# SiyuanHuang95/SUG

Measured on AMD Instinct MI355X. Metric: point-clouds/sec (train step, N=1024), higher is better.
Workload: dtype f32

## Files before the change

include/sug_amd.h:

```cpp
#ifndef SUG_AMD_H
#define SUG_AMD_H

#include <stdint.h>

#ifdef __cplusplus
extern "C" {
#endif

#define SUG_OK 0
#define SUG_ERR_ARG (-1)
#define SUG_ERR_LAUNCH (-2)
#define SUG_STATS_BLOCKS 1024

const char* sug_last_error(void);
#define SUG_ABI_VERSION 7
int sug_abi_version(void);

int sug_knn(const float* x, int64_t ldx, int B, int N, int C, int k,
            int32_t* idx, void* stream);

int sug_knn_reverse(const int32_t* idx, int B, int N, int k,
                    int32_t* rev_off, int32_t* rev_ent, void* stream);

int sug_fps(const float* xyz, const int32_t* start, int B, int N, int npoint,
            int32_t* out, void* stream);

int sug_ball_query(const float* xyz, const float* query, int B, int N, int S,
                   float r2, int nsample, int32_t* out, void* stream);

int sug_knn_query(const float* xyz, const float* query, int B, int N, int S,
                  int k, int32_t* idx_out, float* dist_out, void* stream);
int sug_knn_query_direct(const float* xyz, const float* query, int B, int N, int S, int k,
                         int32_t* idx_out, float* dist_out, void* stream);

int sug_three_nn(const float* query, const float* cand, int B, int N, int S,
                 int32_t* idx3, float* dist3, void* stream);

int sug_three_nn_direct(const float* query, const float* cand, int B, int N, int S,
                        int32_t* idx3, float* dist3, void* stream);

int sug_ball_query_multi(const float* xyz, const float* query, int B, int N, int S, int R, const float* r2,
                         const int32_t* nsample, int32_t* const* out, void* stream);

int sug_fp_interp_fwd(const float* src, int64_t lds, const int32_t* idx3, const float* d3, int B, int N, int S, int D,
                      float* out, int64_t ldo, float* w3, void* stream);
int sug_fp_interp_bwd(const float* g, int64_t ldg, const int32_t* idx3, const float* w3, int B, int N, int S, int D,
                      int32_t* rev_off, int32_t* rev_ent, float* dsrc, int64_t ldd, void* stream);

int sug_copy_rows2d(const float* src, int64_t lds, float* dst, int64_t ldd, int64_t rows, int C, void* stream);

int sug_gather_rows(const float* feat, int64_t ldf, const int32_t* idx,
                    int B, int N, int S, int C, float* out, int64_t ldo, void* stream);
int sug_scatter_add_rows(const float* g, int64_t ldg, const int32_t* idx,
                         int B, int N, int S, int C, float* dfeat, int64_t ldf, void* stream);
int64_t sug_scatter_rows_workspace(int B, int N, int S);
int sug_scatter_rows_ordered_supported(int B, int N, int S);
int sug_scatter_rows_ordered(const float* g, int64_t ldg, const int32_t* idx, int B, int N, int S, int C,
                             float* dfeat, int64_t ldf, int32_t* ws, void* stream);

int sug_group_max(const float* feat, int64_t ldf, const int32_t* idx, int B, int N, int S,
                  int ns, int C, float* out, int32_t* arg, void* stream);
int sug_group_max_bwd(const float* g, const int32_t* arg, int B, int N, int S, int C,
                      float* dfeat, int64_t ldf, void* stream);

int sug_edgeconv_fwd(const float* pq, int64_t ldpq, const int32_t* idx, const float* gamma,
                     int B, int N, int k, int Co, float* z, uint8_t* arg, float* s1,
                     double* stats, float* ws, void* stream);

int sug_bn_finalize(const double* stats, const float* gamma, const float* beta, int C,
                    double count, float eps, float momentum, float* running_mean,
                    float* running_var, float* coef, void* stream);

int sug_edgeconv_fwd_bn(const float* pq, int64_t ldpq, const int32_t* idx, const float* gamma,
                        const float* beta, int B, int N, int k, int Co, float eps, float momentum,
                        float* running_mean, float* running_var, float* z, uint8_t* arg, float* s1,
                        float* coef, float* ws, void* stream);
int sug_col_stats_bn(const float* y, int64_t ldy, int64_t rows, int C, const float* gamma, const float* beta,
                     float eps, float momentum, float* running_mean, float* running_var, float* coef,
                     float* ws, void* stream);

int sug_col_stats_bn_grouped(const float* y, int64_t ldy, int64_t rows, int C, int groups, const float* gamma,
                             const float* beta, float eps, float momentum, float* running_mean, float* running_var,
                             float* coef, float* ws, void* stream);

int sug_bn_replay(const float* coef, int G, int C, float momentum, float* running_mean, float* running_var,
                  void* stream);
int sug_bn_replay_multi(int n, const void* const* coef, const int32_t* G, const int32_t* C, const float* momentum,
                        void* const* running_mean, void* const* running_var, void* stream);

int sug_affine_act(const float* z, int64_t ldz, const float* coef, int64_t rows, int C,
                   float slope, float* out, int64_t ldo, void* stream);

int sug_col_stats(const float* y, int64_t ldy, int64_t rows, int C, double* stats, float* ws,
                  void* stream);

int sug_edgeconv_bwd_reduce(const float* gout, int64_t ldg, const float* z, const float* coef,
                            int64_t rows, int Co, float slope, float* a, double* red, float* ws,
                            void* stream);
int sug_edgeconv_bwd_scatter(const float* a, const uint8_t* arg, const float* s1,
                             const float* pq, int64_t ldpq, const int32_t* rev_off,
                             const int32_t* rev_ent, const float* coef, const double* red,
                             int B, int N, int k, int Co, float* dpq, int64_t lddpq, void* stream);

int64_t sug_linear_dw_workspace(int64_t R, int M, int N);
int sug_linear_dw(const float* g, int64_t ldg, const float* x, int64_t ldx, int64_t R, int M, int N,
                  float* dw, float* ws, void* stream);
int sug_linear_dw_fold(const float* part, int nchunk, int64_t MN, float* dw, void* stream);
int sug_linear_dw_bias(const float* g, int64_t ldg, const float* x, int64_t ldx, int64_t R, int M, int N,
                       float* dw, float* db, float* ws, void* stream);

int64_t sug_colsum_workspace(int64_t rows, int C);
int sug_colsum(const void* x, int64_t ld, int64_t rows, int C, int dtype, float sign, float* out, float* ws, void* stream);

int sug_gate_fwd(const float* x, const float* z, int64_t n, float* out, void* stream);
int sug_gate_bwd(const float* g, const float* x, const float* z, int64_t n, float* dx, float* dz, void* stream);
int sug_gate_bn_fwd(const float* x, const float* z, int M, int C, const float* gamma, const float* beta,
                    float* running_mean, float* running_var, int training, float eps, float momentum, float* out,
                    float* stat, void* stream);
int sug_gate_bn_bwd(const float* g, const float* x, const float* z, int M, int C, const float* gamma, const float* stat,
                    int training, float* dx, float* dz, float* dgamma, float* dbeta, void* stream);

int sug_calayer_supported(int layers, int M, int C, int Hd);
int sug_calayer_fwd(int layers, const float* x, int64_t ldx, int M, int C, int Hd, const float* const* W0,
                    const float* const* b0, const float* const* W2, const float* const* b2, float* hp, float* h, float* z,
                    void* stream);
int sug_calayer_bwd(int layers, const float* x, int64_t ldx, int M, int C, int Hd, const float* const* W0,
                    const float* const* W2, const float* h, const float* dz, const float* dxg, float* const* dW0,
                    float* const* db0, float* const* dW2, float* const* db2, float* dhp, float* dh, float* dx, int64_t lddx,
                    void* stream);

int sug_head_linear_supported(int M, int K, int No, int pro, int epi);
int sug_head_linear_fwd(int heads, const float* const* in, int64_t ldin, const float* const* W, const float* const* bias,
                        float* const* z, const float* const* gamma, const float* const* beta, const float* const* u,
                        float* const* stats, float* const* act, int M, int K, int No, int pro, float slope, float eps,
                        float p_drop, void* stream);
int sug_head_ln_bwd(int heads, const float* const* gup, int64_t ldg, const float* const* z, const float* const* stats,
                    const float* const* gamma, const float* const* beta, const float* const* u,
                    const float* const* gextra, float* const* dz, float* const* dgamma, float* const* dbeta,
                    float* const* db, int M, int No, float slope, float p_drop, void* stream);
int sug_head_linear_bwd(int heads, int sum_da, const float* const* dz, int64_t ldg, const float* const* in, int64_t ldin,
                        const float* const* stats_in, const float* const* gamma_in, const float* const* beta_in,
                        const float* const* u_in, const float* const* W, float* const* dW, float* const* db,
                        float* const* da, int64_t ldda, int M, int K, int No, int pro, float slope, float p_drop_in,
                        void* stream);

int sug_ln_act_fwd(const float* x, const float* gamma, const float* beta, int rows, int C, float eps, float slope,
                   float* y, float* stat, void* stream);
int sug_ln_act_bwd(const float* g, const float* x, const float* gamma, const float* beta, const float* stat, int rows,
                   int C, float slope, float* dx, float* dgamma, float* dbeta, float* ws, void* stream);

int sug_adam_chunk(void);
int sug_adam_step(const int64_t* table, const int32_t* block_first, const int32_t* block_first_host, int T,
                  const void* const* grads_host, double lr, double beta1, double beta2, double eps,
                  double weight_decay, double bias_corr1, double bias_corr2, void* stream);
int sug_adam_step_capturable(const int64_t* table, const int32_t* block_first, const int32_t* block_first_host,
                             int T, const void* const* grads_host, double lr, double beta1, double beta2,
                             double eps, double weight_decay, int32_t* step_dev, float* scalars_dev,
                             const double* lr_dev, void* stream);

#define SUG_ADAM_CHAIN_SLOTS 2
#define SUG_ADAM_CHAIN_BUCKETS 8
int sug_adam_chain_chunk(void);
int sug_adam_chain_step(const int64_t* table, const int32_t* block_map, const int32_t* block_first_host, int T,
                        const void* const* grads_host, int nbuckets, const double* hyper_host, int32_t* steps_dev,
                        float* scalars_dev, const double* lr_dev, void* stream);

int sug_node_offset_fwd(const float* proj, const float* loc, const int32_t* fidx,
                        const int32_t* gidx, int B, int N, int S, int ns, float* off, float* nloc,
                        void* stream);
int sug_node_offset_bwd(const float* proj, const float* loc, const int32_t* fidx,
                        const int32_t* gidx, const float* goff, int B, int N, int S, int ns,
                        float* dproj, void* stream);
int sug_interp3_cat_fwd(const float* fea, int64_t ldf, int C1, const float* node,
                        const int32_t* idx3, const float* d3, int B, int N, int S, int C2,
                        float* out, int64_t ldo, void* stream);
int sug_interp3_cat_bwd(const float* g, int64_t ldg, int C1, const float* node, const int32_t* idx3,
                        const float* d3, const float* xyz, const float* nloc, int B, int N, int S,
                        int C2, float* dnode, float* dnloc, void* stream);
int sug_interp3_cat_bwd_lists(const float* g, int64_t ldg, int C1, const float* node, const int32_t* idx3,
                              const float* d3, const float* xyz, const float* nloc, int B, int N, int S, int C2,
                              int32_t* rev_off, int32_t* rev_ent, float* ddw, float* dnode, float* dnloc,
                              void* stream);
int sug_interp3_cat_bwd_lists_supported(int B, int N, int S);

int sug_bn_bwd_apply(const float* a, const float* y, int64_t ldy, const float* coef,
                     const double* red, int64_t rows, int C, float* dy, int64_t lddy, void* stream);

int sug_bn_act_pool_fwd(const float* y, int64_t ldy, const float* coef, int B, int N, int C,
                        float slope, float* out_max, float* out_mean, int64_t ld_pool, int32_t* arg, float* ws,
                        void* stream);
int sug_bn_act_pool_bwd(const float* y, int64_t ldy, const float* coef, const float* gmax,
                        const float* gmean, int64_t ld_pool, const int32_t* arg, int B, int N, int C, float slope,
                        int train, double* red, float* ws, float* dy, int64_t lddy, void* stream);

int sug_edgeconv_layer_fwd(const float* pq, int64_t ldpq, const int32_t* idx, const float* gamma,
                           const float* beta, int B, int N, int k, int Co, int groups, int training,
                           float eps, float momentum, float slope, float* running_mean,
                           float* running_var, float* z, uint8_t* arg, float* s1, float* coef,
                           float* out, int64_t ldo, double* stats, float* ws, void* stream);
int sug_edgeconv_fused_supported(int N, int k, int Cin, int Co);
int sug_edgeconv_fused_layer_fwd(const float* x, int64_t ldx, int Cin, const float* wcat, const float* qbias,
                                 const int32_t* idx, const float* gamma, const float* beta, int B, int N, int k,
                                 int Co, int groups, int training, float eps, float momentum, float slope,
                                 float* running_mean, float* running_var, float* z, uint8_t* arg, float* s1,
                                 float* pq_out, int64_t ldpq, float* coef, float* out, int64_t ldo, float* ws,
                                 void* stream);
int sug_edgeconv_layer_bwd(const float* gout, int64_t ldg, const float* z, const uint8_t* arg,
                           const float* s1, const float* pq, int64_t ldpq, const int32_t* idx,
                           const float* coef, int B, int N, int k, int Co, int groups, int training,
                           float slope, float* a, double* red, int32_t* rev_off, int32_t* rev_ent,
                           float* dpq, int64_t lddpq, float* ws, float* dgb, void* stream);
int sug_sa_first_fwd(const float* P, int64_t ldp, const float* Q, const int32_t* idx, int B, int N, int S,
                     int ns, int C, int groups, const float* gamma, const float* beta, int training,
                     float eps, float momentum, float* running_mean, float* running_var, float* coef,
                     float* Z, float* ws, void* stream);
int sug_sa_first_bwd(const float* gz, const float* P, int64_t ldp, const float* Q, const int32_t* idx, int B,
                     int N, int S, int ns, int C, int groups, int training, const float* coef, double* red,
                     int32_t* rev_off, int32_t* rev_ent, float* segsum, float* dP, float* dQ, float* ws, float* dgb,
                     void* stream);
int sug_sa_first_geo_fwd(const float* Pf, int64_t ldp, const float* xyz, const float* cent, const float* Wx, int ldw,
                         const float* bias, const int32_t* idx, int B, int N, int S, int ns, int C, int groups,
                         const float* gamma, const float* beta, int training, float eps, float momentum,
                         float* running_mean, float* running_var, float* coef, float* Z, float* ws, void* stream);
int sug_sa_first_geo_bwd(const float* gz, const float* Pf, int64_t ldp, const float* xyz, const float* cent, const float* Wx,
                         int ldw, const float* bias, const int32_t* idx, int B, int N, int S, int ns, int C, int groups,
                         int training, const float* coef, double* red, int32_t* rev_off, int32_t* rev_ent, float* segsum,
                         float* dP, float* dQ, float* ws, float* dgb, void* stream);

int sug_bn_act_rows_fwd(const float* y, int64_t ldy, int64_t rows, int C, int groups, const float* gamma,
                        const float* beta, int training, float eps, float momentum, float slope,
                        float* running_mean, float* running_var, float* coef, float* out, int64_t ldo,
                        double* stats, float* ws, void* stream);
int sug_bn_act_rows_bwd(const float* gout, int64_t ldg, const float* y, int64_t ldy, const float* coef,
                        int64_t rows, int C, int groups, int training, float slope, float* a, double* red,
                        float* dy, float* ws, float* dgb, void* stream);
int sug_bn_act_pool_layer_fwd(const float* y, int64_t ldy, int B, int N, int C, int groups,
                              const float* gamma, const float* beta, int training, float eps, float momentum,
                              float slope, float* running_mean, float* running_var, float* coef,
                              float* out_max, float* out_mean, int64_t ld_pool, int32_t* arg, double* stats, float* ws_stats,
                              float* ws_pool, void* stream);
int sug_bn_act_pool_layer_bwd(const float* y, int64_t ldy, const float* coef, const float* gmax,
                              const float* gmean, int64_t ld_pool, const int32_t* arg, int B, int N, int C, int groups,
                              float slope, int training, double* red, float* ws, float* dy, int64_t lddy,
                              float* dgb, void* stream);

int sug_pointmlp_max_fwd(const float* x, int64_t ldx, int64_t rows, int K, const float* w, const float* bias,
                         const float* gamma, int Co, int seg, float* zext, int32_t* arg, float* ws, int* nblk,
                         void* stream);
int sug_rows_gemm(const float* x, int64_t ldx, int64_t rows, int K, const float* w, const float* bias, int Co,
                  float* y, int64_t ldy, void* stream);
int sug_pointmlp_max_layer_fwd(const float* x, int64_t ldx, int64_t rows, int K, const float* w, const float* bias,
                               const float* gamma, const float* beta, int Co, int seg, int groups, int training,
                               float eps, float momentum, float slope, float* running_mean, float* running_var,
                               float* zext, int32_t* arg, float* coef, float* out, int64_t ldo, float* ws,
                               void* stream);
int sug_pointmlp_max_layer_fwd_xf(const float* y, int64_t ldy, int64_t rows, int K, const float* xcoef, float xslope,
                                  float* zout, int64_t ldz, const float* w, const float* bias, const float* gamma,
                                  const float* beta, int Co, int seg, int groups, int training, float eps, float momentum,
                                  float slope, float* running_mean, float* running_var, float* zext, int32_t* arg,
                                  float* coef, float* out, int64_t ldo, float* ws, void* stream);
int sug_pointmlp_max_bwd_coef(const float* coef, const double* red, const float* bias, const float* w, int64_t rows,
                              int K, int Co, float* kb, float* k2, float* nkb, float* nwk, void* stream);
int sug_pointmlp_max_bwd_dwfix(float* dw, const float* dws, const float* kb, const float* k2, const float* w,
                               const float* xtx, const float* sx, int K, int Co, int with_stats, void* stream);
int64_t sug_pointmlp_max_bwd_workspace(int64_t rows, int K, int Co, int seg);
int sug_pointmlp_max_bwd_sparse(const float* a, const int32_t* arg, const float* x, int64_t ldx, const float* w,
                                int64_t rows, int K, int Co, int seg, float* dx, int64_t lddx, float* dw,
                                float* ws, void* stream);

int sug_ptran_pos1_fwd(const float* xyz, const int32_t* nbr, const float* w1, const float* b1, int B, int n, int k,
                       int d, int dtype, void* out, void* stream);
int sug_ptran_pos1_bwd(const void* g, const float* xyz, const int32_t* nbr, const float* w1, const float* b1, int B,
                       int n, int k, int d, int dtype, float* dw1, float* db1, float* ws, void* stream);
int sug_ptran_qk_fwd(const float* q, const float* kf, const void* delta, const int32_t* nbr, int B, int n, int k, int d,
                     int dtype, void* out, void* stream);
int sug_ptran_qk_bwd(const void* du, void* da, const int32_t* rev_off, const int32_t* rev_ent, int B, int n, int k, int d,
                     int dtype, float* dq, float* dk, float* db, float* ws, void* stream);
int sug_ptran_attn_fwd(const void* logits, const void* delta, const float* vf, const int32_t* nbr, int B, int n, int k,
                       int d, int dtype, float scale, float* mixed, float* mx, float* sm, void* stream);
int sug_ptran_attn_bwd(const float* g, const float* mixed, const void* logits, const void* delta, const float* vf,
                       const int32_t* nbr, const float* mx, const float* sm, const int32_t* rev_off, const int32_t* rev_ent,
                       int B, int n, int k, int d, int dtype, float scale, void* dlogits, void* da, float* dv, float* db,
                       float* ws, void* stream);
int sug_ptran_fused_supported(int B, int n, int k, int d);
int sug_ptran_fused_fwd(const float* xyz, const int32_t* nbr, const float* q, const float* kf, const float* vf,
                        const float* w1, const float* b1, const void* w2, const void* b2, const void* wg1, const void* bg1,
                        const void* wg2, const void* bg2, int B, int n, int k, int d, float scale, int save, void* T0,
                        void* delta, void* U, void* T1, void* Lg, float* mixed, float* mx, float* sm, void* stream);
int64_t sug_ptran_colsum_workspace(int64_t rows);
int sug_ptran_relu_bwd_db(void* G, const void* T1, int64_t rows, int d, int dtype, float* db, float* ws, void* stream);
int sug_grad_scale16(const float* g0, int64_t n0, const float* g1, int64_t n1, const float* g2, int64_t n2, int log2_target,
                     float* out, float* ws, void* stream);

int sug_fold_groups(const double* red, int groups, int n, float* out, void* stream);

int sug_mmd_rbf(const float* z, int64_t ldz, int m, int D, const float* w,
                const float* neg_gamma, int nsigma, double* sums, float* wt, void* stream);

int sug_mmd_rbf_value(const float* z, int64_t ldz, int m, int D, const float* w, const float* neg_gamma,
                      int nsigma, double* sums, float* wt, float* value, void* stream);

int sug_mmd_rbf_bwd(const float* z, int64_t ldz, const float* wt, int m, int D, const float* gscale,
                    float* dz, int64_t lddz, void* stream);

int sug_mmd_rbf_rows(const float* z, int64_t ldz, int m, int D, const float* w, const float* neg_gamma,
                     int nsigma, int row0, int mloc, double* sums, float* wt, void* stream);
int sug_mmd_rbf_rows_bwd(const float* z, int64_t ldz, const float* wt, int m, int D, int row0, int mloc,
                         const float* gscale, float gmul, float* dz, int64_t lddz, void* stream);

int sug_sda_prob_weights(const float* pred_s, int64_t lds, const float* pred_t, int64_t ldt,
                         const int64_t* label_s, const int64_t* label_t, int m, int num_class,
                         float label_weight, int method, float* weights, void* stream);
int sug_sda_prob_weights_multi(int n, const void* const* pred_s, const int64_t* lds, const void* const* pred_t,
                               const int64_t* ldt, const int64_t* label_s, const int64_t* label_t, int m, int num_class,
                               float label_weight, int method, void* const* weights, void* stream);

int sug_mmd_assemble(const float* feat_s, int64_t lds, const float* feat_t, int64_t ldt, const int64_t* label_s,
                     const int64_t* label_t, int m, int D, int num_class, float label_scale, float* z, void* stream);

int sug_soft_mmd_multi_fwd(int n, const void* const* feat_s, const int64_t* lds, const void* const* feat_t,
                           const int64_t* ldt, const int32_t* D, const float* label_scale, const int64_t* label_s,
                           const int64_t* label_t, int m, int num_class, const void* const* w, const float* neg_gamma,
                           int nsigma, void* const* z, void* const* wt, double* sums, float* values, void* stream);
int sug_soft_mmd_multi_bwd(int n, const void* const* z, const int32_t* D, const void* const* wt,
                           const void* const* gscale, int m, int num_class, void* const* dz, void* stream);

#define SUG_CLASS_MMD_MAX_ROWS 1024
#define SUG_CLASS_MMD_MAX_CLASSES 64
#define SUG_CLASS_MMD_MAX_D 1048576
int sug_mmd_select(const int64_t* label_s, const int64_t* label_t, int m, int num_class, int mode, int32_t* idx_s,
                   int32_t* idx_t, int32_t* pos_s, int32_t* pos_t, int32_t* count, void* stream);
int sug_class_mmd_fwd(const float* feat_s, int64_t lds, const float* feat_t, int64_t ldt, int m, int D,
                      const int32_t* idx_s, const int32_t* idx_t, const int32_t* count, const float* neg_gamma,
                      int nsigma, float* z, float* wt, double* sums, float* value, void* stream);
int sug_class_mmd_bwd(const float* z, const float* wt, int m, int D, const int32_t* count, const int32_t* pos_s,
                      const int32_t* pos_t, const float* gscale, float* dz, float* dfeat_s, int64_t ldds,
                      float* dfeat_t, int64_t lddt, void* stream);

#define SUG_MMD_EST_MAX_ROWS 1024
#define SUG_MMD_EST_MAX_D 1048576
#define SUG_MMD_EST_MAX_SIGMAS 8
#define SUG_MMD_POLY_MAX_DEGREE 8
#define SUG_MMD_RATIO_ROW_FIELDS 9
#define SUG_MMD_RATIO_STATS 16
int sug_mmd_ratio_fwd(const float* z, int64_t ldz, int m, int D, const float* neg_gamma, int nsigma, int biased, float* K,
                      float* G, double* rows, double* stats, float* out3, float* wt_m, float* wt_v, void* stream);
int sug_mmd_ratio_bwd(const float* z, int64_t ldz, int m, int D, const float* wt_m, const float* wt_v, const float* out3,
                      const float* g3, float* dz, int64_t lddz, void* stream);
int sug_mmd_adjacent_fwd(const float* x, int64_t ldx, const float* y, int64_t ldy, int m, int D, int mode, int degree,
                         double alpha, double c, double* part, float* coef, float* value, void* stream);
int sug_mmd_adjacent_bwd(const float* x, int64_t ldx, const float* y, int64_t ldy, int m, int D, int mode, const float* coef,
                         const float* gscale, float* dx, int64_t lddx, float* dy, int64_t lddy, void* stream);

#define SUG_CL_LOSS_MAX_ROWS 1024
#define SUG_CL_LOSS_MAX_D 1048576
#define SUG_CL_LOSS_MAX_TERMS 4
#define SUG_CL_LOSS_SUM_FIELDS 3
#define SUG_CL_LOSS_ROW_FIELDS 4
int sug_cl_loss_fwd(int n, const void* const* x, const int64_t* ldx, const void* const* y, const int64_t* ldy, const int32_t* D,
                    const double* margin, const int64_t* label_s, const int64_t* label_t, int m, const void* const* w,
                    double* sums, void* const* coef, float* values, void* stream);
int sug_cl_loss_bwd(int n, const void* const* x, const int64_t* ldx, const void* const* y, const int64_t* ldy, const int32_t* D,
                    int m, const void* const* coef, const void* const* gscale, void* const* dx, const int64_t* lddx,
                    void* const* dy, const int64_t* lddy, void* stream);

int sug_edge_weight_split(const float* in, int Co, int C, int backward, float* out, void* stream);
int sug_edge_weight_split_multi(const void* const* in_host, const int32_t* Co_host, const int32_t* C_host, int n,
                                int backward, void* const* out_host, void* stream);

int64_t sug_chamfer_workspace(int B, int N, int M);
int sug_chamfer(const float* a, const float* b, int B, int N, int M, float* out, float* ws, void* stream);
int sug_chamfer_weights(const float* a, const float* b, int B, int N, int M, int method, float* out, float* ws, void* stream);

#define SUG_CE_PAIR_MAX_ROWS 512
#define SUG_CE_PAIR_MAX_CLASSES 32
int sug_ce_pair_fwd(const float* logits1, const float* logits2, int64_t ld, const int64_t* label, int M, int C, float w,
                    int64_t ignore_index, float* loss, float* lse, void* stream);
int sug_ce_pair_bwd(const float* logits1, const float* logits2, int64_t ld, const int64_t* label, int M, int Mtot, int C,
                    float w, int64_t ignore_index, const float* g, const float* lse, float* d1, float* d2, void* stream);
#define SUG_CE_MAX_ROWS 1024
#define SUG_CE_MAX_CLASSES 64
int sug_ce_fwd(const float* logits, int64_t ld, const int64_t* label, int M, int C, int64_t ignore_index, float label_smoothing,
               float* loss, float* lse, double* totals, void* stream);
int sug_ce_bwd(const float* logits, int64_t ld, const int64_t* label, int M, int C, int64_t ignore_index, float label_smoothing,
               const float* g, const float* lse, float* dlogits, void* stream);
#define SUG_MCD_MAX_ROWS 1024
int sug_mcd_loss_fwd(const float* ys1, const float* ys2, const float* yt1, const float* yt2, int64_t ld, const int64_t* label,
                     const int64_t* label_t, int Ms, int Mt, int C, float a_s, float a_t, float r_s, float* out4, float* lse,
                     double* totals, void* stream);
int sug_mcd_loss_bwd(const float* ys1, const float* ys2, const float* yt1, const float* yt2, int64_t ld, const int64_t* label,
                     const int64_t* label_t, int Ms, int Mt, int C, float a_s, float a_t, const float* g, const float* lse,
                     float* ds1, float* ds2, float* dt1, float* dt2, void* stream);
int sug_cls_loss_fwd(const float* ys1, const float* ys2, const float* yt1, const float* yt2, int64_t ld, const int64_t* label,
                     const int64_t* label_t, int Ms, int Mt, int C, const float* alpha, float gamma, int reduce_sum,
                     int64_t ignore_index, float a_s, float a_t, float a_d, float r_s, float* out4, float* save, double* totals,
                     void* stream);
int sug_cls_loss_bwd(const float* ys1, const float* ys2, const float* yt1, const float* yt2, int64_t ld, const int64_t* label,
                     const int64_t* label_t, int Ms, int Mt, int C, const float* alpha, float gamma, int reduce_sum,
                     int64_t ignore_index, float a_s, float a_t, float a_d, float r_s, const float* g, const float* save,
                     float* ds1, float* ds2, float* dt1, float* dt2, void* stream);
int sug_loss_combine_fwd(const float* loss_cls, const float* v_geo, const float* v_sem1, const float* v_sem2, float wg, float ws,
                         float* out3, void* stream);
int sug_loss_combine_bwd(const float* g, float wg, float ws, float* out4, void* stream);

#define SUG_EVAL_MAX_ROWS 4096
#define SUG_EVAL_MAX_CLASSES 64
#define SUG_EVAL_BATCH_COUNT 0
#define SUG_EVAL_DATA_TOTAL 1
#define SUG_EVAL_CORRECT_TOTAL 2
#define SUG_EVAL_ERROR 3
#define SUG_EVAL_LOSS_TOTAL 4
#define SUG_EVAL_CLASS_ACC 8
#define SUG_EVAL_CLASS_ROWS 136
#define SUG_EVAL_CLASS_CORRECT 200
#define SUG_EVAL_BATCH_ACC 264
#define SUG_EVAL_STATE_WORDS(cap) (SUG_EVAL_BATCH_ACC + (cap))
int sug_eval_accumulate(const float* logits1, const float* logits2, int64_t ld, const int64_t* label, int B, int C,
                        const float* loss_in, int ce_mode, int64_t ignore_index, float label_smoothing, float* out,
                        int64_t* pred, int cls_eval, void* state, int cap, void* stream);


#define SUG_KPCONV_MAX_CLOUD 4096
int sug_grid_subsample(const float* pts, const int32_t* off, int B, int cap, float dl, float* out_pad, int32_t* cnt,
                       float* out, int32_t* out_off, void* stream);
int sug_radius_neighbors(const float* q, const int32_t* qoff, int Nq, const float* s, const int32_t* soff, int Ns, int B,
                         float radius, int limit, int32_t* out, void* stream);
int sug_radius_reverse(const int32_t* nbr, const int32_t* qoff, const int32_t* soff, int B, int H, int Ns, int cap,
                       int32_t* rev_be, int32_t* rev_ent, void* stream);
int sug_kpconv_fwd(const float* q, const float* s, const int32_t* nbr, int Nq, int H, int Ns, const float* kp, int K,
                   float extent, const float* x, int Cin, float* wf, float* w, float* cnt, void* stream);
int sug_kpconv_bwd(const int32_t* rev_be, const int32_t* rev_ent, int H, int K, const float* w, const float* cnt,
                   const float* dwf, int Ns, int Cin, float* dx, void* stream);
int sug_seg_instnorm_fwd(const float* x, const int32_t* off, int B, int C, float eps, int mode, const float* sc, float* y,
                         float* mean, float* rstd, void* stream);
int sug_seg_instnorm_bwd(const float* g, const float* y, const float* x, const float* mean, const float* rstd,
                         const int32_t* off, int B, int C, int mode, float* dx, float* dsc, void* stream);
int sug_seg_max_pool_fwd(const float* x, const int32_t* nbr, int Nq, int H, int Ns, int C, float* y, int32_t* arg,
                         void* stream);
int sug_seg_max_pool_bwd(const float* g, const int32_t* arg, const int32_t* rev_be, const int32_t* rev_ent, int H, int Ns,
                         int C, float* dx, void* stream);
int sug_seg_mean_fwd(const float* x, const int32_t* off, int B, int C, float* y, void* stream);
int sug_seg_mean_bwd(const float* g, const int32_t* off, int B, int N, int C, float* dx, void* stream);
#define SUG_KPCONV_RECORD_INTS 8
int sug_grid_subsample_cap(const float* pts, const int32_t* off, int B, int cap, float dl, int C, int level, float* out_pad,
                           int32_t* cnt, float* out, int32_t* out_off, int32_t* record, void* stream);
int sug_radius_neighbors_cap(const float* q, const int32_t* qoff, int Cq, const float* s, const int32_t* soff, int Cs, int B,
                             float radius, int limit, int32_t* out, void* stream);
int sug_radius_reverse_cap(const int32_t* nbr, const int32_t* qoff, const int32_t* soff, int B, int H, int Cs, int cap,
                           int32_t* rev_be, int32_t* rev_ent, void* stream);
int sug_kpconv_fwd_cap(const float* q, const float* s, const int32_t* nbr, const int32_t* nq_valid, int Cq, int H, int Cs,
                       const float* kp, int K, float extent, const float* x, int Cin, float* wf, float* w, float* cnt,
                       void* stream);
int sug_seg_instnorm_fwd_cap(const float* x, const int32_t* off, int B, int N, int C, float eps, int mode, const float* sc,
                             float* y, float* mean, float* rstd, void* stream);
int sug_seg_instnorm_bwd_cap(const float* g, const float* y, const float* x, const float* mean, const float* rstd,
                             const int32_t* off, int B, int N, int C, int mode, float* dx, float* dsc, void* stream);
int sug_seg_mean_fwd_cap(const float* x, const int32_t* off, int B, int C, float* y, void* stream);
int sug_seg_mean_bwd_cap(const float* g, const int32_t* off, int B, int N, int C, float* dx, void* stream);
int sug_kp_sample_rows(const float* x, const int32_t* off, int B, int S, int D, float* out, void* stream);

int sug_ptcls_head_supported(int B, int P, int K, int N1, int N2, int NC);
int sug_ptcls_head_fwd(const float* points, int B, int P, int K, const float* W1, const float* b1, int N1, const float* W2,
                       const float* b2, int N2, const float* W3, const float* b3, int NC, float* mean, float* h1, float* h2,
                       float* logits, void* stream);
int sug_ptcls_head_bwd(const float* dlogits, const float* mean, const float* h1, const float* h2, int B, int P, int K,
                       const float* W1, int N1, const float* W2, int N2, const float* W3, int NC, float* dz1, float* dz2,
                       float* dpoints, float* dW1, float* db1, float* dW2, float* db2, float* dW3, float* db3,
                       void* stream);

#define SUG_PREP_MAX_POINTS 4096
#define SUG_PREP_NORMALIZE 1
#define SUG_PREP_ROTATE_Z 2
#define SUG_PREP_JITTER 4
#define SUG_PREP_SHUFFLE 8
#define SUG_PREP_DRAW_ANGLE 0x00000000u
#define SUG_PREP_DRAW_SUBSET 0x10000000u
#define SUG_PREP_DRAW_NOISE 0x20000000u
int sug_prepare_batch(const float* pts, int M, int P, const int32_t* idx, int B, int N, int stages,
// ... 33 lines not shown
```

sug_amd/csrc/adapt.hip:

```cpp
#include "common.h"

namespace {

__global__ __launch_bounds__(256) void node_offset_fwd_kernel(const float* __restrict__ proj,
                                                              const float* __restrict__ loc,
                                                              const int32_t* __restrict__ fidx,
                                                              const int32_t* __restrict__ gidx, int N,
                                                              int S, int ns, int total,
                                                              float* __restrict__ off,
                                                              float* __restrict__ nloc) {
  const int e = blockIdx.x * 4 + (threadIdx.x >> 6);
  if (e >= total) return;
  const int lane = threadIdx.x & 63;
  const int b = e / S;
  const float* pb = proj + (int64_t)b * N * 3;
  const float* lb = loc + (int64_t)b * N * 3;
  int f = fidx[e];
  f = f < 0 ? 0 : (f >= N ? N - 1 : f);
  const float pcx = pb[f * 3 + 0], pcy = pb[f * 3 + 1], pcz = pb[f * 3 + 2];
  const float lcx = lb[f * 3 + 0], lcy = lb[f * 3 + 1], lcz = lb[f * 3 + 2];
  float ax = 0.f, ay = 0.f, az = 0.f;
  const int32_t* g = gidx + (int64_t)e * ns;
  for (int j = lane; j < ns; j += 64) {
    const int n = g[j];
    if (n < 0 || n >= N) continue;
    ax += tanhf(pb[n * 3 + 0] - pcx) * (lb[n * 3 + 0] - lcx);
    ay += tanhf(pb[n * 3 + 1] - pcy) * (lb[n * 3 + 1] - lcy);
    az += tanhf(pb[n * 3 + 2] - pcz) * (lb[n * 3 + 2] - lcz);
  }
  ax = wave_sum_f(ax); ay = wave_sum_f(ay); az = wave_sum_f(az);
  if (lane == 0) {
    const float inv = 1.0f / (float)ns;
    ax *= inv; ay *= inv; az *= inv;
    off[e * 3 + 0] = ax; off[e * 3 + 1] = ay; off[e * 3 + 2] = az;
    nloc[e * 3 + 0] = lcx + ax; nloc[e * 3 + 1] = lcy + ay; nloc[e * 3 + 2] = lcz + az;
  }
}

__global__ __launch_bounds__(256) void node_offset_bwd_kernel(const float* __restrict__ proj,
                                                              const float* __restrict__ loc,
                                                              const int32_t* __restrict__ fidx,
                                                              const int32_t* __restrict__ gidx,
                                                              const float* __restrict__ goff, int N,
                                                              int S, int ns, int total,
                                                              float* __restrict__ dproj) {
  const int e = blockIdx.x * 4 + (threadIdx.x >> 6);
  if (e >= total) return;
  const int lane = threadIdx.x & 63;
  const int b = e / S;
  const float* pb = proj + (int64_t)b * N * 3;
  const float* lb = loc + (int64_t)b * N * 3;
  float* db = dproj + (int64_t)b * N * 3;
  int f = fidx[e];
  f = f < 0 ? 0 : (f >= N ? N - 1 : f);
  const float pcx = pb[f * 3 + 0], pcy = pb[f * 3 + 1], pcz = pb[f * 3 + 2];
  const float lcx = lb[f * 3 + 0], lcy = lb[f * 3 + 1], lcz = lb[f * 3 + 2];
  const float inv = 1.0f / (float)ns;
  const float gx = goff[e * 3 + 0] * inv, gy = goff[e * 3 + 1] * inv, gz = goff[e * 3 + 2] * inv;
  float cx = 0.f, cy = 0.f, cz = 0.f;
  const int32_t* g = gidx + (int64_t)e * ns;
  for (int j = lane; j < ns; j += 64) {
    const int n = g[j];
    if (n < 0 || n >= N) continue;
    const float tx = tanhf(pb[n * 3 + 0] - pcx), ty = tanhf(pb[n * 3 + 1] - pcy), tz = tanhf(pb[n * 3 + 2] - pcz);
    const float vx = gx * (lb[n * 3 + 0] - lcx) * (1.f - tx * tx);
    const float vy = gy * (lb[n * 3 + 1] - lcy) * (1.f - ty * ty);
    const float vz = gz * (lb[n * 3 + 2] - lcz) * (1.f - tz * tz);
    atomicAdd(&db[n * 3 + 0], vx); atomicAdd(&db[n * 3 + 1], vy); atomicAdd(&db[n * 3 + 2], vz);
    cx += vx; cy += vy; cz += vz;
  }
  cx = wave_sum_f(cx); cy = wave_sum_f(cy); cz = wave_sum_f(cz);
  if (lane == 0) {
    atomicAdd(&db[f * 3 + 0], -cx); atomicAdd(&db[f * 3 + 1], -cy); atomicAdd(&db[f * 3 + 2], -cz);
  }
}

__global__ __launch_bounds__(1024) void node_offset_bwd_lds_kernel(const float* __restrict__ proj,
                                                                   const float* __restrict__ loc,
                                                                   const int32_t* __restrict__ fidx,
                                                                   const int32_t* __restrict__ gidx,
                                                                   const float* __restrict__ goff, int N, int S,
                                                                   int ns, float* __restrict__ dproj) {
  extern __shared__ float s_d[];
  const int b = blockIdx.x;
  const int lane = threadIdx.x & 63, wave = threadIdx.x >> 6;
  for (int i = threadIdx.x; i < N * 3; i += 1024) s_d[i] = 0.f;
  __syncthreads();
  const float* pb = proj + (int64_t)b * N * 3;
  const float* lb = loc + (int64_t)b * N * 3;
  const float inv = 1.0f / (float)ns;
  for (int sn = wave; sn < S; sn += 16) {
    const int e = b * S + sn;
    int f = fidx[e];
    f = f < 0 ? 0 : (f >= N ? N - 1 : f);
    const float pcx = pb[f * 3 + 0], pcy = pb[f * 3 + 1], pcz = pb[f * 3 + 2];
    const float lcx = lb[f * 3 + 0], lcy = lb[f * 3 + 1], lcz = lb[f * 3 + 2];
    const float gx = goff[e * 3 + 0] * inv, gy = goff[e * 3 + 1] * inv, gz = goff[e * 3 + 2] * inv;
    float cx = 0.f, cy = 0.f, cz = 0.f;
    const int32_t* g = gidx + (int64_t)e * ns;
    for (int j = lane; j < ns; j += 64) {
      const int n = g[j];
      if (n < 0 || n >= N) continue;
      const float tx = tanhf(pb[n * 3 + 0] - pcx), ty = tanhf(pb[n * 3 + 1] - pcy), tz = tanhf(pb[n * 3 + 2] - pcz);
      const float vx = gx * (lb[n * 3 + 0] - lcx) * (1.f - tx * tx);
      const float vy = gy * (lb[n * 3 + 1] - lcy) * (1.f - ty * ty);
      const float vz = gz * (lb[n * 3 + 2] - lcz) * (1.f - tz * tz);
      atomicAdd(&s_d[n * 3 + 0], vx); atomicAdd(&s_d[n * 3 + 1], vy); atomicAdd(&s_d[n * 3 + 2], vz);
      cx += vx; cy += vy; cz += vz;
    }
    cx = wave_sum_f(cx); cy = wave_sum_f(cy); cz = wave_sum_f(cz);
    if (lane == 0) {
      atomicAdd(&s_d[f * 3 + 0], -cx); atomicAdd(&s_d[f * 3 + 1], -cy); atomicAdd(&s_d[f * 3 + 2], -cz);
    }
  }
  __syncthreads();
  float* db = dproj + (int64_t)b * N * 3;
  for (int i = threadIdx.x; i < N * 3; i += 1024) db[i] = s_d[i];
}

template <int P>
__global__ __launch_bounds__(64 * P) void node_offset_bwd_ordered_kernel(const float* __restrict__ proj,
                                                                         const float* __restrict__ loc,
                                                                         const int32_t* __restrict__ fidx,
                                                                         const int32_t* __restrict__ gidx,
                                                                         const float* __restrict__ goff, int N, int S,
                                                                         int ns, float* __restrict__ dproj) {
  extern __shared__ __attribute__((aligned(16))) float s_o[];
  const int lane = threadIdx.x & 63, wave = threadIdx.x >> 6;
  float* plane = s_o + (size_t)wave * 3 * N;
  int* tag = reinterpret_cast<int*>(s_o + (size_t)P * 3 * N) + (size_t)wave * N;
  const int b = blockIdx.x;
  for (int i = lane; i < 3 * N; i += 64) plane[i] = 0.f;
  __builtin_amdgcn_wave_barrier();
  const float* pb = proj + (int64_t)b * N * 3;
  const float* lb = loc + (int64_t)b * N * 3;
  const float inv = 1.0f / (float)ns;
  auto add_node = [&](int n, float vx, float vy, float vz) {
    if (n >= 0) tag[n] = 0x7fffffff;
    __builtin_amdgcn_wave_barrier();
    if (n >= 0) atomicMin(&tag[n], lane);
    __builtin_amdgcn_wave_barrier();
    const int leader = n >= 0 ? tag[n] : lane;
    unsigned long long dup = __ballot(leader != lane);
    float ax = vx, ay = vy, az = vz;
    while (dup) {
      const int i = __builtin_ctzll(dup);
      dup &= dup - 1;
      const int li = __builtin_amdgcn_readlane(leader, i);
      const float dx = __int_as_float(__builtin_amdgcn_readlane(__float_as_int(vx), i));
      const float dy = __int_as_float(__builtin_amdgcn_readlane(__float_as_int(vy), i));
      const float dz = __int_as_float(__builtin_amdgcn_readlane(__float_as_int(vz), i));
      const bool mine = lane == li;
      ax = mine ? ax + dx : ax; ay = mine ? ay + dy : ay; az = mine ? az + dz : az;
    }
    if (n >= 0 && leader == lane) {
      plane[n * 3 + 0] += ax; plane[n * 3 + 1] += ay; plane[n * 3 + 2] += az;
    }
    __builtin_amdgcn_wave_barrier();
  };
  auto centre = [&](int f, float cx, float cy, float cz) {
    cx = wave_sum_f(cx); cy = wave_sum_f(cy); cz = wave_sum_f(cz);
    if (lane == 0) {
      plane[f * 3 + 0] -= cx; plane[f * 3 + 1] -= cy; plane[f * 3 + 2] -= cz;
    }
    __builtin_amdgcn_wave_barrier();
  };
  if (ns <= 64) {
    struct Idx { int f, n; float gx, gy, gz; };
    struct Val { float pc[3], lc[3], pn[3], ln[3]; };
    auto load_idx = [&](int sn) {
      Idx r;
      const int e = b * S + sn;
      int f = fidx[e];
      r.f = f < 0 ? 0 : (f >= N ? N - 1 : f);
      int n = lane < ns ? gidx[(int64_t)e * ns + lane] : -1;
      r.n = n >= N ? -1 : n;
      r.gx = goff[e * 3 + 0] * inv; r.gy = goff[e * 3 + 1] * inv; r.gz = goff[e * 3 + 2] * inv;
      return r;
    };
    auto load_val = [&](const Idx& ix) {
      Val v;
      const int n = ix.n >= 0 ? ix.n : ix.f;
#pragma unroll
      for (int d = 0; d < 3; ++d) {
        v.pc[d] = pb[ix.f * 3 + d]; v.lc[d] = lb[ix.f * 3 + d];
        v.pn[d] = pb[n * 3 + d];    v.ln[d] = lb[n * 3 + d];
      }
      return v;
    };
    Idx i0 = {}, i1 = {};
    Val v0 = {};
    if (wave < S) { i0 = load_idx(wave); v0 = load_val(i0); }
    if (wave + P < S) i1 = load_idx(wave + P);
    for (int sn = wave; sn < S; sn += P) {
      const Idx ci = i0;
      const Val cv = v0;
      i0 = i1;
      if (sn + P < S) v0 = load_val(i0);
      if (sn + 2 * P < S) i1 = load_idx(sn + 2 * P);
      float vx = 0.f, vy = 0.f, vz = 0.f;
      if (ci.n >= 0) {
        const float tx = tanhf(cv.pn[0] - cv.pc[0]), ty = tanhf(cv.pn[1] - cv.pc[1]), tz = tanhf(cv.pn[2] - cv.pc[2]);
        vx = ci.gx * (cv.ln[0] - cv.lc[0]) * (1.f - tx * tx);
        vy = ci.gy * (cv.ln[1] - cv.lc[1]) * (1.f - ty * ty);
        vz = ci.gz * (cv.ln[2] - cv.lc[2]) * (1.f - tz * tz);
      }
      add_node(ci.n, vx, vy, vz);
      centre(ci.f, vx, vy, vz);
    }
  } else {
    for (int sn = wave; sn < S; sn += P) {
      const int e = b * S + sn;
      int f = fidx[e];
      f = f < 0 ? 0 : (f >= N ? N - 1 : f);
      const float pcx = pb[f * 3 + 0], pcy = pb[f * 3 + 1], pcz = pb[f * 3 + 2];
      const float lcx = lb[f * 3 + 0], lcy = lb[f * 3 + 1], lcz = lb[f * 3 + 2];
      const float gx = goff[e * 3 + 0] * inv, gy = goff[e * 3 + 1] * inv, gz = goff[e * 3 + 2] * inv;
      float cx = 0.f, cy = 0.f, cz = 0.f;
      const int32_t* g = gidx + (int64_t)e * ns;
      for (int j0 = 0; j0 < ns; j0 += 64) {
        const int j = j0 + lane;
        int n = j < ns ? g[j] : -1;
        if (n >= N) n = -1;
        float vx = 0.f, vy = 0.f, vz = 0.f;
        if (n >= 0) {
          const float tx = tanhf(pb[n * 3 + 0] - pcx), ty = tanhf(pb[n * 3 + 1] - pcy), tz = tanhf(pb[n * 3 + 2] - pcz);
          vx = gx * (lb[n * 3 + 0] - lcx) * (1.f - tx * tx);
          vy = gy * (lb[n * 3 + 1] - lcy) * (1.f - ty * ty);
          vz = gz * (lb[n * 3 + 2] - lcz) * (1.f - tz * tz);
        }
        cx += vx; cy += vy; cz += vz;
        add_node(n, vx, vy, vz);
      }
      centre(f, cx, cy, cz);
    }
  }
  __syncthreads();
  float* db = dproj + (int64_t)b * N * 3;
  for (int i = threadIdx.x; i < N * 3; i += 64 * P) {
    float a = s_o[i];
#pragma unroll
    for (int p = 1; p < P; ++p) a += s_o[(size_t)p * 3 * N + i];
    db[i] = a;
  }
}

__global__ __launch_bounds__(256) void interp3_cat_fwd_kernel(const float* __restrict__ fea, int64_t ldf,
                                                              int C1, const float* __restrict__ node,
                                                              const int32_t* __restrict__ idx3,
                                                              const float* __restrict__ d3, int N, int S,
                                                              int C2, int64_t BN, float* __restrict__ out,
                                                              int64_t ldo) {
  const int64_t p = (int64_t)blockIdx.x * 16 + threadIdx.x / 16;
  if (p >= BN) return;
  const int lane = threadIdx.x & 15;
  const int64_t b = p / N;
  const float r0 = 1.0f / fmaxf(d3[p * 3 + 0], 1e-10f), r1 = 1.0f / fmaxf(d3[p * 3 + 1], 1e-10f),
              r2 = 1.0f / fmaxf(d3[p * 3 + 2], 1e-10f);
  const float R = (r0 + r1) + r2;
  const float w0 = r0 / R, w1 = r1 / R, w2 = r2 / R;
  const float* n0 = node + (b * S + idx3[p * 3 + 0]) * C2;
  const float* n1 = node + (b * S + idx3[p * 3 + 1]) * C2;
  const float* n2 = node + (b * S + idx3[p * 3 + 2]) * C2;
  for (int c = lane * 4; c < C1; c += 64)
    *reinterpret_cast<float4*>(out + p * ldo + c) = *reinterpret_cast<const float4*>(fea + p * ldf + c);
  for (int c = lane * 4; c < C2; c += 64) {
    const float4 a = *reinterpret_cast<const float4*>(n0 + c), bq = *reinterpret_cast<const float4*>(n1 + c),
                 cq = *reinterpret_cast<const float4*>(n2 + c);
    float4 o;
    o.x = (a.x * w0 + bq.x * w1) + cq.x * w2; o.y = (a.y * w0 + bq.y * w1) + cq.y * w2;
    o.z = (a.z * w0 + bq.z * w1) + cq.z * w2; o.w = (a.w * w0 + bq.w * w1) + cq.w * w2;
    *reinterpret_cast<float4*>(out + p * ldo + C1 + c) = o;
  }
}

__global__ __launch_bounds__(256) void interp3_cat_bwd_kernel(const float* __restrict__ g, int64_t ldg,
                                                              int C1, const float* __restrict__ node,
                                                              const int32_t* __restrict__ idx3,
                                                              const float* __restrict__ d3,
                                                              const float* __restrict__ xyz,
                                                              const float* __restrict__ nloc, int N,
                                                              int S, int C2, int chunks,
                                                              float* __restrict__ dnode,
                                                              float* __restrict__ dnloc) {
  extern __shared__ float s_acc[];
  float* s_dn = s_acc;
  float* s_dl = s_acc + S * C2;
  const int b = blockIdx.y, ck = blockIdx.x;
  for (int i = threadIdx.x; i < S * C2 + S * 3; i += 256) s_acc[i] = 0.f;
  __syncthreads();
  const int lane = threadIdx.x & 15, grp = threadIdx.x >> 4;
  const int n0 = (int)((int64_t)N * ck / chunks), n1 = (int)((int64_t)N * (ck + 1) / chunks);
  const float* nodeb = node + (int64_t)b * S * C2;
  for (int n = n0 + grp; n < n1 + 15; n += 16) {
    const bool live = n < n1;
    const int64_t p = (int64_t)b * N + (live ? n : n0);
    const float d0 = d3[p * 3 + 0], d1 = d3[p * 3 + 1], d2 = d3[p * 3 + 2];
    const float r0 = 1.0f / fmaxf(d0, 1e-10f), r1 = 1.0f / fmaxf(d1, 1e-10f), r2 = 1.0f / fmaxf(d2, 1e-10f);
    const float R = (r0 + r1) + r2;
    const float w0 = r0 / R, w1 = r1 / R, w2 = r2 / R;
    const int i0 = idx3[p * 3 + 0], i1 = idx3[p * 3 + 1], i2 = idx3[p * 3 + 2];
    float s0 = 0.f, s1 = 0.f, s2 = 0.f;
    if (live) {
      for (int c = lane * 4; c < C2; c += 64) {
        const float4 gv = *reinterpret_cast<const float4*>(g + p * ldg + C1 + c);
        const float4 a = *reinterpret_cast<const float4*>(nodeb + i0 * C2 + c);
        const float4 bq = *reinterpret_cast<const float4*>(nodeb + i1 * C2 + c);
        const float4 cq = *reinterpret_cast<const float4*>(nodeb + i2 * C2 + c);
        const float gg[4] = {gv.x, gv.y, gv.z, gv.w};
        const float aa[4] = {a.x, a.y, a.z, a.w}, bb[4] = {bq.x, bq.y, bq.z, bq.w}, cc[4] = {cq.x, cq.y, cq.z, cq.w};
#pragma unroll
        for (int v = 0; v < 4; ++v) {
          const float o = (aa[v] * w0 + bb[v] * w1) + cc[v] * w2;
          s0 += gg[v] * (aa[v] - o); s1 += gg[v] * (bb[v] - o); s2 += gg[v] * (cc[v] - o);
          atomicAdd(&s_dn[i0 * C2 + c + v], w0 * gg[v]);
          atomicAdd(&s_dn[i1 * C2 + c + v], w1 * gg[v]);
          atomicAdd(&s_dn[i2 * C2 + c + v], w2 * gg[v]);
        }
      }
    }
#pragma unroll
    for (int o = 8; o > 0; o >>= 1) {
      s0 += __shfl_xor(s0, o); s1 += __shfl_xor(s1, o); s2 += __shfl_xor(s2, o);
    }
    if (live && lane < 3) {
      const float sv = lane == 0 ? s0 : (lane == 1 ? s1 : s2);
      const float d = lane == 0 ? d0 : (lane == 1 ? d1 : d2);
      const float r = lane == 0 ? r0 : (lane == 1 ? r1 : r2);
      const int i = lane == 0 ? i0 : (lane == 1 ? i1 : i2);
      const float dd = (d < 1e-10f) ? 0.f : -(r * r / R) * sv;
      const float* q = xyz + p * 3;
      const float* cpos = nloc + ((int64_t)b * S + i) * 3;
      atomicAdd(&s_dl[i * 3 + 0], dd * 2.f * (cpos[0] - q[0]));
      atomicAdd(&s_dl[i * 3 + 1], dd * 2.f * (cpos[1] - q[1]));
      atomicAdd(&s_dl[i * 3 + 2], dd * 2.f * (cpos[2] - q[2]));
    }
  }
  __syncthreads();
  float* dnb = dnode + (int64_t)b * S * C2;
  float* dlb = dnloc + (int64_t)b * S * 3;
  for (int i = threadIdx.x; i < S * C2; i += 256) atomicAdd(&dnb[i], s_dn[i]);
  for (int i = threadIdx.x; i < S * 3; i += 256) atomicAdd(&dlb[i], s_dl[i]);
}

__global__ __launch_bounds__(256) void interp3_bwd_point_kernel(const float* __restrict__ g, int64_t ldg, int C1,
                                                                const float* __restrict__ node,
                                                                const int32_t* __restrict__ idx3,
                                                                const float* __restrict__ d3, int N, int S, int C2,
                                                                int64_t BN, float* __restrict__ ddw) {
  const int64_t p = (int64_t)blockIdx.x * 16 + threadIdx.x / 16;
  if (p >= BN) return;
  const int lane = threadIdx.x & 15;
  const int64_t b = p / N;
  const float d0 = d3[p * 3 + 0], d1 = d3[p * 3 + 1], d2 = d3[p * 3 + 2];
  const float r0 = 1.0f / fmaxf(d0, 1e-10f), r1 = 1.0f / fmaxf(d1, 1e-10f), r2 = 1.0f / fmaxf(d2, 1e-10f);
  const float R = (r0 + r1) + r2;
  const float w0 = r0 / R, w1 = r1 / R, w2 = r2 / R;
  const float* n0 = node + (b * S + idx3[p * 3 + 0]) * C2;
  const float* n1 = node + (b * S + idx3[p * 3 + 1]) * C2;
  const float* n2 = node + (b * S + idx3[p * 3 + 2]) * C2;
  float s0 = 0.f, s1 = 0.f, s2 = 0.f;
  for (int c = lane * 4; c < C2; c += 64) {
    const float4 gv = *reinterpret_cast<const float4*>(g + p * ldg + C1 + c);
    const float4 a = *reinterpret_cast<const float4*>(n0 + c), bq = *reinterpret_cast<const float4*>(n1 + c),
                 cq = *reinterpret_cast<const float4*>(n2 + c);
    const float gg[4] = {gv.x, gv.y, gv.z, gv.w};
    const float aa[4] = {a.x, a.y, a.z, a.w}, bb[4] = {bq.x, bq.y, bq.z, bq.w}, cc[4] = {cq.x, cq.y, cq.z, cq.w};
#pragma unroll
    for (int v = 0; v < 4; ++v) {
      const float o = (aa[v] * w0 + bb[v] * w1) + cc[v] * w2;
      s0 += gg[v] * (aa[v] - o); s1 += gg[v] * (bb[v] - o); s2 += gg[v] * (cc[v] - o);
    }
  }
#pragma unroll
  for (int o = 8; o > 0; o >>= 1) {
    s0 += __shfl_xor(s0, o); s1 += __shfl_xor(s1, o); s2 += __shfl_xor(s2, o);
  }
  if (lane < 3) {
    const float sv = lane == 0 ? s0 : (lane == 1 ? s1 : s2);
    const float d = lane == 0 ? d0 : (lane == 1 ? d1 : d2);
    const float r = lane == 0 ? r0 : (lane == 1 ? r1 : r2);
    const float w = lane == 0 ? w0 : (lane == 1 ? w1 : w2);
    ddw[p * 6 + lane] = (d < 1e-10f) ? 0.f : -(r * r / R) * sv;
    ddw[p * 6 + 3 + lane] = w;
  }
}

__global__ __launch_bounds__(256) void interp3_bwd_node_kernel(const float* __restrict__ g, int64_t ldg, int C1,
                                                               const float* __restrict__ ddw,
                                                               const int32_t* __restrict__ rev_off,
                                                               const int32_t* __restrict__ rev_ent,
                                                               const float* __restrict__ xyz,
                                                               const float* __restrict__ nloc, int N, int S, int C2,
                                                               int64_t BS, float* __restrict__ dnode,
                                                               float* __restrict__ dnloc) {
  const int64_t q = (int64_t)blockIdx.x * 16 + threadIdx.x / 16;
  if (q >= BS) return;
  const int lane = threadIdx.x & 15;
  const int64_t b = q / S;
  const int sn = (int)(q - b * S);
  const int32_t* offb = rev_off + b * (S + 1);
  const int off = offb[sn], cnt = offb[sn + 1] - off;
  const int32_t* ent = rev_ent + b * 3 * N + off;
  const int ax = lane < 3 ? lane : 0;
  const float cpos = nloc[q * 3 + ax];
  float dl = 0.f;
  const int npass = (C2 + 63) / 64;
  for (int pass = 0; pass < npass; ++pass) {
    const int c0 = pass * 64 + lane * 4;
    const bool chan = c0 < C2;
    float4 acc = make_float4(0, 0, 0, 0);
    constexpr int JB = 8;
    for (int t0 = 0; t0 < cnt; t0 += JB) {
      int en[JB];
      float4 gv[JB];
      float wv[JB], dv[JB], xv[JB];
#pragma unroll
      for (int t = 0; t < JB; ++t) en[t] = ent[t0 + t < cnt ? t0 + t : cnt - 1];
#pragma unroll
      for (int t = 0; t < JB; ++t) {
        const int n = en[t] / 3, tt = en[t] - 3 * n;
        const int64_t p = b * N + n;
        gv[t] = chan ? *reinterpret_cast<const float4*>(g + p * ldg + C1 + c0) : make_float4(0, 0, 0, 0);
        wv[t] = ddw[p * 6 + 3 + tt];
        dv[t] = ddw[p * 6 + tt];
        xv[t] = xyz[p * 3 + ax];
      }
#pragma unroll
      for (int t = 0; t < JB; ++t) {
        if (t0 + t >= cnt) continue;
        acc.x = fmaf(wv[t], gv[t].x, acc.x); acc.y = fmaf(wv[t], gv[t].y, acc.y);
        acc.z = fmaf(wv[t], gv[t].z, acc.z); acc.w = fmaf(wv[t], gv[t].w, acc.w);
        if (pass == 0) dl += dv[t] * 2.f * (cpos - xv[t]);
      }
    }
    if (chan) *reinterpret_cast<float4*>(dnode + q * C2 + c0) = acc;
  }
  if (lane < 3) dnloc[q * 3 + lane] = dl;
}

}

extern "C" int sug_node_offset_fwd(const float* proj, const float* loc, const int32_t* fidx,
                                   const int32_t* gidx, int B, int N, int S, int ns, float* off,
                                   float* nloc, void* stream) {
  SUG_REQUIRE(proj && loc && fidx && gidx && off && nloc, "sug_node_offset_fwd: null pointer");
  SUG_REQUIRE(B > 0 && N > 0 && S > 0 && ns > 0, "sug_node_offset_fwd: bad shape");
  const int total = B * S;
  hipLaunchKernelGGL(node_offset_fwd_kernel, dim3(sug_divup(total, 4)), dim3(256), 0, (hipStream_t)stream,
                     proj, loc, fidx, gidx, N, S, ns, total, off, nloc);
  SUG_LAUNCH_CHECK("sug_node_offset_fwd");
  return SUG_OK;
}

extern "C" int sug_node_offset_bwd(const float* proj, const float* loc, const int32_t* fidx,
                                   const int32_t* gidx, const float* goff, int B, int N, int S, int ns,
                                   float* dproj, void* stream) {
  SUG_REQUIRE(proj && loc && fidx && gidx && goff && dproj, "sug_node_offset_bwd: null pointer");
  SUG_REQUIRE(B > 0 && N > 0 && S > 0 && ns > 0, "sug_node_offset_bwd: bad shape");
  const int total = B * S;
  hipStream_t st = (hipStream_t)stream;
  {
    static const int unordered = getenv("SUG_NODE_OFFSET_UNORDERED") ? atoi(getenv("SUG_NODE_OFFSET_UNORDERED")) : 0;
    const size_t per_plane = (size_t)N * 4 * sizeof(float);
    if (!unordered && per_plane <= 150 * 1024) {
      if (8 * per_plane <= 150 * 1024) {
        static SugLdsOptIn note;
        if (int rc = sug_allow_dynamic_lds(note, &node_offset_bwd_ordered_kernel<8>, 150 * 1024, "sug_node_offset_bwd")) return rc;
        hipLaunchKernelGGL(node_offset_bwd_ordered_kernel<8>, dim3(B), dim3(512), 8 * per_plane, st, proj, loc, fidx, gidx, goff, N,
                           S, ns, dproj);
      } else if (4 * per_plane <= 150 * 1024) {
        static SugLdsOptIn note;
        if (int rc = sug_allow_dynamic_lds(note, &node_offset_bwd_ordered_kernel<4>, 150 * 1024, "sug_node_offset_bwd")) return rc;
        hipLaunchKernelGGL(node_offset_bwd_ordered_kernel<4>, dim3(B), dim3(256), 4 * per_plane, st, proj, loc, fidx, gidx, goff, N,
                           S, ns, dproj);
      } else if (2 * per_plane <= 150 * 1024) {
        static SugLdsOptIn note;
        if (int rc = sug_allow_dynamic_lds(note, &node_offset_bwd_ordered_kernel<2>, 150 * 1024, "sug_node_offset_bwd")) return rc;
        hipLaunchKernelGGL(node_offset_bwd_ordered_kernel<2>, dim3(B), dim3(128), 2 * per_plane, st, proj, loc, fidx, gidx, goff, N,
                           S, ns, dproj);
      } else {
        static SugLdsOptIn note;
        if (int rc = sug_allow_dynamic_lds(note, &node_offset_bwd_ordered_kernel<1>, 150 * 1024, "sug_node_offset_bwd")) return rc;
        hipLaunchKernelGGL(node_offset_bwd_ordered_kernel<1>, dim3(B), dim3(64), per_plane, st, proj, loc, fidx, gidx, goff, N, S,
                           ns, dproj);
      }
      SUG_LAUNCH_CHECK("sug_node_offset_bwd");
      return SUG_OK;
    }
  }
  if ((size_t)N * 3 * sizeof(float) <= 60 * 1024) {
    hipLaunchKernelGGL(node_offset_bwd_lds_kernel, dim3(B), dim3(1024), (size_t)N * 3 * sizeof(float), st, proj, loc, fidx,
                       gidx, goff, N, S, ns, dproj);
    SUG_LAUNCH_CHECK("sug_node_offset_bwd");
    return SUG_OK;
  }
  if (hipMemsetAsync(dproj, 0, (size_t)B * N * 3 * sizeof(float), st) != hipSuccess) {
    sug_set_error("sug_node_offset_bwd: memset failed");
    return SUG_ERR_LAUNCH;
  }
  hipLaunchKernelGGL(node_offset_bwd_kernel, dim3(sug_divup(total, 4)), dim3(256), 0, st,
                     proj, loc, fidx, gidx, goff, N, S, ns, total, dproj);
  SUG_LAUNCH_CHECK("sug_node_offset_bwd");
  return SUG_OK;
}

extern "C" int sug_interp3_cat_fwd(const float* fea, int64_t ldf, int C1, const float* node,
                                   const int32_t* idx3, const float* d3, int B, int N, int S, int C2,
                                   float* out, int64_t ldo, void* stream) {
  SUG_REQUIRE((fea || C1 == 0) && node && idx3 && d3 && out, "sug_interp3_cat_fwd: null pointer");
  SUG_REQUIRE(B > 0 && N > 0 && S >= 3 && C1 >= 0 && C2 > 0 && C1 % 4 == 0 && C2 % 4 == 0 && ldf % 4 == 0 &&
                  ldo % 4 == 0 && ldo >= C1 + C2 && ldf >= C1,
              "sug_interp3_cat_fwd: bad shape (channel counts and strides must be multiples of 4)");
  SUG_REQUIRE(((uintptr_t)fea % 16 == 0) && ((uintptr_t)node % 16 == 0) && ((uintptr_t)out % 16 == 0),
              "sug_interp3_cat_fwd: pointers must be 16-byte aligned");
  const int64_t BN = (int64_t)B * N;
  hipLaunchKernelGGL(interp3_cat_fwd_kernel, dim3(sug_divup(BN, 16)), dim3(256), 0, (hipStream_t)stream, fea,
                     ldf, C1, node, idx3, d3, N, S, C2, BN, out, ldo);
  SUG_LAUNCH_CHECK("sug_interp3_cat_fwd");
  return SUG_OK;
}

extern "C" int sug_interp3_cat_bwd(const float* g, int64_t ldg, int C1, const float* node,
                                   const int32_t* idx3, const float* d3, const float* xyz,
                                   const float* nloc, int B, int N, int S, int C2, float* dnode,
                                   float* dnloc, void* stream) {
  SUG_REQUIRE(g && node && idx3 && d3 && xyz && nloc && dnode && dnloc, "sug_interp3_cat_bwd: null pointer");
  SUG_REQUIRE(B > 0 && N > 0 && S >= 3 && C2 > 0 && C1 % 4 == 0 && C2 % 4 == 0 && ldg % 4 == 0 &&
                  ldg >= C1 + C2 && ((uintptr_t)g % 16 == 0) && ((uintptr_t)node % 16 == 0),
              "sug_interp3_cat_bwd: bad shape / alignment");
  const size_t sh = (size_t)(S * C2 + S * 3) * sizeof(float);
  SUG_REQUIRE(sh <= 64 * 1024 && B <= 65535, "sug_interp3_cat_bwd: S*C2=%d too large for the LDS accumulator", S * C2);
  int chunks = 512 / B;
  if (chunks < 1) chunks = 1;
  if (chunks > sug_divup(N, 64)) chunks = sug_divup(N, 64);
  hipLaunchKernelGGL(interp3_cat_bwd_kernel, dim3(chunks, B), dim3(256), sh, (hipStream_t)stream, g, ldg, C1, node,
                     idx3, d3, xyz, nloc, N, S, C2, chunks, dnode, dnloc);
  SUG_LAUNCH_CHECK("sug_interp3_cat_bwd");
  return SUG_OK;
}

size_t sug_reverse_lists_lds_bytes(int B, int E, int N, int* ranges);

extern "C" int sug_interp3_cat_bwd_lists_supported(int B, int N, int S) {
  return (B > 0 && N > 0 && S >= 3 && (int64_t)3 * N <= INT32_MAX &&
          sug_reverse_lists_lds_bytes(B, 3 * N, S, nullptr) <= 160 * 1024) ? 1 : 0;
}

extern "C" int sug_interp3_cat_bwd_lists(const float* g, int64_t ldg, int C1, const float* node, const int32_t* idx3,
                                         const float* d3, const float* xyz, const float* nloc, int B, int N, int S, int C2,
                                         int32_t* rev_off, int32_t* rev_ent, float* ddw, float* dnode, float* dnloc,
                                         void* stream) {
  SUG_REQUIRE(g && node && idx3 && d3 && xyz && nloc && rev_off && rev_ent && ddw && dnode && dnloc,
              "sug_interp3_cat_bwd_lists: null pointer");
  SUG_REQUIRE(B > 0 && N > 0 && S >= 3 && C2 > 0 && C1 % 4 == 0 && C2 % 4 == 0 && ldg % 4 == 0 &&
                  ldg >= C1 + C2 && ((uintptr_t)g % 16 == 0) && ((uintptr_t)node % 16 == 0) && ((uintptr_t)dnode % 16 == 0),
              "sug_interp3_cat_bwd_lists: bad shape / alignment");
  hipStream_t st = (hipStream_t)stream;
  if (int rc = sug_reverse_lists(idx3, B, 3 * N, S, 1, rev_off, rev_ent, st)) return rc;
  const int64_t BN = (int64_t)B * N, BS = (int64_t)B * S;
  hipLaunchKernelGGL(interp3_bwd_point_kernel, dim3(sug_divup(BN, 16)), dim3(256), 0, st, g, ldg, C1, node, idx3, d3, N, S, C2,
                     BN, ddw);
  SUG_LAUNCH_CHECK("sug_interp3_cat_bwd_lists(point)");
  hipLaunchKernelGGL(interp3_bwd_node_kernel, dim3(sug_divup(BS, 16)), dim3(256), 0, st, g, ldg, C1, ddw, rev_off, rev_ent, xyz,
                     nloc, N, S, C2, BS, dnode, dnloc);
  SUG_LAUNCH_CHECK("sug_interp3_cat_bwd_lists(node)");
  return SUG_OK;
}
```

sug_amd/csrc/group.hip:

```cpp
#include "common.h"

namespace {

__global__ __launch_bounds__(256) void gather_rows_kernel(const float* __restrict__ feat, int64_t ldf,
                                                          const int32_t* __restrict__ idx, int N,
                                                          int S, int C, int64_t total,
                                                          float* __restrict__ out, int64_t ldo) {
  for (int64_t e = (int64_t)blockIdx.x * 256 + threadIdx.x; e < total; e += (int64_t)gridDim.x * 256) {
    const int c = (int)(e % C);
    const int64_t row = e / C;
    const int b = (int)(row / S);
    const int j = idx[row];
    float v = 0.f;
    if (j >= 0 && j < N) v = feat[((int64_t)b * N + j) * ldf + c];
    out[row * ldo + c] = v;
  }
}

__global__ __launch_bounds__(256) void scatter_add_rows_kernel(const float* __restrict__ g, int64_t ldg,
                                                               const int32_t* __restrict__ idx, int N,
                                                               int S, int C, int64_t total,
                                                               float* __restrict__ dfeat, int64_t ldf) {
  for (int64_t e = (int64_t)blockIdx.x * 256 + threadIdx.x; e < total; e += (int64_t)gridDim.x * 256) {
    const int c = (int)(e % C);
    const int64_t row = e / C;
    const int b = (int)(row / S);
    const int j = idx[row];
    if (j >= 0 && j < N) atomicAdd(&dfeat[((int64_t)b * N + j) * ldf + c], g[row * ldg + c]);
  }
}

__global__ __launch_bounds__(256) void group_max_kernel(const float* __restrict__ feat, int64_t ldf,
                                                        const int32_t* __restrict__ idx, int N, int S,
                                                        int ns, int C, int64_t total,
                                                        float* __restrict__ out,
                                                        int32_t* __restrict__ arg) {
  for (int64_t e = (int64_t)blockIdx.x * 256 + threadIdx.x; e < total; e += (int64_t)gridDim.x * 256) {
    const int c = (int)(e % C);
    const int64_t row = e / C;
    const int b = (int)(row / S);
    const int32_t* ir = idx + row * ns;
    float best = -INFINITY;
    int bj = -1;
    for (int t0 = 0; t0 < ns; t0 += 8) {
      int j[8];
      float v[8];
#pragma unroll
      for (int u = 0; u < 8; ++u) j[u] = ir[t0 + u < ns ? t0 + u : ns - 1];
#pragma unroll
      for (int u = 0; u < 8; ++u) {
        const int jc = j[u] < 0 ? 0 : (j[u] >= N ? N - 1 : j[u]);
        v[u] = feat[((int64_t)b * N + jc) * ldf + c];
      }
#pragma unroll
      for (int u = 0; u < 8; ++u) {
        if (t0 + u >= ns || j[u] < 0 || j[u] >= N) continue;
        if (v[u] > best || bj < 0) {
          best = v[u];
          bj = j[u];
        }
      }
    }
    out[e] = bj < 0 ? 0.f : best;
    arg[e] = bj;
  }
}

__global__ __launch_bounds__(256) void group_max_bwd_kernel(const float* __restrict__ g,
                                                            const int32_t* __restrict__ arg, int N,
                                                            int S, int C, int64_t total,
                                                            float* __restrict__ dfeat, int64_t ldf) {
  for (int64_t e = (int64_t)blockIdx.x * 256 + threadIdx.x; e < total; e += (int64_t)gridDim.x * 256) {
    const int c = (int)(e % C);
    const int64_t row = e / C;
    const int b = (int)(row / S);
    const int j = arg[e];
    if (j >= 0 && j < N) atomicAdd(&dfeat[((int64_t)b * N + j) * ldf + c], g[e]);
  }
}

inline int ew_grid(int64_t total) {
  int64_t g = (total + 255) / 256;
  return (int)(g > 4096 ? 4096 : (g < 1 ? 1 : g));
}

__global__ __launch_bounds__(256) void copy_rows2d_kernel(const float* __restrict__ src, int64_t lds, float* __restrict__ dst,
                                                          int64_t ldd, int64_t R, int C4) {
  const int64_t total = R * C4;
  for (int64_t e = (int64_t)blockIdx.x * 256 + threadIdx.x; e < total; e += (int64_t)gridDim.x * 256) {
    const int64_t r = e / C4;
    const int c = (int)(e - r * C4) * 4;
    *reinterpret_cast<float4*>(dst + r * ldd + c) = *reinterpret_cast<const float4*>(src + r * lds + c);
  }
}

template <int V>
__global__ __launch_bounds__(256) void gather_sum_rows_kernel(const float* __restrict__ g, int64_t ldg,
                                                              const int32_t* __restrict__ rev_off,
                                                              const int32_t* __restrict__ rev_ent, int N, int S, int C,
                                                              int64_t total, float* __restrict__ dfeat, int64_t ldf) {
  const int CV = C / V;
  for (int64_t t = (int64_t)blockIdx.x * 256 + threadIdx.x; t < total; t += (int64_t)gridDim.x * 256) {
    const int c = (int)(t % CV) * V;
    const int64_t row = t / CV;
    const int64_t b = row / N;
    const int n = (int)(row - b * N);
    const int32_t* off = rev_off + b * (N + 1) + n;
    const int e0 = off[0], e1 = off[1];
    const int32_t* ent = rev_ent + b * S;
    float acc[V];
#pragma unroll
    for (int v = 0; v < V; ++v) acc[v] = 0.f;
    for (int i = e0; i < e1; ++i) {
      const float* gr = g + (b * S + ent[i]) * ldg + c;
      if (V == 4) {
        const float4 q = *reinterpret_cast<const float4*>(gr);
        acc[0] += q.x; acc[1] += q.y; acc[2] += q.z; acc[3] += q.w;
      } else {
#pragma unroll
        for (int v = 0; v < V; ++v) acc[v] += gr[v];
      }
    }
#pragma unroll
    for (int v = 0; v < V; ++v) dfeat[row * ldf + c + v] = acc[v];
  }
}

constexpr int GMB_CH = 16;
__global__ __launch_bounds__(256) void group_max_bwd_ordered_kernel(const float* __restrict__ g,
                                                                    const int32_t* __restrict__ arg, int N, int S, int C,
                                                                    float* __restrict__ dfeat, int64_t ldf) {
  extern __shared__ __attribute__((aligned(16))) int s_gm[];
  int (*s_arg)[GMB_CH + 1] = reinterpret_cast<int (*)[GMB_CH + 1]>(s_gm);
  float (*s_g)[GMB_CH + 1] = reinterpret_cast<float (*)[GMB_CH + 1]>(s_gm + 64 * (GMB_CH + 1));
  const int lane = threadIdx.x & 63, wv = threadIdx.x >> 6;
  int* tag = s_gm + 2 * 64 * (GMB_CH + 1) + wv * N;
  const int b = blockIdx.y, c0 = blockIdx.x * GMB_CH;
  const int cc = (C - c0 < GMB_CH) ? C - c0 : GMB_CH;
  for (int e = threadIdx.x; e < S * GMB_CH; e += 256) {
    const int sI = e / GMB_CH, c = e % GMB_CH;
    const bool in = c < cc;
    const int64_t o = ((int64_t)b * S + sI) * C + c0 + c;
    s_arg[sI][c] = in ? arg[o] : -1;
    s_g[sI][c] = in ? g[o] : 0.f;
  }
  __syncthreads();
  for (int c = wv; c < cc; c += 4) {
    int j = lane < S ? s_arg[lane][c] : -1;
    if (j >= N) j = -1;
    const float gv = lane < S ? s_g[lane][c] : 0.f;
    if (j >= 0) tag[j] = 0x7fffffff;
    __builtin_amdgcn_wave_barrier();
    if (j >= 0) atomicMin(&tag[j], lane);
    __builtin_amdgcn_wave_barrier();
    const int leader = j >= 0 ? tag[j] : lane;
    unsigned long long dup = __ballot(leader != lane);
    float acc = gv;
    while (dup) {
      const int i = __builtin_ctzll(dup);
      dup &= dup - 1;
      const int li = __builtin_amdgcn_readlane(leader, i);
      const float gi = __int_as_float(__builtin_amdgcn_readlane(__float_as_int(gv), i));
      acc = (lane == li) ? acc + gi : acc;
    }
    if (j >= 0 && leader == lane) dfeat[((int64_t)b * N + j) * ldf + c0 + c] = acc;
    __builtin_amdgcn_wave_barrier();
  }
}

}

extern "C" int sug_gather_rows(const float* feat, int64_t ldf, const int32_t* idx, int B, int N, int S,
                               int C, float* out, int64_t ldo, void* stream) {
  SUG_REQUIRE(feat && idx && out, "sug_gather_rows: null pointer");
  SUG_REQUIRE(B > 0 && N > 0 && S > 0 && C > 0 && ldf >= C && ldo >= C, "sug_gather_rows: bad shape");
  const int64_t total = (int64_t)B * S * C;
  hipLaunchKernelGGL(gather_rows_kernel, dim3(ew_grid(total)), dim3(256), 0, (hipStream_t)stream, feat,
                     ldf, idx, N, S, C, total, out, ldo);
  SUG_LAUNCH_CHECK("sug_gather_rows");
  return SUG_OK;
}

extern "C" int sug_scatter_add_rows(const float* g, int64_t ldg, const int32_t* idx, int B, int N,
                                    int S, int C, float* dfeat, int64_t ldf, void* stream) {
  SUG_REQUIRE(g && idx && dfeat, "sug_scatter_add_rows: null pointer");
  SUG_REQUIRE(B > 0 && N > 0 && S > 0 && C > 0 && ldf >= C && ldg >= C, "sug_scatter_add_rows: bad shape");
  const int64_t total = (int64_t)B * S * C;
  hipLaunchKernelGGL(scatter_add_rows_kernel, dim3(ew_grid(total)), dim3(256), 0, (hipStream_t)stream,
                     g, ldg, idx, N, S, C, total, dfeat, ldf);
  SUG_LAUNCH_CHECK("sug_scatter_add_rows");
  return SUG_OK;
}

extern "C" int64_t sug_scatter_rows_workspace(int B, int N, int S) { return (int64_t)B * (N + 1) + (int64_t)B * S; }

size_t sug_reverse_lists_lds_bytes(int B, int E, int N, int* ranges);

extern "C" int sug_scatter_rows_ordered_supported(int B, int N, int S) {
  return (B > 0 && N > 0 && S > 0 && sug_reverse_lists_lds_bytes(B, S, N, nullptr) <= 160 * 1024) ? 1 : 0;
}

extern "C" int sug_scatter_rows_ordered(const float* g, int64_t ldg, const int32_t* idx, int B, int N, int S, int C,
                                        float* dfeat, int64_t ldf, int32_t* ws, void* stream) {
  SUG_REQUIRE(g && idx && dfeat && ws, "sug_scatter_rows_ordered: null pointer");
  SUG_REQUIRE(B > 0 && N > 0 && S > 0 && C > 0 && ldf >= C && ldg >= C, "sug_scatter_rows_ordered: bad shape");
  SUG_REQUIRE(sug_scatter_rows_ordered_supported(B, N, S), "sug_scatter_rows_ordered: %d entries per cloud do not fit the LDS-resident "
              "reverse-list build (use sug_scatter_add_rows)", S);
  int32_t* rev_off = ws;
  int32_t* rev_ent = ws + (int64_t)B * (N + 1);
  hipStream_t st = (hipStream_t)stream;
  if (int rc = sug_reverse_lists(idx, B, S, N, 1, rev_off, rev_ent, st)) return rc;
  const bool v4 = C % 4 == 0 && ldg % 4 == 0 && ((uintptr_t)g % 16) == 0;
  const int64_t total = (int64_t)B * N * (v4 ? C / 4 : C);
  if (v4)
    hipLaunchKernelGGL((gather_sum_rows_kernel<4>), dim3(ew_grid(total)), dim3(256), 0, st, g, ldg, rev_off, rev_ent, N, S, C, total,
                       dfeat, ldf);
  else
    hipLaunchKernelGGL((gather_sum_rows_kernel<1>), dim3(ew_grid(total)), dim3(256), 0, st, g, ldg, rev_off, rev_ent, N, S, C, total,
                       dfeat, ldf);
  SUG_LAUNCH_CHECK("sug_scatter_rows_ordered");
  return SUG_OK;
}

extern "C" int sug_group_max(const float* feat, int64_t ldf, const int32_t* idx, int B, int N, int S,
                             int ns, int C, float* out, int32_t* arg, void* stream) {
  SUG_REQUIRE(feat && idx && out && arg, "sug_group_max: null pointer");
  SUG_REQUIRE(B > 0 && N > 0 && S > 0 && ns > 0 && C > 0 && ldf >= C, "sug_group_max: bad shape");
  const int64_t total = (int64_t)B * S * C;
  hipLaunchKernelGGL(group_max_kernel, dim3(ew_grid(total)), dim3(256), 0, (hipStream_t)stream, feat,
                     ldf, idx, N, S, ns, C, total, out, arg);
  SUG_LAUNCH_CHECK("sug_group_max");
  return SUG_OK;
}

extern "C" int sug_group_max_bwd(const float* g, const int32_t* arg, int B, int N, int S, int C,
                                 float* dfeat, int64_t ldf, void* stream) {
  SUG_REQUIRE(g && arg && dfeat, "sug_group_max_bwd: null pointer");
  SUG_REQUIRE(B > 0 && N > 0 && S > 0 && C > 0 && ldf >= C, "sug_group_max_bwd: bad shape");
  const int64_t total = (int64_t)B * S * C;
  static const int unordered = getenv("SUG_GROUP_MAX_UNORDERED") ? atoi(getenv("SUG_GROUP_MAX_UNORDERED")) : 0;
  const size_t sh = ((size_t)2 * 64 * (GMB_CH + 1) + (size_t)4 * N) * sizeof(int);
  bool ordered = S <= 64 && B <= 65535 && sh <= 150 * 1024 && !unordered;
  if (ordered && sh > 64 * 1024) {
    static SugLdsOptIn note;
    if (int rc = sug_allow_dynamic_lds(note, &group_max_bwd_ordered_kernel, 150 * 1024, "sug_group_max_bwd")) return rc;
  }
  if (ordered) {
    hipLaunchKernelGGL(group_max_bwd_ordered_kernel, dim3(sug_divup(C, GMB_CH), B), dim3(256), sh, (hipStream_t)stream, g, arg, N, S, C,
                       dfeat, ldf);
    SUG_LAUNCH_CHECK("sug_group_max_bwd");
    return SUG_OK;
  }
  hipLaunchKernelGGL(group_max_bwd_kernel, dim3(ew_grid(total)), dim3(256), 0, (hipStream_t)stream, g,
                     arg, N, S, C, total, dfeat, ldf);
  SUG_LAUNCH_CHECK("sug_group_max_bwd");
  return SUG_OK;
}

extern "C" int sug_copy_rows2d(const float* src, int64_t lds, float* dst, int64_t ldd, int64_t rows, int C, void* stream) {
  SUG_REQUIRE(src && dst && rows > 0 && C > 0 && C % 4 == 0 && lds >= C && ldd >= C && lds % 4 == 0 && ldd % 4 == 0,
              "sug_copy_rows2d: bad shape rows=%lld C=%d lds=%lld ldd=%lld", (long long)rows, C, (long long)lds, (long long)ldd);
  SUG_REQUIRE(((uintptr_t)src % 16) == 0 && ((uintptr_t)dst % 16) == 0, "sug_copy_rows2d: operands must be 16-byte aligned");
  const int64_t total = rows * (C / 4);
  const int grid = (int)(total / 256 + 1 < 8192 ? total / 256 + 1 : 8192);
  hipLaunchKernelGGL(copy_rows2d_kernel, dim3(grid), dim3(256), 0, (hipStream_t)stream, src, lds, dst, ldd, rows, C / 4);
  SUG_LAUNCH_CHECK("sug_copy_rows2d");
  return SUG_OK;
}
```

sug_amd/model/Model.py:

```python
import weakref

import torch
import torch.nn as nn
import torch.nn.functional as F

from .. import ops
from .model_utils import conv_2d, fc_layer, transform_net, adapt_layer_off, _bn_rows, bn_module, edge_wcats
from . import model_utils as _mu
from .pointnet2_utils import PointNetSetAbstraction
from . import PTran_utils
from .Ptran_transformer import TransformerBlock

K = 20


class _PrefixEntry:

    def __init__(self, tensors, extra=None, source=None, live=None, provider=None):
        self.tensors, self.extra = tensors, extra
        self._live, self.provider = live, provider
        self._source = weakref.ref(source) if source is not None else None
        self._flag = flag = [True]
        last = tensors[-1]
        if last.requires_grad:
            last.register_hook(lambda grad, f=flag: f.__setitem__(0, False))

    @property
    def alive(self):
        return self._flag[0]

    def __deepcopy__(self, memo):
        return _dead_prefix_entry()

    def __reduce__(self):
        return (_dead_prefix_entry, ())

    def servable(self):
        return self._flag[0] and self._source is not None and self._source() is not None and (self._live is None or self._live())

    def serves(self, x):
        return self._flag[0] and self._source is not None and self._source() is x and (self._live is None or self._live())


class _PrefixSharing:

    def _prefix_params(self):
        raise NotImplementedError

    def _prefix_key(self, x):
        ver = sum(p._version for p in self._prefix_params())
        return (x.data_ptr(), x._version, tuple(x.shape), torch.is_grad_enabled(), ver, ops.CTX.bn_groups)

    def find_prefix(self, x):
        hit = self._prefix_cache.get(self._prefix_key(x))
        return hit if (hit is not None and hit.serves(x)) else None

    def last_prefix(self, x):
        return self._prefix_cache.get(self._prefix_key(x))

    def _prune_prefix_cache(self):
        if len(self._prefix_cache) >= 4:
            self._prefix_cache = {k: e for k, e in self._prefix_cache.items() if e.servable()}
            if len(self._prefix_cache) >= 8:
                self._prefix_cache.clear()

    def install_prefix(self, x, tensors, extra, live=None, provider=None):
        self._prune_prefix_cache()
        e = self._prefix_cache[self._prefix_key(x)] = _PrefixEntry(tuple(tensors), extra, source=x, live=live, provider=provider)
        return e

    def clear_prefix_cache(self):
        self._prefix_cache = {}


def _dead_prefix_entry():
    e = _PrefixEntry.__new__(_PrefixEntry)
    e.tensors, e.extra, e._source, e._flag, e._live, e.provider = (), None, None, [False], None, None
    return e


def _sharing_on(flag, training):
    return bool(flag) and training


class CALayer(nn.Module):

    def __init__(self, channel, reduction=8):
        super(CALayer, self).__init__()
        self.conv_du = nn.Sequential(
            nn.Conv2d(channel, channel // reduction, 1, padding=0, bias=True),
            nn.ReLU(inplace=False),
            nn.Conv2d(channel // reduction, channel, 1, padding=0, bias=True),
            nn.Sigmoid())
        self.bn = nn.BatchNorm1d(4096)

    def forward(self, x):
        v = x.reshape(x.shape[0], -1)
        if ops.calayer_supported((self,), v):
            return ops.calayers((self,), v)
        c0, c2 = self.conv_du[0], self.conv_du[2]
        y = F.relu(F.linear(v, c0.weight.view(c0.weight.shape[0], -1), c0.bias))
        z = F.linear(y, c2.weight.view(c2.weight.shape[0], -1), c2.bias)
        if ops.gate_bn_supported(v, self.bn):
            return ops.gate_bn(v, z, self.bn)
        return self.bn(ops.gate(v, z))


class GradReverse(torch.autograd.Function):

    @staticmethod
    def forward(ctx, x):
        return x.view_as(x)

    @staticmethod
    def backward(ctx, g):
        return g


def grad_reverse(x, lambd=1.0):
    return x.view_as(x)


class DGCNN(nn.Module, _PrefixSharing):

    def __init__(self):
        super(DGCNN, self).__init__()
        self.k = K
        self.input_transform_net = transform_net(6, 3)
        self.conv1 = conv_2d(6, 64, kernel=1, bias=False, activation='leakyrelu')
        self.conv2 = conv_2d(64 * 2, 64, kernel=1, bias=False, activation='leakyrelu')
        self.conv3 = conv_2d(64 * 2, 128, kernel=1, bias=False, activation='leakyrelu')
        self.conv4 = conv_2d(128 * 2, 256, kernel=1, bias=False, activation='leakyrelu')
        self.bn5 = nn.BatchNorm1d(512)
        self.conv5 = nn.Conv1d(64 + 64 + 128 + 256, 512, kernel_size=1, bias=False)
        self.node_fea_adapt = adapt_layer_off()
        self.conv1d = nn.Conv1d(128, 64, 1)
        self.dim_redu = nn.MaxPool1d(3, stride=16)
        self.share_prefix = 'auto'
        self._prefix_cache = {}

    def _prefix_params(self):
        return [p for m in (self.conv1, self.conv2) for p in m.parameters()]

    def _prefix(self, x, loc, nb, out1=None, wc=(None, None)):
        if not _sharing_on(self.share_prefix, self.training):
            x1 = self.conv1.edge_rows(loc, nb(loc, 0), out=out1, wcat=wc[0])
            return x1, self.conv2.edge_rows(x1, nb(x1, 1), wcat=wc[1])
        key = self._prefix_key(x)
        hit = self._prefix_cache.get(key)
        if hit is not None and hit.serves(x):
            x1, x2 = hit.tensors
            st1, st2 = hit.extra
            ops.replay_bn_stats([(self.conv1.conv[1], st1), (self.conv2.conv[1], st2)])
            return x1, x2
        x1, st1 = self.conv1.edge_rows(loc, nb(loc, 0), return_stats=True, out=out1, wcat=wc[0])
        x2, st2 = self.conv2.edge_rows(x1, nb(x1, 1), return_stats=True, wcat=wc[1])
        self._prune_prefix_cache()
        self._prefix_cache[key] = _PrefixEntry((x1, x2), (st1, st2), source=x)
        return x1, x2

    def plan_geometry(self, x, passes, groups=1):
        return self.node_fea_adapt.plan_geometry(ops.cloud_rows(x), passes, groups)

    def forward(self, x, node=False, knn_idx=None, feat_grad=True):
        B, N = x.size(0), x.size(2)
        loc = ops.cloud_rows(x)
        gi = knn_idx or [None] * 4
        if knn_idx is not None:
            self._prefix_cache = {}
        nb = lambda f, i: gi[i] if gi[i] is not None else ops.knn(f, self.k)
        cat_in = torch.empty(B, N, 512, dtype=torch.float32, device=x.device)
        wc = edge_wcats((self.conv1, self.conv2, self.conv3, self.conv4))
        x1, x2 = self._prefix(x, loc, nb, out1=cat_in[:, :, 0:64], wc=wc[:2])
        x_, node_fea, _ = self.node_fea_adapt.rows(x2, loc)
        with torch.set_grad_enabled(torch.is_grad_enabled() and feat_grad):
            x2 = ops.linear_rows(x_, self.conv1d.weight.squeeze(-1), self.conv1d.bias)
            x3 = self.conv3.edge_rows(x2, nb(x2, 2), out=cat_in[:, :, 128:256], wcat=wc[2])
            x4 = self.conv4.edge_rows(x3, nb(x3, 3), out=cat_in[:, :, 256:512], wcat=wc[3])
            x5 = ops.linear_rows(ops.assemble_rows(cat_in, (x1, x2, x3, x4)), self.conv5.weight.squeeze(-1))
            if feat_grad:
                feat = ops.bn_act_pool_cat(x5, self.bn5, 0.2)
            else:
                ops.bn_update_stats(x5, self.bn5)
                feat = None
        node_fea = node_fea.transpose(1, 2).unsqueeze(-1)
        if node:
            return feat, node_fea, None
        return feat, node_fea


class Pointnet2_g(nn.Module):

    def __init__(self, normal_channel=False):
        super(Pointnet2_g, self).__init__()
        in_channel = 6 if normal_channel else 3
        self.normal_channel = normal_channel
        self.num_class = 10
        self.sa1 = PointNetSetAbstraction(512, 0.2, 32, in_channel, [64, 64, 128], False)
        self.sa2 = PointNetSetAbstraction(128, 0.4, 64, 128 + 3, [128, 128, 256], False)
        self.sa3 = PointNetSetAbstraction(None, None, None, 256 + 3, [256, 512, 1024], True)
        self.channel_redu = nn.Conv2d(512, 64, 1)
        self.dim_redu = nn.MaxPool1d(3, stride=8)

    def fps_plan(self, N):
        return [N, self.sa1.npoint]

    def can_plan_geometry(self):
        return not (self.normal_channel or self.sa1.group_all or self.sa2.group_all) and \
            all(sa.takes_index_path() for sa in (self.sa1, self.sa2))

    def plan_geometry(self, xyz, passes, groups=1):
        if self.normal_channel or self.sa1.group_all or self.sa2.group_all:
            return None
        if not all(sa.takes_index_path() for sa in (self.sa1, self.sa2)):
            return None
        loc = ops.cloud_rows(xyz)[:, :, :3].contiguous()
        B, N = loc.shape[0], loc.shape[1]
        S1, S2 = self.sa1.npoint, self.sa2.npoint
        st1, st2 = [], []
        dev = loc.device
        for _ in range(passes):
            if groups == 1:
                st1.append(ops.draw_start(B, N))
                st2.append(ops.draw_start(B, S1))
            else:
                d = [[ops.draw_group_start(B // groups, n) for n in (N, S1)] for _ in range(groups)]
                st1.append(torch.cat([d[g][0].to(device=dev, dtype=torch.int32, non_blocking=True) for g in range(groups)]))
                st2.append(torch.cat([d[g][1].to(device=dev, dtype=torch.int32, non_blocking=True) for g in range(groups)]))
        cat_starts = lambda sts: torch.cat([t.to(device=dev, dtype=torch.int32, non_blocking=True) for t in sts])
        locp = loc.repeat(passes, 1, 1) if passes > 1 else loc
        f1 = ops.fps(locp, S1, cat_starts(st1))
        nx1 = ops.gather_rows(locp, f1)
        i1 = ops.ball_query(locp, nx1, self.sa1.radius, self.sa1.nsample)
        f2 = ops.fps(nx1, S2, cat_starts(st2))
        nx2 = ops.gather_rows(nx1, f2)
        i2 = ops.ball_query(nx1, nx2, self.sa2.radius, self.sa2.nsample)
        return [[(nx1[p * B:(p + 1) * B], i1[p * B:(p + 1) * B]), (nx2[p * B:(p + 1) * B], i2[p * B:(p + 1) * B])]
                for p in range(passes)]

    def forward(self, xyz, node=False, feat_grad=True, need_node=True):
        rows = ops.cloud_rows(xyz)
        B = rows.shape[0]
        norm = rows[:, :, 3:].contiguous() if self.normal_channel else None
        loc = rows[:, :, :3].contiguous()
        if not need_node:
            l1_xyz, l1_pts = self.sa1.rows(loc, norm)
            with torch.set_grad_enabled(torch.is_grad_enabled() and feat_grad):
                l2_xyz, l2_pts = self.sa2.rows(l1_xyz, l1_pts)
                _, l3_pts = self.sa3.rows(l2_xyz, l2_pts)
            feat = l3_pts.reshape(B, 1024)
            return (feat, None, None) if node else (feat, None)
        l1_xyz, l1_pts, node_fea = self.sa1.rows(loc, norm, adapt=True, tail_grad=feat_grad)
        with torch.set_grad_enabled(torch.is_grad_enabled() and feat_grad):
            l2_xyz, l2_pts = self.sa2.rows(l1_xyz, l1_pts)
            _, l3_pts = self.sa3.rows(l2_xyz, l2_pts)
        feat = l3_pts.reshape(B, 1024)
        node_fea = self.dim_redu(node_fea.transpose(1, 2)).reshape(B, 64, 64, 1)
        if node:
            return feat, node_fea, None
        return feat, node_fea


class Pointnet_g(nn.Module, _PrefixSharing):

    def __init__(self):
        super(Pointnet_g, self).__init__()
        self.trans_net1 = transform_net(3, 3)
        self.trans_net2 = transform_net(64, 64)
        self.conv1 = conv_2d(3, 64, 1)
        self.conv2 = conv_2d(64, 64, 1)
        self.conv3 = adapt_layer_off()
        self.conv4 = conv_2d(128, 128, 1)
        self.conv5 = conv_2d(128, 1024, 1)
        self.bn1 = nn.BatchNorm1d(1024)
        self.share_prefix = 'auto'
        self._prefix_cache = {}

    def _prefix_modules(self):
        return (self.trans_net1, self.conv1, self.conv2, self.trans_net2)

    def _prefix_params(self):
        return [p for mod in self._prefix_modules() for p in mod.parameters()]

    def _prefix(self, x, loc):
        def run():
            y = torch.bmm(loc, self.trans_net1.rows(loc))
            y = self.conv2.rows(self.conv1.rows(y))
            return torch.bmm(y, self.trans_net2.rows(y))
        if not (_sharing_on(self.share_prefix, self.training) and x.is_cuda):
            return run()
        key = self._prefix_key(x)
        hit = self._prefix_cache.get(key)
        if hit is not None and hit.serves(x):
            ops.replay_bn_stats(hit.extra)
            return hit.tensors[0]
        with ops.record_bn_stats() as rec:
            y = run()
        self._prune_prefix_cache()
        self._prefix_cache[key] = _PrefixEntry((y,), rec, source=x)
        return y

    def plan_geometry(self, x, passes, groups=1):
        return self.conv3.plan_geometry(ops.cloud_rows(x), passes, groups)

    def forward(self, x, node=False, feat_grad=True):
        loc = ops.cloud_rows(x)
        y = self._prefix(x, loc)
        y, node_fea, node_off = self.conv3.rows(y, loc)
        with torch.set_grad_enabled(torch.is_grad_enabled() and feat_grad):
            y = self.conv5.rows_max_after(self.conv4, y)
            bn = self.bn1
            if y.is_cuda and y.dtype == torch.float32 and _mu.OWN_BN(bn) and bn.track_running_stats and bn.momentum is not None \
                    and bn.affine:
                y = ops.bn_act_rows(y, bn, 1.0)
            else:
                y = bn_module(bn, y)
        node_fea = node_fea.transpose(1, 2).unsqueeze(-1)
        node_off = node_off.transpose(1, 2)
        if node:
            return y, node_fea, node_off
        return y, node_fea


class TransitionDown(nn.Module):

    def __init__(self, k, nneighbor, channels):
        super().__init__()
        self.sa = PTran_utils.PointNetSetAbstraction(k, 0, nneighbor, channels[0], channels[1:], group_all=False,
                                                     knn=True)

    def forward(self, xyz, points):
        return self.sa(xyz, points)


class PTran_g(nn.Module, _PrefixSharing):

    def __init__(self):
        super(PTran_g, self).__init__()
        npoints, nblocks, nneighbor, d_points = 1024, 4, 16, 3
        transformer_dim = 512
        self.fc1 = nn.Sequential(nn.Linear(d_points, 32), nn.ReLU(), nn.Linear(32, 32))
        self.transformer1 = TransformerBlock(32, transformer_dim, nneighbor)
        self.transition_downs = nn.ModuleList()
        self.transformers = nn.ModuleList()
        for i in range(nblocks):
            channel = 32 * 2 ** (i + 1)
            self.transition_downs.append(TransitionDown(npoints // 4 ** (i + 1), nneighbor,
                                                        [channel // 2 + 3, channel, channel]))
            self.transformers.append(TransformerBlock(channel, transformer_dim, nneighbor))
        self.nblocks = nblocks
        self.npoints = npoints
        self.conv1d = nn.Conv1d(64, 64, 1, stride=2)
        self.share_prefix = 'auto'
        self._prefix_cache = {}

    def _prefix_params(self):
        return [p for m in (self.fc1, self.transformer1) for p in m.parameters()]

    def _prefix_key(self, x):
        ver = sum(p._version for p in self._prefix_params())
        return (x.data_ptr(), x._version, tuple(x.shape), torch.is_grad_enabled(), ver)

    def _lift(self, x_):
        h = F.relu(ops.linear_rows(x_, self.fc1[0].weight, self.fc1[0].bias))
        return ops.linear_rows(h, self.fc1[2].weight, self.fc1[2].bias)

    def _prefix(self, x, x_, xyz):
        if not _sharing_on(self.share_prefix, self.training):
            return self.transformer1(xyz, self._lift(x_))[0]
        key = self._prefix_key(x)
        hit = self._prefix_cache.get(key)
        if hit is None or not hit.serves(x):
            self._prune_prefix_cache()
            hit = self._prefix_cache[key] = _PrefixEntry((self.transformer1(xyz, self._lift(x_))[0],), source=x)
        return hit.tensors[0]

    def fps_plan(self, N):
        return [N] + [self.npoints // 4 ** (i + 1) for i in range(self.nblocks - 1)]

    def forward(self, x, node=False, feat_grad=True):
        x_ = ops.cloud_rows(x)
        xyz = x_[..., :3]
        points = self._prefix(x, x_, xyz)
        xyz_and_feats = [(xyz, points)]
        for i in range(self.nblocks):
            with torch.set_grad_enabled(torch.is_grad_enabled() and (feat_grad or i < 2)):
                xyz, points = self.transition_downs[i](xyz, points)
                points = self.transformers[i](xyz, points)[0]
            xyz_and_feats.append((xyz, points))
        nf = xyz_and_feats[2][1]
        node_features = torch.matmul(self.conv1d.weight.squeeze(-1), nf[:, :, ::2]) + self.conv1d.bias.view(1, -1, 1)
        points = points.mean(1)
        if node:
            return points, node_features, None
        return points, node_features


class Pointnet_c(nn.Module):

    def __init__(self, num_class=10, dgcnn_flag=False, PTran_flag=False):
        super(Pointnet_c, self).__init__()
        activate, bias = ('leakyrelu', True) if dgcnn_flag else ('relu', False)
        self.mlp1 = fc_layer(1024, 512, bn=True, activation=activate, bias=bias)
        self.dropout1 = nn.Dropout2d(p=0.4)
        self.mlp2 = fc_layer(512, 256, bn=True, activation=activate, bias=True)
        self.dropout2 = nn.Dropout2d(p=0.4)
        self.mlp3 = nn.Linear(256, num_class)
        self.PTran = PTran_flag

    @staticmethod
    def _drop(layer, x):
        if x.dim() == 2:
            return F.dropout(x, layer.p, layer.training)
        return layer(x)

    def forward(self, x, adapt=False):
        if not self.PTran:
            x = self._drop(self.dropout1, self.mlp1(x))
        x = self.mlp2(x)
        mid_feature = x
        x = self.mlp3(self._drop(self.dropout2, x))
        if adapt:
            return x, mid_feature
        return x


class KPConv_g(nn.Module):
    graph_capturable = False
    level_caps = None
    samples_fps = False

    def __init__(self, config=None):
        super(KPConv_g, self).__init__()
        from .KPConv_model import KPFEncoder, PreprocessorGPU, GlobalAverageBlock, KPConvConfig
        from .KPConv_blocks import sample_tensor_slices
        self.config = KPConvConfig if config is None else config
        self.sample_tensor_slices = sample_tensor_slices
        self.preprocessor = PreprocessorGPU(self.config)
        self.encoder = KPFEncoder(self.config)
        self.global_avg_pooling = GlobalAverageBlock()
        self.deform_fitting_power = self.config.deform_fitting_power

    def set_level_caps(self, caps):
        from .KPConv_model import LevelCaps
        LevelCaps.set_level_caps(self, caps)

    def capacity_report(self, reset=False):
        return self.preprocessor.capacity_report(reset)

    def forward(self, x, node=False, feat_grad=True):
        from .KPConv_model import _split_clouds
        pts, lengths = _split_clouds(x)
        kpconv_meta = self.preprocessor.forward_packed(pts, lengths)
        feats0 = kpconv_meta["points"][0][:, 0:1]
        feats = self.encoder(feats0, kpconv_meta)
        if kpconv_meta.get('capacity', False):
            nodes = ops.kp_sample_rows(feats[2], kpconv_meta["offsets"][1])
        else:
            nodes = self.sample_tensor_slices(feats[2], kpconv_meta["lengths"][1])
        feats = self.global_avg_pooling(feats[0], kpconv_meta["offsets"][-1], kpconv_meta.get('capacity', False))
        if node:
            return feats, nodes, None
        return feats, nodes


class KPConv_c(nn.Module):

    def __init__(self, num_class=10, dgcnn_flag=False, PTran_flag=False):
        super(KPConv_c, self).__init__()
        self.mlp1 = nn.Linear(1024, 256)
        self.mlp2 = nn.Linear(256, 64)
        self.mlp3 = nn.Linear(64, num_class)
        self.act = nn.ReLU()

    def forward(self, x, adapt=False):
        x = self.mlp1(x)
        mid_feature = x
# ... 218 lines not shown
```

sug_amd/model/model_utils.py:

```python
import torch
import torch.nn as nn
import torch.nn.functional as F

from .. import ops
from . import point_utils

_ACT_SLOPE = {'relu': 0.0, 'leakyrelu': 0.01}


def OWN_BN(bn):
    return True


def bn_module(bn, y):
    if ops.CTX.bn_groups == 1:
        return bn(y)
    return torch.cat([bn(c) for c in y.chunk(ops.CTX.bn_groups, dim=0)], dim=0)


def _bn_rows(bn, y):
    if ops.CTX.bn_groups > 1:
        G = ops.CTX.bn_groups
        with ops.bn_groups(1):
            return torch.cat([_bn_rows(bn, c) for c in y.chunk(G, dim=0)], dim=0)
    shp = y.shape
    y2 = y.reshape(-1, shp[-1])
    if bn.training and bn.track_running_stats and bn.num_batches_tracked is not None:
        bn.num_batches_tracked.add_(1)
    y2 = F.batch_norm(y2, bn.running_mean, bn.running_var, bn.weight, bn.bias,
                      bn.training or not bn.track_running_stats, bn.momentum, bn.eps)
    return y2.view(shp)


def edge_wcats(layers):
    grad = torch.is_grad_enabled()
    out, miss = [None] * len(layers), []
    for i, l in enumerate(layers):
        W = l.weight2d()
        hit = l._wcat if l.cache_weight_split else None
        if hit is not None and hit[0] == W._version and (hit[1] or not grad):
            out[i] = hit[2]
        else:
            miss.append((i, l, W))
    if miss:
        for (i, l, W), wc in zip(miss, ops.edge_weight_split_multi([W for _, _, W in miss])):
            out[i] = wc
            l._wcat = (W._version, grad, wc) if l.cache_weight_split else None
    return out


class conv_2d(nn.Module):

    def __init__(self, in_ch, out_ch, kernel, activation='relu', bias=True):
        super(conv_2d, self).__init__()
        assert kernel == 1 or kernel == (1, 1), 'the hot path only has 1x1 convolutions'
        act = {'relu': nn.ReLU(inplace=False), 'tanh': nn.Tanh(), 'leakyrelu': nn.LeakyReLU()}[activation]
        self.conv = nn.Sequential(nn.Conv2d(in_ch, out_ch, kernel_size=kernel, bias=bias),
                                  nn.BatchNorm2d(out_ch), act)
        self.activation = activation
        self.cache_weight_split = False
        self._wcat = None

    def weight2d(self):
        w = self.conv[0].weight
        return w.view(w.shape[0], w.shape[1])

    def rows(self, x):
        y = ops.linear_rows(x, self.weight2d(), self.conv[0].bias)
        if self.activation in _ACT_SLOPE and OWN_BN(self.conv[1]):
            return ops.bn_act_rows(y, self.conv[1], _ACT_SLOPE[self.activation])
        return self.conv[2](_bn_rows(self.conv[1], y))

    def forward(self, x):
        return self.rows(x.permute(0, 2, 3, 1)).permute(0, 3, 1, 2)

    def rows_max_after(self, prev, x):
        B, N, _ = x.shape
        Wp, W = prev.weight2d(), self.weight2d()
        if ops.SA_MID_FUSED and x.is_cuda and self.activation in _ACT_SLOPE and prev.activation in _ACT_SLOPE and \
                OWN_BN(self.conv[1]) and OWN_BN(prev.conv[1]) and prev.conv[1].training == self.conv[1].training and \
                ops.pointmlp_max_supported(Wp.shape[0], W.shape[0], N):
            y = ops.linear_rows(x, Wp, prev.conv[0].bias)
            return ops.bn_act_pointmlp_max(y, prev.conv[1], _ACT_SLOPE[prev.activation], W, self.conv[0].bias, self.conv[1],
                                           _ACT_SLOPE[self.activation], N)[0]
        return self.rows_max(prev.rows(x))

    def rows_max(self, x):
        B, N, C = x.shape
        W = self.weight2d()
        if self.activation in _ACT_SLOPE and OWN_BN(self.conv[1]) and ops.pointmlp_max_supported(C, W.shape[0], N):
            return ops.pointmlp_max(x, W, self.conv[0].bias, self.conv[1], _ACT_SLOPE[self.activation], N)
        return torch.max(self.rows(x), dim=1)[0]

    def edge_rows(self, x, idx, return_stats=False, out=None, wcat=None):
        assert self.activation in _ACT_SLOPE
        B, N, C = x.shape
        W = self.weight2d()
        assert W.shape[1] == 2 * C
        Wcat = wcat if wcat is not None else edge_wcats((self,))[0]
        bias = self.conv[0].bias
        bn = self.conv[1]
        ops._count_bn_call(bn)
        if ops.edgeconv_fused_supported(N, idx.shape[2], C, W.shape[0]):
            out, coef = ops.edgeconv_fused(x, Wcat, bias, idx, bn.weight, bn.bias, bn.running_mean, bn.running_var,
                                           bn.training, _ACT_SLOPE[self.activation], bn.eps, bn.momentum, out=out)
            return (out, coef) if return_stats else out
        pq = ops.linear_rows(x.reshape(B * N, C), Wcat)
        if bias is not None:
            pq = pq + torch.cat((torch.zeros_like(bias), bias))
        out, coef = ops.edgeconv_bn_act_max(pq.view(B, N, -1), idx, bn.weight, bn.bias, bn.running_mean,
                                            bn.running_var, bn.training, _ACT_SLOPE[self.activation],
                                            bn.eps, bn.momentum, out=out)
        return (out, coef) if return_stats else out

    def replay_bn_update(self, coef):
        ops.bn_replay(self.conv[1], coef)


class fc_layer(nn.Module):

    def __init__(self, in_ch, out_ch, bn=True, activation='leakyrelu', bias=False):
        super(fc_layer, self).__init__()
        self.ac = nn.ReLU(inplace=False) if activation == 'relu' else nn.LeakyReLU(negative_slope=0.2, inplace=False)
        layers = [nn.Linear(in_ch, out_ch, bias=bias)]
        if bn:
            layers.append(nn.LayerNorm(out_ch))
        layers.append(self.ac)
        self.fc = nn.Sequential(*layers)

    def forward(self, x):
        if ops.CTX.fused_heads and len(self.fc) == 3 and x.is_cuda and ops.ln_act_supported(x, self.fc[1]):
            slope = 0.0 if isinstance(self.ac, nn.ReLU) else self.ac.negative_slope
            return ops.ln_act(self.fc[0](x), self.fc[1], slope)
        return self.fc(x)


class transform_net(nn.Module):

    def __init__(self, in_ch, K=3):
        super(transform_net, self).__init__()
        self.K = K
        self.conv2d1 = conv_2d(in_ch, 64, 1)
        self.conv2d2 = conv_2d(64, 128, 1)
        self.conv2d3 = conv_2d(128, 1024, 1)
        self.maxpool1 = nn.MaxPool2d(kernel_size=(512, 1))
        self.fc1 = fc_layer(1024, 512)
        self.fc2 = fc_layer(512, 256)
        self.fc3 = nn.Linear(256, K * K)

    def rows(self, x):
        y = self.conv2d3.rows_max_after(self.conv2d2, self.conv2d1.rows(x))
        y = self.fc3(self.fc2(self.fc1(y)))
        y = y + torch.eye(self.K, device=y.device, dtype=y.dtype).view(1, self.K * self.K)
        return y.view(-1, self.K, self.K)

    def forward(self, x, DGCNN_Flag=False):
        if DGCNN_Flag:
            y = self.conv2d2(self.conv2d1(x)).max(dim=-1, keepdim=True)[0]
            return self.rows_tail(y.squeeze(-1).transpose(1, 2))
        return self.rows(x.squeeze(-1).transpose(1, 2))

    def rows_tail(self, y):
        y = self.conv2d3.rows_max(y)
        y = self.fc3(self.fc2(self.fc1(y)))
        y = y + torch.eye(self.K, device=y.device, dtype=y.dtype).view(1, self.K * self.K)
        return y.view(-1, self.K, self.K)


class adapt_layer_off(nn.Module):

    def __init__(self, num_node=64, offset_dim=3, trans_dim_in=64, trans_dim_out=64, fc_dim=64):
        super(adapt_layer_off, self).__init__()
        self.num_node = num_node
        self.offset_dim = offset_dim
        self.trans = conv_2d(trans_dim_in, trans_dim_out, 1)
        self.pred_offset = nn.Sequential(
            nn.Conv2d(trans_dim_out, offset_dim, kernel_size=1, bias=False),
            nn.Tanh())
        self.residual = conv_2d(trans_dim_in, fc_dim, 1)

    def rows(self, fea, loc):
        B, N, _ = loc.shape
        S = self.num_node
        plan = ops.CTX.geometry_plan
        if plan:
            fidx, f_loc, gidx = plan.pop(0)
            if fidx.shape != (B, S) or gidx.shape[:2] != (B, S):
                raise RuntimeError('geometry plan does not match the SA-node module')
        else:
            start = ops.draw_start(B, N)
            fidx = ops.fps(loc, S, start)
            f_loc = ops.gather_rows(loc, fidx)
            gidx = ops.ball_query(loc, f_loc, 0.3, 64)
        w_off = self.pred_offset[0].weight.view(self.offset_dim, -1)
        proj = ops.linear_rows(fea, w_off)
        if self.offset_dim == 3 and gidx.shape[2] == S:
            node_off, n_loc = ops.node_offset(proj, loc, fidx, gidx)
        else:
            sem = torch.tanh(ops.gather_rows(proj, gidx) - ops.gather_rows(proj, fidx).unsqueeze(2))
            g_loc = ops.gather_rows(loc, gidx) - f_loc.unsqueeze(2)
            node_off = (sem * g_loc).mean(dim=2)
            n_loc = f_loc + node_off
        gidx2 = ops.knn_query(loc, n_loc, 64)
        res = self.residual.rows(fea)
        node_fea = ops.group_max(res, gidx2)
        if fea.shape[2] % 4 == 0 and node_fea.shape[2] % 4 == 0:
            out = ops.interp3_cat(fea, node_fea, loc, n_loc)
        else:
            out = torch.cat((fea, point_utils.interpolate_rows(loc, n_loc, node_fea, 3)), dim=2)
        return out, node_fea, node_off

    def plan_geometry(self, loc, passes, groups=1):
        B, N, _ = loc.shape
        S = self.num_node
        starts = []
        for _ in range(passes):
            if ops.CTX.start_provider is not None or groups == 1:
                starts.append(ops.draw_start(B, N))
            else:
                starts.append(torch.cat([torch.randint(0, N, (B // groups,), dtype=torch.long) for _ in range(groups)]))
        dev = loc.device
        st = torch.cat([t.to(device=dev, dtype=torch.int32, non_blocking=True) for t in starts])
        locp = loc.repeat(passes, 1, 1) if passes > 1 else loc
        fidx = ops.fps(locp, S, st)
        f_loc = ops.gather_rows(locp, fidx)
        gidx = ops.ball_query(locp, f_loc, 0.3, 64)
        return [[(fidx[p * B:(p + 1) * B], f_loc[p * B:(p + 1) * B], gidx[p * B:(p + 1) * B])] for p in range(passes)]

    def forward(self, input_fea, input_loc):
        out, node_fea, node_off = self.rows(input_fea.squeeze(-1).transpose(1, 2).contiguous(),
                                            input_loc.transpose(1, 2).contiguous())
        return (out.transpose(1, 2).unsqueeze(3), node_fea.transpose(1, 2).unsqueeze(3),
                node_off.transpose(1, 2))


class focal_loss(nn.Module):

    def __init__(self, alpha=None, gamma=2, num_classes=3, size_average=True):
        super(focal_loss, self).__init__()
        self.size_average = size_average
        if isinstance(alpha, list):
            assert len(alpha) == num_classes
            self.alpha = torch.Tensor(alpha)
        else:
            self.alpha = torch.Tensor([1 / num_classes] * num_classes)
        self.gamma = gamma

    def forward(self, preds, labels):
        preds = preds.view(-1, preds.size(-1))
        logp = F.log_softmax(preds, dim=1).gather(1, labels.view(-1, 1)).view(-1)
        alpha = self.alpha.to(preds.device).gather(0, labels.view(-1))
        loss = alpha * (-(1 - torch.exp(logp)) ** self.gamma * logp)
        return loss.mean() if self.size_average else loss.sum()


def knn(x, k):
    return ops.knn(x.transpose(1, 2), k).long()


def get_graph_feature(x, k=20, idx=None):
    B, N = x.size(0), x.size(2)
    rows = x.reshape(B, -1, N).transpose(1, 2).contiguous()
    if idx is None:
        idx = ops.knn(rows, k)
    nbr = ops.gather_rows(rows, idx)
    ctr = rows.unsqueeze(2).expand_as(nbr)
    return torch.cat((nbr - ctr, ctr), dim=3).permute(0, 3, 1, 2)
```

sug_amd/ops.py:

```python
import contextlib
import ctypes
import math
import os as _os

import torch

from ._lib import lib, check, STATS_BLOCKS, CONSTANTS as _H

class StepContext:
    __slots__ = ('bn_groups', 'start_queue', 'start_provider', 'geometry_plan', 'profile', 'profile_only', 'parallel_branches',
                 'fused_heads', 'w16_cache', 'bn_record', 'pending_counts')

    def __init__(self):
        self.bn_groups = 1
        self.start_queue = self.start_provider = self.geometry_plan = None
        self.profile = self.profile_only = None
        self.parallel_branches = False
        self.fused_heads = False
        self.w16_cache = self.bn_record = self.pending_counts = None

    @contextlib.contextmanager
    def scoped(self, **fields):
        old = {k: getattr(self, k) for k in fields}
        for k, v in fields.items():
# ... 22 lines not shown
        return [f() for f in fns]
    main = torch.cuda.current_stream()
    dev = main.device_index
    sides = []
    for i in range(1, len(fns)):
        st = _SIDE_STREAMS.get((dev, i))
        if st is None:
            st = _SIDE_STREAMS[(dev, i)] = torch.cuda.Stream(device=dev)
        st.wait_stream(main)
        sides.append(st)
    outs = [fns[0]()]
    for f, st in zip(fns[1:], sides):
        with torch.cuda.stream(st):
            outs.append(f())
    for st in sides:
        main.wait_stream(st)
    return outs


@contextlib.contextmanager
def capture_guard():
    import gc
    clear_rows_cache()
    was = gc.isenabled()
    gc.disable()
    try:
        yield
    finally:
        if was:
            gc.enable()


def bn_groups(g):
    return CTX.scoped(bn_groups=int(g))


def start_queue(q):
    return CTX.scoped(start_queue=list(q) if q is not None else None)


def draw_start(B, N):
    if CTX.start_queue:
        t = CTX.start_queue.pop(0)
        if t.numel() != B:
            raise RuntimeError('FPS start plan does not match the encoder (%d starts for %d clouds)' % (t.numel(), B))
        return t
    if CTX.start_provider is not None:
        return CTX.start_provider(B, N)
    G = CTX.bn_groups
    if G > 1 and B % G == 0:
        return torch.cat([torch.randint(0, N, (B // G,), dtype=torch.long) for _ in range(G)])
    return torch.randint(0, N, (B,), dtype=torch.long)


def draw_group_start(B, N):
    if CTX.start_provider is not None:
        return CTX.start_provider(B, N)
    return torch.randint(0, N, (B,), dtype=torch.long)


def _timed(name, shape, call):
    if CTX.profile is None or (CTX.profile_only is not None and not name.startswith(tuple(CTX.profile_only))):
        return call()
    if torch.cuda.is_current_stream_capturing():
        return call()
    a = torch.cuda.Event(enable_timing=True)
    b = torch.cuda.Event(enable_timing=True)
    a.record()
    r = call()
    b.record()
    CTX.profile.setdefault(name, []).append((a, b, shape))
    return r


def _p(t):
    return ctypes.c_void_p(t.data_ptr()) if t is not None else None


def _st():
    return ctypes.c_void_p(torch._C._cuda_getCurrentRawStream(torch.cuda.current_device()))


def _need_gpu(*ts):
    for t in ts:
        if t is not None and not t.is_cuda:
            raise RuntimeError('sug_amd ops run on a HIP device only (got a %s tensor); '
                               'there is no CPU fallback' % t.device)


def _rows3(t):
    assert t.dim() == 3 and t.dtype == torch.float32
    B, N, C = t.shape
    if t.stride(2) != 1 or t.stride(0) != N * t.stride(1) or t.stride(1) < C:
        t = t.contiguous()
    return t, B, N, C, t.stride(1)


def _i32(t):
    return t if t.dtype == torch.int32 else t.to(torch.int32)


def knn(x, k):
    _need_gpu(x)
    x, B, N, C, ld = _rows3(x.detach())
    idx = torch.empty(B, N, k, dtype=torch.int32, device=x.device)
    check(_timed('knn_C%d' % C, {'B': B, 'N': N, 'C': C, 'k': k},
                 lambda: lib().sug_knn(_p(x), ld, B, N, C, k, _p(idx), _st())), 'sug_knn')
    return idx


def knn_reverse(idx):
    _need_gpu(idx)
    idx = _i32(idx).contiguous()
    B, N, k = idx.shape
    off = torch.empty(B, N + 1, dtype=torch.int32, device=idx.device)
    ent = torch.empty(B, N * k, dtype=torch.int32, device=idx.device)
    check(lib().sug_knn_reverse(_p(idx), B, N, k, _p(off), _p(ent), _st()), 'sug_knn_reverse')
    return off, ent


def fps(xyz, npoint, start):
    _need_gpu(xyz)
    xyz = xyz.detach().contiguous()
    B, N, _ = xyz.shape
    start = start.to(device=xyz.device, dtype=torch.int32, non_blocking=True)
    out = torch.empty(B, npoint, dtype=torch.int32, device=xyz.device)
    check(lib().sug_fps(_p(xyz), _p(start), B, N, npoint, _p(out), _st()), 'sug_fps')
    return out


def ball_query(xyz, query, radius, nsample):
    _need_gpu(xyz, query)
    xyz, query = xyz.detach().contiguous(), query.detach().contiguous()
    B, N, _ = xyz.shape
    S = query.shape[1]
    r2 = float(torch.tensor(radius ** 2, dtype=torch.float32))
    out = torch.empty(B, S, nsample, dtype=torch.int32, device=xyz.device)
    check(lib().sug_ball_query(_p(xyz), _p(query), B, N, S, r2, nsample, _p(out), _st()), 'sug_ball_query')
    return out


def knn_query(xyz, query, k, want_dist=False, direct=False):
    _need_gpu(xyz, query)
    xyz, query = xyz.detach().contiguous(), query.detach().contiguous()
    B, N, _ = xyz.shape
    S = query.shape[1]
    idx = torch.empty(B, S, k, dtype=torch.int32, device=xyz.device)
    dist = torch.empty(B, S, k, dtype=torch.float32, device=xyz.device) if want_dist else None
    fn = lib().sug_knn_query_direct if direct else lib().sug_knn_query
    check(fn(_p(xyz), _p(query), B, N, S, k, _p(idx), _p(dist), _st()), 'sug_knn_query')
    return (idx, dist) if want_dist else idx


def ball_query_multi(xyz, query, radii, nsamples):
    _need_gpu(xyz, query)
    xyz, query = xyz.detach().contiguous(), query.detach().contiguous()
    B, N, _ = xyz.shape
    S = query.shape[1]
    R = len(radii)
    if R != len(nsamples) or not 1 <= R <= 4:
        raise RuntimeError('ball_query_multi: need 1..4 radii and as many list lengths (got %d / %d)' % (R, len(nsamples)))
    outs = [torch.empty(B, S, int(ns), dtype=torch.int32, device=xyz.device) for ns in nsamples]
    r2 = (ctypes.c_float * R)(*[float(torch.tensor(r ** 2, dtype=torch.float32)) for r in radii])
    ns = (ctypes.c_int32 * R)(*[int(n) for n in nsamples])
    check(lib().sug_ball_query_multi(_p(xyz), _p(query), B, N, S, R, r2, ns, _ptrs(outs), _st()), 'sug_ball_query_multi')
    return outs


def three_nn_raw(query, cand, direct=False):
    _need_gpu(query, cand)
    query, cand = query.detach().contiguous(), cand.detach().contiguous()
    B, N, _ = query.shape
    S = cand.shape[1]
    idx = torch.empty(B, N, 3, dtype=torch.int32, device=query.device)
    dist = torch.empty(B, N, 3, dtype=torch.float32, device=query.device)
    if direct:
        check(lib().sug_three_nn_direct(_p(query), _p(cand), B, N, S, _p(idx), _p(dist), _st()), 'sug_three_nn_direct')
    else:
        check(lib().sug_three_nn(_p(query), _p(cand), B, N, S, _p(idx), _p(dist), _st()), 'sug_three_nn')
    return idx, dist


class _FPInterp(torch.autograd.Function):

    @staticmethod
    def forward(ctx, points1, src, idx3, d3):
        _need_gpu(points1, src, idx3, d3)
        src, B, S, D2, lds = _rows3(src)
        N = idx3.shape[1]
        D1 = 0 if points1 is None else points1.shape[2]
        out = torch.empty(B, N, D1 + D2, dtype=torch.float32, device=src.device)
        if D1:
            out[:, :, :D1].copy_(points1)
        w3 = torch.empty(B, N, 3, dtype=torch.float32, device=src.device)
        dst = ctypes.c_void_p(out.data_ptr() + 4 * D1)
        check(lib().sug_fp_interp_fwd(_p(src), lds, _p(idx3), _p(d3), B, N, S, D2, dst, D1 + D2, _p(w3), _st()),
              'sug_fp_interp_fwd')
        ctx.save_for_backward(idx3, w3)
        ctx.meta = (B, N, S, D1, D2)
        return out

    @staticmethod
    def backward(ctx, g):
        idx3, w3 = ctx.saved_tensors
        B, N, S, D1, D2 = ctx.meta
        g = g.contiguous()
        dsrc = None
        if ctx.needs_input_grad[1]:
            dsrc = torch.empty(B, S, D2, dtype=torch.float32, device=g.device)
            off = torch.empty(B, S + 1, dtype=torch.int32, device=g.device)
            ent = torch.empty(B, 3 * N, dtype=torch.int32, device=g.device)
            gs = ctypes.c_void_p(g.data_ptr() + 4 * D1)
            check(lib().sug_fp_interp_bwd(gs, D1 + D2, _p(idx3), _p(w3), B, N, S, D2, _p(off), _p(ent), _p(dsrc), D2, _st()),
                  'sug_fp_interp_bwd')
        return (g[:, :, :D1] if D1 and ctx.needs_input_grad[0] else None), dsrc, None, None


def fp_interp(xyz1, xyz2, points1, points2, direct=False):
    _need_gpu(xyz1, xyz2, points1, points2)
    if xyz1.requires_grad or xyz2.requires_grad:
        raise RuntimeError('fp_interp: no gradient flows to the coordinates (xyz1 / xyz2 require grad); the interpolation '
                           'weights are treated as constants -- pass detached coordinates')
    B, N, _ = xyz1.shape
    S = xyz2.shape[1]
    if S == 1:
        interp = points2.expand(B, N, points2.shape[2])
        return interp.contiguous() if points1 is None else torch.cat([points1, interp], dim=-1)
    if S == 2:
        raise RuntimeError('feature propagation needs S == 1 or S >= 3 coarse points: with S = 2 the reference itself fails '
                           '(three neighbours are taken of two candidates)')
    idx3, d3 = three_nn_raw(xyz1, xyz2, direct=direct)
    return _FPInterp.apply(points1, points2, idx3, d3)


class _ThreeNN(torch.autograd.Function):

    @staticmethod
    def forward(ctx, query, cand):
        idx, dist = three_nn_raw(query, cand)
        ctx.save_for_backward(query, cand, idx)
        ctx.mark_non_differentiable(idx)
        return idx, dist

    @staticmethod
    def backward(ctx, _gidx, gdist):
        query, cand, idx = ctx.saved_tensors
        B, N, _ = query.shape
        S = cand.shape[1]
        li = idx.long().view(B, N * 3)
        sel = torch.gather(cand, 1, li.unsqueeze(-1).expand(B, N * 3, 3)).view(B, N, 3, 3)
        g = (2.0 * gdist).unsqueeze(-1) * (sel - query.unsqueeze(2))
        gc = torch.zeros(B, S, 3, device=cand.device, dtype=cand.dtype)
        gc.scatter_add_(1, li.unsqueeze(-1).expand(B, N * 3, 3), g.view(B, N * 3, 3))
        return None, gc


def three_nn(query, cand):
    return _ThreeNN.apply(query, cand)


SCATTER_ORDERED = _os.environ.get('SUG_SCATTER_ORDERED', '1') != '0'


class _GatherRows(torch.autograd.Function):
    @staticmethod
    def forward(ctx, feat, idx):
        _need_gpu(feat, idx)
        feat_c, B, N, C, ld = _rows3(feat)
        idx2 = _i32(idx).reshape(B, -1).contiguous()
        S = idx2.shape[1]
        out = torch.empty(B, S, C, dtype=torch.float32, device=feat.device)
        check(lib().sug_gather_rows(_p(feat_c), ld, _p(idx2), B, N, S, C, _p(out), C, _st()), 'sug_gather_rows')
        ctx.save_for_backward(idx2)
        ctx.shape = (B, N, C)
        return out.view(*idx.shape, C)

    @staticmethod
    def backward(ctx, g):
        (idx2,) = ctx.saved_tensors
        B, N, C = ctx.shape
        S = idx2.shape[1]
        g = g.reshape(B, S, C).contiguous()
        L = lib()
        if SCATTER_ORDERED and L.sug_scatter_rows_ordered_supported(B, N, S):
            d = torch.empty(B, N, C, dtype=torch.float32, device=g.device)
            ws = torch.empty(L.sug_scatter_rows_workspace(B, N, S), dtype=torch.int32, device=g.device)
            check(L.sug_scatter_rows_ordered(_p(g), C, _p(idx2), B, N, S, C, _p(d), C, _p(ws), _st()), 'sug_scatter_rows_ordered')
            return d, None
        d = torch.zeros(B, N, C, dtype=torch.float32, device=g.device)
        check(L.sug_scatter_add_rows(_p(g), C, _p(idx2), B, N, S, C, _p(d), C, _st()), 'sug_scatter_add_rows')
        return d, None


def reverse_lists_fit(B, N, E):
    return bool(lib().sug_scatter_rows_ordered_supported(B, N, E))


def gather_rows(feat, idx):
    return _GatherRows.apply(feat, idx)


class _GroupMax(torch.autograd.Function):
    @staticmethod
    def forward(ctx, feat, idx):
        _need_gpu(feat, idx)
        feat_c, B, N, C, ld = _rows3(feat)
        idx = _i32(idx).contiguous()
        S, ns = idx.shape[1], idx.shape[2]
        out = torch.empty(B, S, C, dtype=torch.float32, device=feat.device)
        arg = torch.empty(B, S, C, dtype=torch.int32, device=feat.device)
        check(lib().sug_group_max(_p(feat_c), ld, _p(idx), B, N, S, ns, C, _p(out), _p(arg), _st()), 'sug_group_max')
        ctx.save_for_backward(arg)
        ctx.shape = (B, N, C)
        return out

    @staticmethod
    def backward(ctx, g):
        (arg,) = ctx.saved_tensors
        B, N, C = ctx.shape
        S = arg.shape[1]
        g = g.contiguous()
        d = torch.zeros(B, N, C, dtype=torch.float32, device=g.device)
        check(lib().sug_group_max_bwd(_p(g), _p(arg), B, N, S, C, _p(d), C, _st()), 'sug_group_max_bwd')
        return d, None


def group_max(feat, idx):
    return _GroupMax.apply(feat, idx)


DW_LIBRARY_SHAPES = set()
DW_FORCE_LIBRARY = False
DW_SHAPE_LOG = None
OWN_ROWS_GEMM = _os.environ.get('SUG_OWN_ROWS_GEMM', '0') == '1'


class _LinearRows(torch.autograd.Function):

    @staticmethod
    def forward(ctx, x, weight, bias):
        M, N = weight.shape
        x2 = x.reshape(-1, N)
        if OWN_ROWS_GEMM and N in (64, 128) and M % 128 == 0 and x2.shape[0] >= 4096 and x2.stride(1) == 1 \
                and x2.stride(0) % 4 == 0 and x2.data_ptr() % 16 == 0 and weight.is_contiguous():
            y = torch.empty(x2.shape[0], M, dtype=torch.float32, device=x.device)
            check(_timed('rows_gemm_K%d_Co%d' % (N, M), {'B': x2.shape[0], 'N': 1, 'k': N, 'Co': M},
                         lambda: lib().sug_rows_gemm(_p(x2), x2.stride(0), x2.shape[0], N, _p(weight.detach()),
                                                     _p(None if bias is None else bias.detach()), M, _p(y), M, _st())),
                  'sug_rows_gemm')
            y = y.view(*x.shape[:-1], M)
        else:
            y = torch.nn.functional.linear(x, weight, bias)
        ctx.save_for_backward(x, weight)
        ctx.has_bias = bias is not None
        return y

    @staticmethod
    def backward(ctx, g):
        x, weight = ctx.saved_tensors
        M, N = weight.shape
        dx, dw, db = linear_rows_backward(x.reshape(-1, N), weight, g.reshape(-1, M), ctx.needs_input_grad[0],
                                          ctx.needs_input_grad[1], ctx.has_bias and ctx.needs_input_grad[2])
        return (None if dx is None else dx.view(x.shape)), dw, db


DW_BMM = _os.environ.get('SUG_DW_BMM', '1') == '1'


def _dw_bmm_chunks(R, M, N, g2, x2):
    if not DW_BMM or M * N < 128 * 128 or min(M, N) < 64 or g2.stride(0) != M or x2.stride(0) != N or \
            g2.stride(1) != 1 or x2.stride(1) != 1:
        return 0
    S = 64
    while S > 8 and R // S < 4096:
        S //= 2
    return S if (R % S == 0 and R // S >= 1024) else 0


def linear_rows_backward(x2, weight, g2, need_dx, need_dw, need_db):
    M, N = weight.shape
    if g2.stride(1) != 1:
        g2 = g2.contiguous()
    if x2.stride(1) != 1:
        x2 = x2.contiguous()
    R = g2.shape[0]
    dx = dw = db = None
    if need_dx:
        dx = g2 @ weight
    if need_dw:
        if DW_SHAPE_LOG is not None:
            DW_SHAPE_LOG.append((R, M, N))
        lib_ok = DW_FORCE_LIBRARY or ((R, M, N) in DW_LIBRARY_SHAPES and not torch.cuda.is_current_stream_capturing())
        S = _dw_bmm_chunks(R, M, N, g2, x2) if not need_db else 0
        if M * N > 512 * 512 or lib_ok:
            dw = g2.t() @ x2
        elif S:
            import torch.cuda.tunable as _tn
            tuned = _tn.is_enabled()
            if tuned:
                _tn.enable(False)
            try:
                part = torch.bmm(g2.view(S, R // S, M).transpose(1, 2), x2.view(S, R // S, N))
            finally:
                if tuned:
                    _tn.enable(True)
            dw = torch.empty(M, N, dtype=torch.float32, device=g2.device)
            check(lib().sug_linear_dw_fold(_p(part), S, M * N, _p(dw), _st()), 'sug_linear_dw_fold')
        else:
            dw = torch.empty(M, N, dtype=torch.float32, device=g2.device)
            ws = torch.empty(int(lib().sug_linear_dw_workspace(R, M, N)), dtype=torch.float32, device=g2.device)
            if need_db:
                db = torch.empty(M, dtype=torch.float32, device=g2.device)
            check(lib().sug_linear_dw_bias(_p(g2), g2.stride(0), _p(x2), x2.stride(0), R, M, N, _p(dw), _p(db), _p(ws),
                                           _st()), 'sug_linear_dw_bias')
    if need_db and db is None:
        db = colsum(g2)
    return dx, dw, db


def linear_rows(x, weight, bias=None):
    _need_gpu(x, weight)
    if x.dtype != torch.float32:
        raise RuntimeError('sug_amd.ops.linear_rows: fp32 rows only (got %s)' % x.dtype)
    return _LinearRows.apply(x, weight, bias)


class _NodeOffset(torch.autograd.Function):

    @staticmethod
    def forward(ctx, proj, loc, fidx, gidx):
        _need_gpu(proj, loc, fidx, gidx)
        proj, loc = proj.contiguous(), loc.detach().contiguous()
        fidx, gidx = _i32(fidx).contiguous(), _i32(gidx).contiguous()
        B, N, _ = proj.shape
        S, ns = gidx.shape[1], gidx.shape[2]
        off = torch.empty(B, S, 3, dtype=torch.float32, device=proj.device)
        nloc = torch.empty(B, S, 3, dtype=torch.float32, device=proj.device)
        check(lib().sug_node_offset_fwd(_p(proj), _p(loc), _p(fidx), _p(gidx), B, N, S, ns, _p(off), _p(nloc), _st()),
              'sug_node_offset_fwd')
        ctx.save_for_backward(proj, loc, fidx, gidx)
        ctx.set_materialize_grads(False)
        return off, nloc

    @staticmethod
    def backward(ctx, goff, gnloc):
        proj, loc, fidx, gidx = ctx.saved_tensors
        B, N, _ = proj.shape
        S, ns = gidx.shape[1], gidx.shape[2]
        if goff is None and gnloc is None:
            return None, None, None, None
        g = (goff if gnloc is None else gnloc if goff is None else goff + gnloc).contiguous()
        dproj = torch.empty_like(proj)
        check(lib().sug_node_offset_bwd(_p(proj), _p(loc), _p(fidx), _p(gidx), _p(g), B, N, S, ns, _p(dproj), _st()),
              'sug_node_offset_bwd')
        return dproj, None, None, None


def node_offset(proj, loc, fidx, gidx):
    return _NodeOffset.apply(proj, loc, fidx, gidx)


class _Interp3Cat(torch.autograd.Function):

    @staticmethod
    def forward(ctx, fea, node, xyz, nloc):
        _need_gpu(fea, node, xyz, nloc)
        fea, B, N, C1, ldf = _rows3(fea)
        node = node.contiguous()
        xyz, nlocd = xyz.detach().contiguous(), nloc.detach().contiguous()
        S, C2 = node.shape[1], node.shape[2]
        idx3, d3 = three_nn_raw(xyz, nlocd)
        out = torch.empty(B, N, C1 + C2, dtype=torch.float32, device=fea.device)
        check(lib().sug_interp3_cat_fwd(_p(fea) if C1 else None, ldf if C1 else 0, C1, _p(node), _p(idx3), _p(d3), B, N, S,
                                        C2, _p(out), C1 + C2, _st()), 'sug_interp3_cat_fwd')
        ctx.save_for_backward(node, idx3, d3, xyz, nlocd)
        ctx.meta = (B, N, S, C1, C2)
        return out

    @staticmethod
    def backward(ctx, g):
        node, idx3, d3, xyz, nloc = ctx.saved_tensors
        B, N, S, C1, C2 = ctx.meta
        g = g.contiguous()
        L = lib()
        if L.sug_interp3_cat_bwd_lists_supported(B, N, S):
            dnode = torch.empty_like(node)
            dnloc = torch.empty_like(nloc)
            off = torch.empty(B, S + 1, dtype=torch.int32, device=g.device)
            ent = torch.empty(B, 3 * N, dtype=torch.int32, device=g.device)
            ddw = torch.empty(B, N, 6, dtype=torch.float32, device=g.device)
            check(L.sug_interp3_cat_bwd_lists(_p(g), C1 + C2, C1, _p(node), _p(idx3), _p(d3), _p(xyz), _p(nloc), B, N, S,
                                              C2, _p(off), _p(ent), _p(ddw), _p(dnode), _p(dnloc), _st()),
                  'sug_interp3_cat_bwd_lists')
        else:
            dnode = torch.zeros_like(node)
            dnloc = torch.zeros_like(nloc)
            check(L.sug_interp3_cat_bwd(_p(g), C1 + C2, C1, _p(node), _p(idx3), _p(d3), _p(xyz), _p(nloc), B, N, S, C2,
                                        _p(dnode), _p(dnloc), _st()), 'sug_interp3_cat_bwd')
        return g[:, :, :C1], dnode, None, dnloc


def interp3_cat(fea, node, xyz, nloc):
    return _Interp3Cat.apply(fea, node, xyz, nloc)


def bn_coef(stats, gamma, beta, count, eps, momentum, running_mean, running_var, out=None):
    C = gamma.numel()
    coef = torch.empty(5, C, dtype=torch.float32, device=gamma.device) if out is None else out
    check(lib().sug_bn_finalize(_p(stats), _p(gamma), _p(beta), C, float(count), eps, momentum,
                                _p(running_mean), _p(running_var), _p(coef), _st()), 'sug_bn_finalize')
    return coef


def eval_coef(gamma, beta, running_mean, running_var, eps):
    rstd = torch.rsqrt(running_var + eps)
    scale = gamma * rstd
    return torch.stack([scale, beta - running_mean * scale, running_mean, rstd, running_var]).contiguous()


class _BNState:
    __slots__ = ('mean', 'var', 'training', 'train', 'eps', 'momentum', 'G')

    def __init__(self, running_mean, running_var, training, eps, momentum):
        self.mean, self.var = running_mean, running_var
        self.training = bool(training)
        self.train = 1 if training else 0
        self.eps, self.momentum, self.G = eps, momentum, CTX.bn_groups


def _bn_state(bn):
    return _BNState(bn.running_mean, bn.running_var, bn.training, bn.eps, bn.momentum)


def _bn_params(gamma, beta, st, C):
    g, b = gamma.detach().contiguous(), beta.detach().contiguous()
    coef = torch.empty(st.G, 5, C, dtype=torch.float32, device=g.device)
    if not st.training:
        coef.copy_(eval_coef(g, b, st.mean, st.var, st.eps))
    return g, b, coef


def _stats_ws(C, dev):
    return torch.empty(STATS_BLOCKS * 2 * C, dtype=torch.float32, device=dev)


def _check_groups(op, n, what, G, seg=None):
    if seg is None and n % G:
        raise RuntimeError('%s: %d %s do not split into %d domain groups' % (op, n, what, G))
    if seg is not None and n % (G * seg):
        raise RuntimeError('%s: %d %s do not split into %d groups of %d-row segments' % (op, n, what, G, seg))


def _dgamma_dbeta(rf):
    C = rf.numel() // 2
    return rf[C:], rf[:C]


def affine_act(z, coef, slope, out=None):
    _need_gpu(z)
    C = z.shape[-1]
    z2 = z.reshape(-1, C)
    if z2.stride(1) != 1:
        z2 = z2.contiguous()
    rows = z2.shape[0]
    if out is None:
        out = torch.empty(rows, C, dtype=torch.float32, device=z.device)
    o2 = out.view(-1, C) if out.is_contiguous() else out
    check(lib().sug_affine_act(_p(z2), z2.stride(0), _p(coef), rows, C, float(slope), _p(o2), o2.stride(0), _st()),
          'sug_affine_act')
    return out.view(*z.shape)


def col_stats(y2, ws=None):
    rows, C = y2.shape
    stats = torch.empty(2 * C, dtype=torch.float64, device=y2.device)
    if ws is None:
        ws = _stats_ws(C, y2.device)
    check(lib().sug_col_stats(_p(y2), y2.stride(0), rows, C, _p(stats), _p(ws), _st()), 'sug_col_stats')
    return stats


class _BNActRows(torch.autograd.Function):

    @staticmethod
    def forward(ctx, y, gamma, beta, st, slope):
        _need_gpu(y, gamma)
        C = y.shape[-1]
        y2 = y.reshape(-1, C)
        if y2.stride(1) != 1 or y2.stride(0) != C:
            y2 = y2.contiguous()
        rows = y2.shape[0]
        _check_groups('bn_act_rows', rows, 'rows', st.G)
        dev = y.device
        g, b, coef = _bn_params(gamma, beta, st, C)
        out = torch.empty(rows, C, dtype=torch.float32, device=dev)
        stats = torch.empty(2 * C, dtype=torch.float64, device=dev)
        ws = _stats_ws(C, dev)
        check(lib().sug_bn_act_rows_fwd(_p(y2), C, rows, C, st.G, _p(g), _p(b), st.train, st.eps, st.momentum,
                                        float(slope), _p(st.mean), _p(st.var), _p(coef), _p(out), C,
                                        _p(stats), _p(ws), _st()), 'sug_bn_act_rows_fwd')
        if any(ctx.needs_input_grad[i] for i in (0, 1, 2)):
            ctx.save_for_backward(y2, coef)
            ctx.meta = (rows, C, float(slope), st.training, tuple(y.shape), st.G)
        ctx.mark_non_differentiable(coef)
        ctx.set_materialize_grads(False)
        return out.view(y.shape), coef

    @staticmethod
    def backward(ctx, gout, _gcoef):
        y2, coef = ctx.saved_tensors
        rows, C, slope, training, shape, G = ctx.meta
        if gout is None:
            gout = torch.zeros_like(y2)
        dy, dgamma, dbeta = _bn_act_rows_backward(gout, y2, coef, rows, C, slope, training, G)
        return dy.view(shape), dgamma, dbeta, None, None


def _bn_act_rows_backward(gout, y2, coef, rows, C, slope, training, G):
    dev = gout.device
    g2 = gout.reshape(rows, C)
    if g2.stride(1) != 1:
        g2 = g2.contiguous()
    a = torch.empty(rows, C, dtype=torch.float32, device=dev)
    red = torch.empty(G, 2 * C, dtype=torch.float64, device=dev)
    ws = _stats_ws(C, dev)
    dy = torch.empty(rows, C, dtype=torch.float32, device=dev) if training else a
    rf = torch.empty(2 * C, dtype=torch.float32, device=dev)
    check(lib().sug_bn_act_rows_bwd(_p(g2), g2.stride(0), _p(y2), C, _p(coef), rows, C, G, int(training),
                                    slope, _p(a), _p(red), _p(dy), _p(ws), _p(rf), _st()), 'sug_bn_act_rows_bwd')
    return (dy,) + _dgamma_dbeta(rf)


class _SAFirstLayer(torch.autograd.Function):

    @staticmethod
    def forward(ctx, P, Q, idx, gamma, beta, st):
        _need_gpu(P, Q, idx)
        P, Q = P.contiguous(), Q.contiguous()
        idx = _i32(idx).contiguous()
        B, N, C = P.shape
        S, ns = idx.shape[1], idx.shape[2]
        _check_groups('sa_first_layer', B, 'clouds', st.G)
        dev = P.device
        g, b, coef = _bn_params(gamma, beta, st, C)
        Z = torch.empty(B, S, ns, C, dtype=torch.float32, device=dev)
        ws = _stats_ws(C, dev)
        check(lib().sug_sa_first_fwd(_p(P.detach()), C, _p(Q.detach()), _p(idx), B, N, S, ns, C, st.G, _p(g), _p(b),
                                     st.train, st.eps, st.momentum, _p(st.mean), _p(st.var), _p(coef),
                                     _p(Z), _p(ws), _st()), 'sug_sa_first_fwd')
        ctx.save_for_backward(P, Q, idx, coef)
        ctx.meta = (st.train, st.G)
        return Z

    @staticmethod
    def backward(ctx, gz):
        P, Q, idx, coef = ctx.saved_tensors
        train, G = ctx.meta
        B, N, C = P.shape
        S, ns = idx.shape[1], idx.shape[2]
        gz = gz.contiguous()
        bufs = _sa_first_bwd_buffers(B, N, S, ns, C, G, gz.device)
        check(lib().sug_sa_first_bwd(_p(gz), _p(P), C, _p(Q), _p(idx), B, N, S, ns, C, G, train, _p(coef),
                                     *map(_p, bufs), _st()), 'sug_sa_first_bwd')
        dP, dQ, rf = bufs[4], bufs[5], bufs[7]
        return (dP, dQ, None) + _dgamma_dbeta(rf) + (None,)


def _sa_first_bwd_buffers(B, N, S, ns, C, G, dev):
    f32 = dict(dtype=torch.float32, device=dev)
    return (torch.zeros(G + 1, 2 * C, dtype=torch.float64, device=dev),
            torch.empty(B, N + 1, dtype=torch.int32, device=dev), torch.empty(B, S * ns, dtype=torch.int32, device=dev),
            torch.empty(2, B, S, C, **f32), torch.empty(B, N, C, **f32), torch.empty(B, S, C, **f32),
            _stats_ws(C, dev), torch.empty(2 * C, **f32))


class _SAFirstLayerGeo(torch.autograd.Function):

    @staticmethod
    def forward(ctx, Pf, Px, Q, idx, xyz, cent, Wx, bias, gamma, beta, st):
        _need_gpu(Px, Q, idx, xyz)
        idx = _i32(idx).contiguous()
        B, N, C = Px.shape
        S, ns = idx.shape[1], idx.shape[2]
        _check_groups('sa_first_layer', B, 'clouds', st.G)
        dev = Px.device
        Pfc = None if Pf is None else Pf.detach().contiguous()
        xyz, cent = xyz.detach().contiguous(), cent.detach().contiguous()
        Wxc = Wx.detach().contiguous()
        bc = None if bias is None else bias.detach().contiguous()
        g, b, coef = _bn_params(gamma, beta, st, C)
        Z = torch.empty(B, S, ns, C, dtype=torch.float32, device=dev)
        ws = _stats_ws(C, dev)
        check(lib().sug_sa_first_geo_fwd(_p(Pfc), C, _p(xyz), _p(cent), _p(Wxc), 3, _p(bc), _p(idx), B, N, S, ns, C, st.G,
                                         _p(g), _p(b), st.train, st.eps, st.momentum, _p(st.mean), _p(st.var), _p(coef), _p(Z),
                                         _p(ws), _st()), 'sug_sa_first_geo_fwd')
        saved = [idx, coef, xyz, cent, Wxc] + ([Pfc] if Pfc is not None else []) + ([bc] if bc is not None else [])
        ctx.save_for_backward(*saved)
        ctx.meta = (st.train, st.G, Pfc is not None, bc is not None, N, C)
        return Z

    @staticmethod
    def backward(ctx, gz):
        train, G, has_p, has_b, N, C = ctx.meta
        sv = list(ctx.saved_tensors)
        idx, coef, xyz, cent, Wxc = sv[:5]
        Pfc = sv[5] if has_p else None
        bc = sv[5 + int(has_p)] if has_b else None
        B, S, ns = idx.shape
        gz = gz.contiguous()
        bufs = _sa_first_bwd_buffers(B, N, S, ns, C, G, gz.device)
        check(lib().sug_sa_first_geo_bwd(_p(gz), _p(Pfc), C, _p(xyz), _p(cent), _p(Wxc), 3, _p(bc), _p(idx), B, N, S, ns, C, G,
                                         train, _p(coef), *map(_p, bufs), _st()), 'sug_sa_first_geo_bwd')
        dP, dQ, rf = bufs[4], bufs[5], bufs[7]
        return ((dP if has_p else None), dP, dQ, None, None, None, None, None) + _dgamma_dbeta(rf) + (None,)


SA_FIRST_GEO = _os.environ.get('SUG_SA_FIRST_GEO', '0') == '1'


def sa_first_layer_geo(Pf, Px, Q, idx, xyz, cent, Wx, bias, bn):
    _count_bn_call(bn)
    return _SAFirstLayerGeo.apply(Pf, Px, Q, idx, xyz, cent, Wx, bias, bn.weight, bn.bias, _bn_state(bn))


SA_FIRST = _os.environ.get('SUG_SA_FIRST', '1') != '0'


def sa_first_layer_supported(C):
    return SA_FIRST and C in (64, 128)


def sa_first_layer(P, Q, idx, bn):
    _count_bn_call(bn)
    return _SAFirstLayer.apply(P, Q, idx, bn.weight, bn.bias, _bn_state(bn))


class _LNAct(torch.autograd.Function):

    @staticmethod
    def forward(ctx, x, gamma, beta, eps, slope):
        _need_gpu(x, gamma)
        x2 = x.reshape(-1, x.shape[-1]).contiguous()
        rows, C = x2.shape
        g, b = gamma.detach().contiguous(), beta.detach().contiguous()
        y = torch.empty_like(x2)
        stat = torch.empty(rows, 2, dtype=torch.float32, device=x.device)
        check(lib().sug_ln_act_fwd(_p(x2), _p(g), _p(b), rows, C, eps, float(slope), _p(y), _p(stat), _st()), 'sug_ln_act_fwd')
        ctx.save_for_backward(x2, g, b, stat)
        ctx.meta = (float(slope), tuple(x.shape))
        return y.view(x.shape)

    @staticmethod
    def backward(ctx, gy):
        x2, g, b, stat = ctx.saved_tensors
        slope, shape = ctx.meta
        rows, C = x2.shape
        gy = gy.reshape(rows, C).contiguous()
        dx, ws = torch.empty_like(x2), torch.empty_like(x2)
        dgb = torch.empty(2, C, dtype=torch.float32, device=x2.device)
        check(lib().sug_ln_act_bwd(_p(gy), _p(x2), _p(g), _p(b), _p(stat), rows, C, slope, _p(dx), _p(dgb[0]), _p(dgb[1]),
                                   _p(ws), _st()), 'sug_ln_act_bwd')
        return dx.view(shape), dgb[0], dgb[1], None, None




def ln_act_supported(x, ln):
    return x.is_cuda and x.dtype == torch.float32 and x.shape[-1] <= 1024 and ln.elementwise_affine and \
        len(ln.normalized_shape) == 1 and ln.weight is not None and ln.bias is not None


def ln_act(x, ln, slope):
    return _LNAct.apply(x, ln.weight, ln.bias, ln.eps, slope)


HEADS_FUSED = _os.environ.get('SUG_HEADS_FUSED', '1') != '0'


def _ptrs(ts):
    return (ctypes.c_void_p * len(ts))(*[None if t is None else t.data_ptr() for t in ts])


def heads_fused_supported(heads, x):
    if not (HEADS_FUSED and 1 <= len(heads) <= 2 and x.is_cuda and x.dtype == torch.float32 and x.dim() == 2):
        return False
    M, K = x.shape
    L = lib()
    h0 = heads[0]
    for hd in heads:
        if hd.PTran != h0.PTran or hd.training != h0.training or hd.dropout1.p != h0.dropout1.p or hd.dropout2.p != h0.dropout2.p:
            return False
        layers = ([] if hd.PTran else [hd.mlp1]) + [hd.mlp2]
        for fc in layers:
            if len(fc.fc) != 3 or not ln_act_supported(x, fc.fc[1]) or fc.fc[1].eps != h0.mlp2.fc[1].eps:
                return False
        if type(hd.mlp2.ac) is not type(h0.mlp2.ac) or (not hd.PTran and type(hd.mlp1.ac) is not type(hd.mlp2.ac)):
            return False
        for lin in [fc.fc[0] for fc in layers] + [hd.mlp3]:
            if lin.weight.dtype != torch.float32 or not lin.weight.is_cuda:
                return False
        if hd.mlp3.weight.shape != h0.mlp3.weight.shape or hd.mlp2.fc[0].weight.shape != h0.mlp2.fc[0].weight.shape:
            return False
    dims = [K] + ([] if h0.PTran else [h0.mlp1.fc[0].out_features]) + [h0.mlp2.fc[0].out_features, h0.mlp3.out_features]
    first = (h0.mlp2 if h0.PTran else h0.mlp1).fc[0]
    if first.in_features != K or h0.mlp3.in_features != dims[-2] or (not h0.PTran and h0.mlp2.fc[0].in_features != dims[1]):
        return False
    nl = len(dims) - 1
    for i in range(nl):
        pro, epi = int(i > 0), int(i < nl - 1)
        if not L.sug_head_linear_supported(M, dims[i], dims[i + 1], pro, epi):
            return False
    return True


class _HeadsFused(torch.autograd.Function):

    @staticmethod
    def forward(ctx, x, training, p1, p2, slope, eps, nheads, *params):
        _need_gpu(x)
        assert len(params) == 10 * nheads
        P = [[None if t is None else t.detach().contiguous() for t in params[10 * h:10 * h + 10]] for h in range(nheads)]
        three = P[0][0] is not None
        x2 = x.detach().contiguous()
        M, K = x2.shape
        dev = x.device
        N1 = P[0][0].shape[0] if three else 0
        N2, NC = P[0][4].shape[0], P[0][8].shape[0]
        drop1, drop2 = training and three and p1 > 0, training and p2 > 0
        u = torch.rand(nheads * M * (N1 + N2), dtype=torch.float32, device=dev) if (drop1 or drop2) else None
        u1 = [u[h * M * N1:(h + 1) * M * N1].view(M, N1) if drop1 else None for h in range(nheads)] if three else None
        o2 = nheads * M * N1
        u2 = [u[o2 + h * M * N2:o2 + (h + 1) * M * N2].view(M, N2) if drop2 else None for h in range(nheads)]
        H = range(nheads)
        L = lib()
        col = lambda i: [P[h][i] for h in H]
        new = lambda n: [torch.empty(M, n, dtype=torch.float32, device=dev) for _ in H]
        z1 = st1 = None
        if three:
            z1, st1 = new(N1), new(2)
            check(L.sug_head_linear_fwd(nheads, _ptrs([x2] * nheads), K, _ptrs(col(0)), _ptrs(col(1)), _ptrs(z1), None, None, None,
                                        None, None, M, K, N1, 0, slope, eps, 0.0, _st()), 'sug_head_linear_fwd')
        z2, st2, mid, logits = new(N2), new(2), new(N2), new(NC)
        if three:
            check(L.sug_head_linear_fwd(nheads, _ptrs(z1), N1, _ptrs(col(4)), _ptrs(col(5)), _ptrs(z2), _ptrs(col(2)), _ptrs(col(3)),
                                        _ptrs(u1), _ptrs(st1), None, M, N1, N2, 1, slope, eps, p1 if drop1 else 0.0, _st()),
                  'sug_head_linear_fwd')
        else:
            check(L.sug_head_linear_fwd(nheads, _ptrs([x2] * nheads), K, _ptrs(col(4)), _ptrs(col(5)), _ptrs(z2), None, None, None,
                                        None, None, M, K, N2, 0, slope, eps, 0.0, _st()), 'sug_head_linear_fwd')
        check(L.sug_head_linear_fwd(nheads, _ptrs(z2), N2, _ptrs(col(8)), _ptrs(col(9)), _ptrs(logits), _ptrs(col(6)), _ptrs(col(7)),
                                    _ptrs(u2), _ptrs(st2), _ptrs(mid), M, N2, NC, 1, slope, eps, p2 if drop2 else 0.0, _st()),
              'sug_head_linear_fwd')
        flatP = [t for h in H for t in P[h]]
        acts = []
        for h in H:
            acts += [z1[h] if three else None, st1[h] if three else None, z2[h], st2[h],
                     u1[h] if (three and u1 is not None) else None, u2[h]]
        ctx.save_for_backward(*flatP, *acts, x2)
        ctx.meta = (three, M, K, N1, N2, NC, float(slope), float(eps), float(p1 if drop1 else 0.0), float(p2 if drop2 else 0.0),
                    nheads, tuple(x.shape))
        ctx.need_dx = ctx.needs_input_grad[0]
        out = []
        for h in H:
            out += [logits[h], mid[h]]
        return tuple(out)

    @staticmethod
    def backward(ctx, *gs):
        three, M, K, N1, N2, NC, slope, eps, p1, p2, nheads, xshape = ctx.meta
        saved = ctx.saved_tensors
        H = range(nheads)
        P = [list(saved[10 * h:10 * h + 10]) for h in H]
        acts = saved[10 * nheads:10 * nheads + 6 * nheads]
        x2 = saved[-1]
        z1, st1, z2, st2, u1, u2 = ([acts[6 * h + i] for h in H] for i in range(6))
        dev = x2.device
        L = lib()
        col = lambda i: [P[h][i] for h in H]
        zeros = lambda n: torch.zeros(M, n, dtype=torch.float32, device=dev)
        gl = [gs[2 * h].contiguous() if gs[2 * h] is not None else zeros(NC) for h in H]
        gm = [None if gs[2 * h + 1] is None else gs[2 * h + 1].contiguous() for h in H]
        like = lambda i: [None if P[h][i] is None else torch.empty_like(P[h][i]) for h in H]
        new = lambda n: [torch.empty(M, n, dtype=torch.float32, device=dev) for _ in H]
        grads = [like(i) for i in range(10)]
        da2, dz2 = new(N2), new(N2)
        check(L.sug_head_linear_bwd(nheads, 0, _ptrs(gl), NC, _ptrs(z2), N2, _ptrs(st2), _ptrs(col(6)), _ptrs(col(7)), _ptrs(u2),
                                    _ptrs(col(8)), _ptrs(grads[8]), _ptrs(grads[9]), _ptrs(da2), N2, M, N2, NC, 1, slope, p2, _st()),
              'sug_head_linear_bwd')
        check(L.sug_head_ln_bwd(nheads, _ptrs(da2), N2, _ptrs(z2), _ptrs(st2), _ptrs(col(6)), _ptrs(col(7)), _ptrs(u2), _ptrs(gm),
                                _ptrs(dz2), _ptrs(grads[6]), _ptrs(grads[7]), _ptrs(grads[5]), M, N2, slope, p2, _st()), 'sug_head_ln_bwd')
        dx = torch.empty(M, K, dtype=torch.float32, device=dev) if ctx.need_dx else None
        dxs = _ptrs([dx] + [None] * (nheads - 1))
        if three:
            da1, dz1 = new(N1), new(N1)
            check(L.sug_head_linear_bwd(nheads, 0, _ptrs(dz2), N2, _ptrs(z1), N1, _ptrs(st1), _ptrs(col(2)), _ptrs(col(3)), _ptrs(u1),
                                        _ptrs(col(4)), _ptrs(grads[4]), None, _ptrs(da1), N1, M, N1, N2, 1, slope, p1, _st()),
                  'sug_head_linear_bwd')
            check(L.sug_head_ln_bwd(nheads, _ptrs(da1), N1, _ptrs(z1), _ptrs(st1), _ptrs(col(2)), _ptrs(col(3)), _ptrs(u1), None,
                                    _ptrs(dz1), _ptrs(grads[2]), _ptrs(grads[3]), _ptrs(grads[1]), M, N1, slope, p1, _st()),
                  'sug_head_ln_bwd')
            check(L.sug_head_linear_bwd(nheads, 1, _ptrs(dz1), N1, _ptrs([x2] * nheads), K, None, None, None, None, _ptrs(col(0)),
                                        _ptrs(grads[0]), None, dxs, K, M, K, N1, 0, slope, 0.0, _st()), 'sug_head_linear_bwd')
        else:
            check(L.sug_head_linear_bwd(nheads, 1, _ptrs(dz2), N2, _ptrs([x2] * nheads), K, None, None, None, None, _ptrs(col(4)),
                                        _ptrs(grads[4]), None, dxs, K, M, K, N2, 0, slope, 0.0, _st()), 'sug_head_linear_bwd')
        flat = []
        for h in H:
            flat += [grads[i][h] for i in range(10)]
        return (None if dx is None else dx.view(xshape), None, None, None, None, None, None) + tuple(flat)


def heads_fused(heads, x):
    h0 = heads[0]
    act = h0.mlp2.ac
    slope = 0.0 if isinstance(act, torch.nn.ReLU) else float(act.negative_slope)
    params = []
    for hd in heads:
        if hd.PTran:
            params += [None, None, None, None]
        else:
            params += [hd.mlp1.fc[0].weight, hd.mlp1.fc[0].bias, hd.mlp1.fc[1].weight, hd.mlp1.fc[1].bias]
        params += [hd.mlp2.fc[0].weight, hd.mlp2.fc[0].bias, hd.mlp2.fc[1].weight, hd.mlp2.fc[1].bias, hd.mlp3.weight, hd.mlp3.bias]
    out = _HeadsFused.apply(x, h0.training, float(h0.dropout1.p), float(h0.dropout2.p), slope, float(h0.mlp2.fc[1].eps),
                            len(heads), *params)
    return [(out[2 * i], out[2 * i + 1]) for i in range(len(heads))]


PTCLS_HEAD_FUSED = _os.environ.get('SUG_PTCLS_HEAD_FUSED', '1') != '0'


def ptcls_head_supported(points, fc2):
    if not (PTCLS_HEAD_FUSED and points.is_cuda and points.dtype == torch.float32 and points.dim() == 3 and len(fc2) == 5):
        return False
    l1, l2, l3 = fc2[0], fc2[2], fc2[4]
    for t in (l1.weight, l1.bias, l2.weight, l2.bias, l3.weight, l3.bias):
        if t is None or not t.is_cuda or t.dtype != torch.float32:
            return False
    B, P, K = points.shape
    if l1.in_features != K or l2.in_features != l1.out_features or l3.in_features != l2.out_features:
        return False
    return bool(lib().sug_ptcls_head_supported(B, P, K, l1.out_features, l2.out_features, l3.out_features))


class _PtclsHead(torch.autograd.Function):

    @staticmethod
    def forward(ctx, points, w1, b1, w2, b2, w3, b3):
        _need_gpu(points, w1, b1, w2, b2, w3, b3)
        p = points.detach().contiguous()
        W = [t.detach().contiguous() for t in (w1, b1, w2, b2, w3, b3)]
        B, P, K = p.shape
        N1, N2, NC = W[0].shape[0], W[2].shape[0], W[4].shape[0]
        new = lambda *shape: torch.empty(*shape, dtype=torch.float32, device=p.device)
        mean, h1, h2, logits = new(B, K), new(B, N1), new(B, N2), new(B, NC)
        check(lib().sug_ptcls_head_fwd(_p(p), B, P, K, _p(W[0]), _p(W[1]), N1, _p(W[2]), _p(W[3]), N2, _p(W[4]), _p(W[5]), NC,
                                       _p(mean), _p(h1), _p(h2), _p(logits), _st()), 'sug_ptcls_head_fwd')
        ctx.save_for_backward(mean, h1, h2, W[0], W[2], W[4])
        ctx.P = P
        return logits

    @staticmethod
    def backward(ctx, g):
        mean, h1, h2, w1, w2, w3 = ctx.saved_tensors
        B, K = mean.shape
        P, N1, N2, NC = ctx.P, w1.shape[0], w2.shape[0], w3.shape[0]
        g = g.contiguous()
        new = lambda *shape: torch.empty(*shape, dtype=torch.float32, device=g.device)
        dz1, dz2, dpts = new(B, N1), new(B, N2), new(B, P, K)
        dw1, db1, dw2, db2, dw3, db3 = new(N1, K), new(N1), new(N2, N1), new(N2), new(NC, N2), new(NC)
        check(lib().sug_ptcls_head_bwd(_p(g), _p(mean), _p(h1), _p(h2), B, P, K, _p(w1), N1, _p(w2), N2, _p(w3), NC,
                                       _p(dz1), _p(dz2), _p(dpts), _p(dw1), _p(db1), _p(dw2), _p(db2), _p(dw3), _p(db3), _st()),
              'sug_ptcls_head_bwd')
        return dpts, dw1, db1, dw2, db2, dw3, db3


def ptcls_head(points, w1, b1, w2, b2, w3, b3):
    return _PtclsHead.apply(points, w1, b1, w2, b2, w3, b3)




@contextlib.contextmanager
def deferred_bn_counts():
    if CTX.pending_counts is not None:
        yield
        return
    CTX.pending_counts = {}
    try:
        yield
    finally:
        flush_bn_counts()
        CTX.pending_counts = None


def flush_bn_counts():
    pend = CTX.pending_counts
    if pend:
        torch._foreach_add_([t for t, _ in pend.values()], [n for _, n in pend.values()])
        pend.clear()


def _count_bn_call(bn, n=None):
    if bn.training and bn.num_batches_tracked is not None:
        n = CTX.bn_groups if n is None else n
        if CTX.pending_counts is not None:
            t = bn.num_batches_tracked
            old = CTX.pending_counts.get(id(t))
            CTX.pending_counts[id(t)] = (t, n + (old[1] if old else 0))
        else:
            bn.num_batches_tracked.add_(n)




@contextlib.contextmanager
def record_bn_stats():
    with CTX.scoped(bn_record=[]):
        yield CTX.bn_record


def _record_bn(bn, coef):
    if CTX.bn_record is not None and bn.training and bn.track_running_stats:
        CTX.bn_record.append((bn, coef))


def replay_bn_stats(rec):
    rec = list(rec)
    i = 0
    while i < len(rec):
        run, seen = [], set()
        while i < len(rec) and len(run) < 16 and id(rec[i][0]) not in seen:
            seen.add(id(rec[i][0]))
            run.append(rec[i])
            i += 1
        if len(run) == 1:
            bn_replay(*run[0])
            continue
        c3s = []
        for _, coef in run:
            c3 = coef if coef.dim() == 3 else coef.unsqueeze(0)
            c3s.append(c3 if c3.is_contiguous() else c3.contiguous())
        n = len(run)
        I32, F32 = ctypes.c_int32 * n, ctypes.c_float * n
        check(lib().sug_bn_replay_multi(n, _ptrs(c3s), I32(*[c.shape[0] for c in c3s]), I32(*[c.shape[2] for c in c3s]),
                                        F32(*[float(bn.momentum) for bn, _ in run]), _ptrs([bn.running_mean for bn, _ in run]),
                                        _ptrs([bn.running_var for bn, _ in run]), _st()), 'sug_bn_replay_multi')
        for (bn, _), c3 in zip(run, c3s):
            _count_bn_call(bn, c3.shape[0])


def bn_replay(bn, coef):
    c3 = coef if coef.dim() == 3 else coef.unsqueeze(0)
    c3 = c3 if c3.is_contiguous() else c3.contiguous()
    G, _, C = c3.shape
    check(lib().sug_bn_replay(_p(c3), G, C, float(bn.momentum), _p(bn.running_mean), _p(bn.running_var), _st()),
          'sug_bn_replay')
    _count_bn_call(bn, G)


def bn_act_rows(y, bn, slope):
    _count_bn_call(bn)
    out, coef = _BNActRows.apply(y, bn.weight, bn.bias, _bn_state(bn), slope)
    _record_bn(bn, coef)
    return out


class _BNActPool(torch.autograd.Function):

    @staticmethod
    def forward(ctx, y, gamma, beta, st, slope):
        _need_gpu(y, gamma)
        y, B, N, C, ld = _rows3(y)
        G = st.G
        _check_groups('bn_act_pool', B, 'clouds', G)
        dev = y.device
        g, b, coef = _bn_params(gamma, beta, st, C)
        pooled = torch.empty(B, 2 * C, dtype=torch.float32, device=dev)
        omax, omean = pooled[:, :C], pooled[:, C:]
        arg = torch.empty(B, C, dtype=torch.int32, device=dev)
        stats = torch.empty(2 * C, dtype=torch.float64, device=dev)
        wss = _stats_ws(C, dev)
        wsp = torch.empty(12 * (B // G) * C, dtype=torch.float32, device=dev)
        check(lib().sug_bn_act_pool_layer_fwd(_p(y), ld, B, N, C, G, _p(g), _p(b), st.train, st.eps, st.momentum,
                                              float(slope), _p(st.mean), _p(st.var), _p(coef), _p(omax),
                                              _p(omean), 2 * C, _p(arg), _p(stats), _p(wss), _p(wsp), _st()),
              'sug_bn_act_pool_layer_fwd')
        ctx.save_for_backward(y, coef, arg)
        ctx.meta = (B, N, C, ld, float(slope), st.train, G)
        return pooled

    @staticmethod
    def backward(ctx, g):
        y, coef, arg = ctx.saved_tensors
        B, N, C, ld, slope, train, G = ctx.meta
        dev = y.device
        if g.stride(1) != 1 or g.stride(0) < 2 * C:
            g = g.contiguous()
        gmax, gmean, ldp = g[:, :C], g[:, C:], g.stride(0)
        red = torch.empty(G, 2 * C, dtype=torch.float64, device=dev)
        ws = _stats_ws(C, dev)
        dy = torch.empty(B, N, C, dtype=torch.float32, device=dev)
        rf = torch.empty(2 * C, dtype=torch.float32, device=dev)
        check(lib().sug_bn_act_pool_layer_bwd(_p(y), ld, _p(coef), _p(gmax), _p(gmean), ldp, _p(arg), B, N, C, G, slope,
                                              train, _p(red), _p(ws), _p(dy), C, _p(rf), _st()),
              'sug_bn_act_pool_layer_bwd')
        return (dy,) + _dgamma_dbeta(rf) + (None, None)


def bn_update_stats(y, bn):
    if not bn.training:
        return
    _need_gpu(y)
    C = y.shape[-1]
    y2 = y.detach().reshape(-1, C)
    if y2.stride(1) != 1:
        y2 = y2.contiguous()
    rows, G = y2.shape[0], CTX.bn_groups
    _check_groups('bn_update_stats', rows, 'rows', G)
    rg = rows // G
    g, b = bn.weight.detach().contiguous(), bn.bias.detach().contiguous()
    coef = torch.empty(5, C, dtype=torch.float32, device=y.device)
    ws = _stats_ws(C, y.device)
    for i in range(G):
        yi = y2[i * rg:(i + 1) * rg]
        check(lib().sug_col_stats_bn(_p(yi), yi.stride(0), rg, C, _p(g), _p(b), bn.eps, bn.momentum,
                                     _p(bn.running_mean), _p(bn.running_var), _p(coef), _p(ws), _st()),
              'sug_col_stats_bn')
    _count_bn_call(bn)


def bn_act_pool_cat(y, bn, slope):
    _count_bn_call(bn)
    return _BNActPool.apply(y, bn.weight, bn.bias, _bn_state(bn), slope)


def bn_act_pool(y, bn, slope):
    C = y.shape[-1]
    pooled = bn_act_pool_cat(y, bn, slope)
    return pooled[:, :C], pooled[:, C:]


def _edgeconv_out(out_holder, B, N, Co, dev):
    if out_holder is None:
        return torch.empty(B, N, Co, dtype=torch.float32, device=dev)
    out = out_holder[0]
    if tuple(out.shape) != (B, N, Co) or out.stride(2) != 1 or out.stride(0) != N * out.stride(1) \
            or out.dtype != torch.float32 or out.requires_grad:
        raise RuntimeError('edgeconv: bad destination slice')
    return out


def _edgeconv_backward(gout, z, arg, s1, pq, ldpq, idx, coef, B, N, k, Co, G, slope, train):
    dev = gout.device
    gout, _, _, _, ldg = _rows3(gout)
    a = torch.empty(B, N, Co, dtype=torch.float32, device=dev)
    red = (torch.empty if train else torch.zeros)(G + 1, 2 * Co, dtype=torch.float64, device=dev)
    ws = _stats_ws(Co, dev)
    off = torch.empty(B, N + 1, dtype=torch.int32, device=dev)
    ent = torch.empty(B, N * k, dtype=torch.int32, device=dev)
    dpq = torch.empty(B, N, 2 * Co, dtype=torch.float32, device=dev)
    rf = torch.empty(2 * Co, dtype=torch.float32, device=dev)
    check(_timed('edgeconv_layer_bwd_Co%d' % Co, {'B': B, 'N': N, 'k': k, 'Co': Co},
                 lambda: lib().sug_edgeconv_layer_bwd(_p(gout), ldg, _p(z), _p(arg), _p(s1), _p(pq), ldpq, _p(idx),
                                                      _p(coef), B, N, k, Co, G, train, slope, _p(a),
                                                      _p(red), _p(off), _p(ent), _p(dpq), 2 * Co, _p(ws), _p(rf), _st())),
          'sug_edgeconv_layer_bwd')
    return (dpq,) + _dgamma_dbeta(rf)


class _EdgeConv(torch.autograd.Function):

    @staticmethod
    def forward(ctx, pq, idx, gamma, beta, st, slope, out_holder, grad_on=True):
        _need_gpu(pq, idx, gamma)
        pq, B, N, C2, ld = _rows3(pq)
        Co = C2 // 2
        idx = _i32(idx).contiguous()
        k = idx.shape[2]
        G = st.G
        _check_groups('edgeconv', B, 'clouds', G)
        dev = pq.device
        gamma_c, beta_c, coef = _bn_params(gamma, beta, st, Co)
        need_bwd = grad_on and any(ctx.needs_input_grad[i] for i in (0, 2, 3))
        z = torch.empty(B, N, Co, dtype=torch.float32, device=dev)
        arg = torch.empty(B, N, Co, dtype=torch.uint8, device=dev)
        s1 = torch.empty(B, N, Co, dtype=torch.float32, device=dev) if need_bwd else None
        stats = torch.empty(2 * Co, dtype=torch.float64, device=dev)
        ws = _stats_ws(Co, dev)
        out = _edgeconv_out(out_holder, B, N, Co, dev)
        ldo = out.stride(1)
        check(_timed('edgeconv_layer_fwd_Co%d' % Co, {'B': B, 'N': N, 'k': k, 'Co': Co},
                     lambda: lib().sug_edgeconv_layer_fwd(_p(pq), ld, _p(idx), _p(gamma_c), _p(beta_c), B, N, k, Co, G,
                                                          st.train, st.eps, st.momentum, float(slope),
                                                          _p(st.mean), _p(st.var), _p(z), _p(arg), _p(s1),
                                                          _p(coef), _p(out), ldo, _p(stats), _p(ws), _st())),
              'sug_edgeconv_layer_fwd')
        if need_bwd:
            ctx.save_for_backward(pq, idx, z, arg, s1, coef)
            ctx.meta = (B, N, k, Co, ld, float(slope), st.train, G)
        coef_out = coef[0] if G == 1 else coef
        ctx.mark_non_differentiable(coef_out)
        ctx.set_materialize_grads(False)
        return out, coef_out

    @staticmethod
    def backward(ctx, gout, _gcoef):
        if gout is None:
            return (None,) * 8
        pq, idx, z, arg, s1, coef = ctx.saved_tensors
        B, N, k, Co, ld, slope, train, G = ctx.meta
        dpq, dgamma, dbeta = _edgeconv_backward(gout, z, arg, s1, pq, ld, idx, coef, B, N, k, Co, G, slope, train)
        return dpq, None, dgamma, dbeta, None, None, None, None


def edgeconv_bn_act_max(pq, idx, gamma, beta, running_mean, running_var, training, slope, eps=1e-5, momentum=0.1,
                        out=None):
    return _EdgeConv.apply(pq, idx, gamma, beta, _BNState(running_mean, running_var, training, eps, momentum), slope,
                           None if out is None else [out], torch.is_grad_enabled())


EDGECONV_FUSED = _os.environ.get('SUG_EDGECONV_FUSED', '1') == '1'


EDGECONV_FUSED_MAXC = int(_os.environ.get('SUG_EDGECONV_FUSED_MAXC', '64'))


def edgeconv_fused_supported(N, k, Cin, Co):
    return EDGECONV_FUSED and Cin <= EDGECONV_FUSED_MAXC and bool(lib().sug_edgeconv_fused_supported(N, k, Cin, Co))


class _EdgeConvFused(torch.autograd.Function):

    @staticmethod
    def forward(ctx, x, wcat, bias, idx, gamma, beta, st, slope, out_holder, grad_on=True):
        _need_gpu(x, wcat, idx, gamma)
        x3, B, N, C, ld = _rows3(x)
        Co = wcat.shape[0] // 2
        idx = _i32(idx).contiguous()
        k = idx.shape[2]
        G = st.G
        _check_groups('edgeconv', B, 'clouds', G)
        dev = x.device
        w = wcat.detach().contiguous()
        b1 = None if bias is None else bias.detach().contiguous()
        gamma_c, beta_c, coef = _bn_params(gamma, beta, st, Co)
        need_bwd = grad_on and any(ctx.needs_input_grad[i] for i in (0, 1, 2, 4, 5))
        z = torch.empty(B, N, Co, dtype=torch.float32, device=dev)
        arg = torch.empty(B, N, Co, dtype=torch.uint8, device=dev) if need_bwd else None
        s1 = torch.empty(B, N, Co, dtype=torch.float32, device=dev) if need_bwd else None
        pq = torch.empty(B, N, 2 * Co, dtype=torch.float32, device=dev) if need_bwd else None
        ws = _stats_ws(Co, dev)
        out = _edgeconv_out(out_holder, B, N, Co, dev)
        check(_timed('edgeconv_fused_fwd_C%d_Co%d' % (C, Co), {'B': B, 'N': N, 'k': k, 'Co': Co, 'C': C, 'train': int(need_bwd)},
                     lambda: lib().sug_edgeconv_fused_layer_fwd(_p(x3), ld, C, _p(w), _p(b1), _p(idx), _p(gamma_c), _p(beta_c),
                                                                B, N, k, Co, G, st.train, st.eps, st.momentum,
                                                                float(slope), _p(st.mean), _p(st.var), _p(z),
                                                                _p(arg), _p(s1), _p(pq), 2 * Co, _p(coef), _p(out),
                                                                out.stride(1), _p(ws), _st())),
              'sug_edgeconv_fused_layer_fwd')
        if need_bwd:
            ctx.save_for_backward(x3, w, idx, z, arg, s1, coef, pq)
            ctx.meta = (B, N, k, C, Co, float(slope), st.train, G, b1 is not None, tuple(x.shape))
        coef_out = coef[0] if G == 1 else coef
        ctx.mark_non_differentiable(coef_out)
        ctx.set_materialize_grads(False)
        return out, coef_out

    @staticmethod
    def backward(ctx, gout, _gcoef):
        if gout is None:
            return (None,) * 10
        x3, w, idx, z, arg, s1, coef, pq = ctx.saved_tensors
        B, N, k, C, Co, slope, train, G, has_bias, xshape = ctx.meta
        dpq, dgamma, dbeta = _edgeconv_backward(gout, z, arg, s1, pq, 2 * Co, idx, coef, B, N, k, Co, G, slope, train)
        x2 = x3.reshape(B * N, C) if x3.is_contiguous() else x3.view(B * N, C) if x3.stride(0) == N * x3.stride(1) else x3.reshape(B * N, C)
        dpq2 = dpq.view(B * N, 2 * Co)
        dx, dw, _ = linear_rows_backward(x2, w, dpq2, ctx.needs_input_grad[0], ctx.needs_input_grad[1], False)
        db = None
        if has_bias and ctx.needs_input_grad[2]:
            db = colsum(dpq2[:, Co:])
        return (None if dx is None else dx.view(xshape)), dw, db, None, dgamma, dbeta, None, None, None, None


def edgeconv_fused(x, wcat, bias, idx, bn_weight, bn_bias, running_mean, running_var, training, slope, eps=1e-5,
                   momentum=0.1, out=None):
    return _EdgeConvFused.apply(x, wcat, bias, idx, bn_weight, bn_bias,
                                _BNState(running_mean, running_var, training, eps, momentum), slope,
                                None if out is None else [out], torch.is_grad_enabled())


POINTMLP_MAX = _os.environ.get('SUG_POINTMLP_MAX', '1') != '0'


def pointmlp_max_supported(K, Co, seg):
    return POINTMLP_MAX and K in (64, 128) and Co % 128 == 0 and seg >= 32 and seg % 32 == 0


class _PointMLPMax(torch.autograd.Function):

    @staticmethod
    def forward(ctx, x, weight, bias, gamma, beta, st, slope, seg):
        _need_gpu(x, weight, gamma)
        K = x.shape[-1]
        x2 = x.reshape(-1, K)
        if x2.stride(1) != 1 or x2.stride(0) % 4 or x2.data_ptr() % 16:
            x2 = x2.contiguous()
        rows, Co = x2.shape[0], weight.shape[0]
        _check_groups('pointmlp_max', rows, 'rows', st.G, seg)
        S = rows // seg
        dev = x.device
        w2 = weight.detach().reshape(Co, K).contiguous()
        b1 = None if bias is None else bias.detach().contiguous()
        g, b, coef = _bn_params(gamma, beta, st, Co)
        zext = torch.empty(S, Co, dtype=torch.float32, device=dev)
        arg = torch.empty(S, Co, dtype=torch.int32, device=dev)
        out = torch.empty(S, Co, dtype=torch.float32, device=dev)
        ws = _stats_ws(Co, dev)
        check(_timed('pointmlp_max_K%d_Co%d' % (K, Co), {'B': rows, 'N': seg, 'k': K, 'Co': Co},
                     lambda: lib().sug_pointmlp_max_layer_fwd(_p(x2), x2.stride(0), rows, K, _p(w2), _p(b1), _p(g), _p(b),
                                                              Co, seg, st.G, st.train, st.eps, st.momentum,
                                                              float(slope), _p(st.mean), _p(st.var), _p(zext),
                                                              _p(arg), _p(coef), _p(out), Co, _p(ws), _st())),
              'sug_pointmlp_max_layer_fwd')
        if any(ctx.needs_input_grad[i] for i in (0, 1, 2, 3, 4)):
            ctx.save_for_backward(x2, w2, b1, zext, arg, coef)
            ctx.meta = (rows, K, Co, seg, st.G, float(slope), st.training, tuple(x.shape), tuple(weight.shape))
        ctx.mark_non_differentiable(coef)
        ctx.set_materialize_grads(False)
        return out, coef

    @staticmethod
    def backward(ctx, gout, _gcoef):
        x2, w2, b1, zext, arg, coef = ctx.saved_tensors
        rows, K, Co, seg, G, slope, training, xshape, wshape = ctx.meta
        if gout is None:
            gout = torch.zeros_like(zext)
        dx, dw, db, dgamma, dbeta = _pointmlp_max_backward(gout, x2, w2, b1, zext, arg, coef, rows, K, Co, seg, G, slope, training)
        return dx.view(xshape), dw.view(wshape), db, dgamma, dbeta, None, None, None


def _pointmlp_max_backward(gout, x2, w2, b1, zext, arg, coef, rows, K, Co, seg, G, slope, training):
    dev = gout.device
    S = rows // seg
    rg, sg = rows // G, S // G
    gout = gout.reshape(S, Co)
    if gout.stride(1) != 1 or gout.stride(0) % 4 or gout.data_ptr() % 16:
        gout = gout.contiguous()
    a = torch.empty(S, Co, dtype=torch.float32, device=dev)
    red = torch.empty(G, 2 * Co, dtype=torch.float64, device=dev)
    ws = _stats_ws(Co, dev)
    dx = torch.empty(rows, K, dtype=torch.float32, device=dev) if training else \
        torch.zeros(rows, K, dtype=torch.float32, device=dev)
    zdb = Co if (b1 is not None and training) else 0
    zbuf = torch.zeros(Co * K + zdb, dtype=torch.float32, device=dev)
    dw = zbuf[:Co * K].view(Co, K)
    dws = torch.empty(Co, K, dtype=torch.float32, device=dev)
    wsp = torch.empty(int(lib().sug_pointmlp_max_bwd_workspace(rg, K, Co, seg)), dtype=torch.float32, device=dev)
    L = lib()
    f32 = dict(dtype=torch.float32, device=dev)
    kbk2, negA, negv = torch.empty(2, Co, **f32), torch.empty(K, K, **f32), torch.empty(K, **f32)
    nkb, nwk = torch.empty(Co, **f32), torch.empty(Co, K, **f32)
    xtx, sx = torch.empty(K, K, **f32), torch.empty(K, **f32)
    wsx = torch.empty(int(L.sug_linear_dw_workspace(rg, K, K)), **f32) if training else None
# ... 2124 lines not shown
```

Before: 13570.

## Share the node-adapt first half across passes and batch the SA glue kernels

Adds Bsrc-aware variants of node_offset, group_max and interp3_cat, so clouds planned for several passes can read source features from a single shared batch. The model caches the node-adapt projection, residual and BN stats in the prefix cache entry and reuses them through precomputed forward values, replaying the BN statistics. A batched glue path computes offsets, knn, group-max and interpolation for all passes in one go. This is meant to cut repeated forward work and launches, at the cost of more cache state and more complex autograd plumbing.

```diff
diff --git a/include/sug_amd.h b/include/sug_amd.h
--- a/include/sug_amd.h
+++ b/include/sug_amd.h
@@ -60,6 +60,8 @@
 
 int sug_group_max(const float* feat, int64_t ldf, const int32_t* idx, int B, int N, int S,
                   int ns, int C, float* out, int32_t* arg, void* stream);
+int sug_group_max_shared(const float* feat, int64_t ldf, int Bsrc, const int32_t* idx, int B, int N, int S,
+                         int ns, int C, float* out, int32_t* arg, void* stream);
 int sug_group_max_bwd(const float* g, const int32_t* arg, int B, int N, int S, int C,
                       float* dfeat, int64_t ldf, void* stream);
 
@@ -171,9 +173,15 @@
 int sug_node_offset_bwd(const float* proj, const float* loc, const int32_t* fidx,
                         const int32_t* gidx, const float* goff, int B, int N, int S, int ns,
                         float* dproj, void* stream);
+int sug_node_offset_fwd_shared(const float* proj, int Bsrc, const float* loc, const int32_t* fidx,
+                               const int32_t* gidx, int B, int N, int S, int ns, float* off, float* nloc,
+                               void* stream);
 int sug_interp3_cat_fwd(const float* fea, int64_t ldf, int C1, const float* node,
                         const int32_t* idx3, const float* d3, int B, int N, int S, int C2,
                         float* out, int64_t ldo, void* stream);
+int sug_interp3_cat_fwd_shared(const float* fea, int64_t ldf, int C1, int Bsrc, const float* node,
+                               const int32_t* idx3, const float* d3, int B, int N, int S, int C2,
+                               float* out, int64_t ldo, void* stream);
 int sug_interp3_cat_bwd(const float* g, int64_t ldg, int C1, const float* node, const int32_t* idx3,
                         const float* d3, const float* xyz, const float* nloc, int B, int N, int S,
                         int C2, float* dnode, float* dnloc, void* stream);
diff --git a/sug_amd/csrc/adapt.hip b/sug_amd/csrc/adapt.hip
--- a/sug_amd/csrc/adapt.hip
+++ b/sug_amd/csrc/adapt.hip
@@ -6,14 +6,14 @@
                                                               const float* __restrict__ loc,
                                                               const int32_t* __restrict__ fidx,
                                                               const int32_t* __restrict__ gidx, int N,
-                                                              int S, int ns, int total,
+                                                              int S, int ns, int total, int Bsrc,
                                                               float* __restrict__ off,
                                                               float* __restrict__ nloc) {
   const int e = blockIdx.x * 4 + (threadIdx.x >> 6);
   if (e >= total) return;
   const int lane = threadIdx.x & 63;
   const int b = e / S;
-  const float* pb = proj + (int64_t)b * N * 3;
+  const float* pb = proj + (int64_t)(b % Bsrc) * N * 3;
   const float* lb = loc + (int64_t)b * N * 3;
   int f = fidx[e];
   f = f < 0 ? 0 : (f >= N ? N - 1 : f);
@@ -249,12 +249,13 @@
                                                               int C1, const float* __restrict__ node,
                                                               const int32_t* __restrict__ idx3,
                                                               const float* __restrict__ d3, int N, int S,
-                                                              int C2, int64_t BN, float* __restrict__ out,
-                                                              int64_t ldo) {
+                                                              int C2, int64_t BN, int64_t BNsrc,
+                                                              float* __restrict__ out, int64_t ldo) {
   const int64_t p = (int64_t)blockIdx.x * 16 + threadIdx.x / 16;
   if (p >= BN) return;
   const int lane = threadIdx.x & 15;
   const int64_t b = p / N;
+  const int64_t ps = p % BNsrc;
   const float r0 = 1.0f / fmaxf(d3[p * 3 + 0], 1e-10f), r1 = 1.0f / fmaxf(d3[p * 3 + 1], 1e-10f),
               r2 = 1.0f / fmaxf(d3[p * 3 + 2], 1e-10f);
   const float R = (r0 + r1) + r2;
@@ -263,7 +264,7 @@
   const float* n1 = node + (b * S + idx3[p * 3 + 1]) * C2;
   const float* n2 = node + (b * S + idx3[p * 3 + 2]) * C2;
   for (int c = lane * 4; c < C1; c += 64)
-    *reinterpret_cast<float4*>(out + p * ldo + c) = *reinterpret_cast<const float4*>(fea + p * ldf + c);
+    *reinterpret_cast<float4*>(out + p * ldo + c) = *reinterpret_cast<const float4*>(fea + ps * ldf + c);
   for (int c = lane * 4; c < C2; c += 64) {
     const float4 a = *reinterpret_cast<const float4*>(n0 + c), bq = *reinterpret_cast<const float4*>(n1 + c),
                  cq = *reinterpret_cast<const float4*>(n2 + c);
@@ -441,16 +442,24 @@
 
 }
 
+extern "C" int sug_node_offset_fwd_shared(const float* proj, int Bsrc, const float* loc, const int32_t* fidx,
+                                          const int32_t* gidx, int B, int N, int S, int ns, float* off,
+                                          float* nloc, void* stream) {
+  SUG_REQUIRE(proj && loc && fidx && gidx && off && nloc, "sug_node_offset_fwd: null pointer");
+  SUG_REQUIRE(B > 0 && N > 0 && S > 0 && ns > 0, "sug_node_offset_fwd: bad shape");
+  SUG_REQUIRE(Bsrc > 0 && B % Bsrc == 0, "sug_node_offset_fwd: %d clouds are not whole passes over %d source clouds", B, Bsrc);
+  SUG_REQUIRE((int64_t)B * S <= INT32_MAX, "sug_node_offset_fwd: B*S too large");
+  const int total = B * S;
+  hipLaunchKernelGGL(node_offset_fwd_kernel, dim3(sug_divup(total, 4)), dim3(256), 0, (hipStream_t)stream,
+                     proj, loc, fidx, gidx, N, S, ns, total, Bsrc, off, nloc);
+  SUG_LAUNCH_CHECK("sug_node_offset_fwd");
+  return SUG_OK;
+}
+
 extern "C" int sug_node_offset_fwd(const float* proj, const float* loc, const int32_t* fidx,
                                    const int32_t* gidx, int B, int N, int S, int ns, float* off,
                                    float* nloc, void* stream) {
-  SUG_REQUIRE(proj && loc && fidx && gidx && off && nloc, "sug_node_offset_fwd: null pointer");
-  SUG_REQUIRE(B > 0 && N > 0 && S > 0 && ns > 0, "sug_node_offset_fwd: bad shape");
-  const int total = B * S;
-  hipLaunchKernelGGL(node_offset_fwd_kernel, dim3(sug_divup(total, 4)), dim3(256), 0, (hipStream_t)stream,
-                     proj, loc, fidx, gidx, N, S, ns, total, off, nloc);
-  SUG_LAUNCH_CHECK("sug_node_offset_fwd");
-  return SUG_OK;
+  return sug_node_offset_fwd_shared(proj, B, loc, fidx, gidx, B, N, S, ns, off, nloc, stream);
 }
 
 extern "C" int sug_node_offset_bwd(const float* proj, const float* loc, const int32_t* fidx,
@@ -505,20 +514,27 @@
   return SUG_OK;
 }
 
-extern "C" int sug_interp3_cat_fwd(const float* fea, int64_t ldf, int C1, const float* node,
-                                   const int32_t* idx3, const float* d3, int B, int N, int S, int C2,
-                                   float* out, int64_t ldo, void* stream) {
+extern "C" int sug_interp3_cat_fwd_shared(const float* fea, int64_t ldf, int C1, int Bsrc, const float* node,
+                                          const int32_t* idx3, const float* d3, int B, int N, int S, int C2,
+                                          float* out, int64_t ldo, void* stream) {
   SUG_REQUIRE((fea || C1 == 0) && node && idx3 && d3 && out, "sug_interp3_cat_fwd: null pointer");
   SUG_REQUIRE(B > 0 && N > 0 && S >= 3 && C1 >= 0 && C2 > 0 && C1 % 4 == 0 && C2 % 4 == 0 && ldf % 4 == 0 &&
                   ldo % 4 == 0 && ldo >= C1 + C2 && ldf >= C1,
               "sug_interp3_cat_fwd: bad shape (channel counts and strides must be multiples of 4)");
+  SUG_REQUIRE(Bsrc > 0 && B % Bsrc == 0, "sug_interp3_cat_fwd: %d clouds are not whole passes over %d source clouds", B, Bsrc);
   SUG_REQUIRE(((uintptr_t)fea % 16 == 0) && ((uintptr_t)node % 16 == 0) && ((uintptr_t)out % 16 == 0),
               "sug_interp3_cat_fwd: pointers must be 16-byte aligned");
   const int64_t BN = (int64_t)B * N;
   hipLaunchKernelGGL(interp3_cat_fwd_kernel, dim3(sug_divup(BN, 16)), dim3(256), 0, (hipStream_t)stream, fea,
-                     ldf, C1, node, idx3, d3, N, S, C2, BN, out, ldo);
+                     ldf, C1, node, idx3, d3, N, S, C2, BN, (int64_t)Bsrc * N, out, ldo);
   SUG_LAUNCH_CHECK("sug_interp3_cat_fwd");
   return SUG_OK;
+}
+
+extern "C" int sug_interp3_cat_fwd(const float* fea, int64_t ldf, int C1, const float* node,
+                                   const int32_t* idx3, const float* d3, int B, int N, int S, int C2,
+                                   float* out, int64_t ldo, void* stream) {
+  return sug_interp3_cat_fwd_shared(fea, ldf, C1, B, node, idx3, d3, B, N, S, C2, out, ldo, stream);
 }
 
 extern "C" int sug_interp3_cat_bwd(const float* g, int64_t ldg, int C1, const float* node,
diff --git a/sug_amd/csrc/group.hip b/sug_amd/csrc/group.hip
--- a/sug_amd/csrc/group.hip
+++ b/sug_amd/csrc/group.hip
@@ -32,13 +32,13 @@
 
 __global__ __launch_bounds__(256) void group_max_kernel(const float* __restrict__ feat, int64_t ldf,
                                                         const int32_t* __restrict__ idx, int N, int S,
-                                                        int ns, int C, int64_t total,
+                                                        int ns, int C, int64_t total, int Bsrc,
                                                         float* __restrict__ out,
                                                         int32_t* __restrict__ arg) {
   for (int64_t e = (int64_t)blockIdx.x * 256 + threadIdx.x; e < total; e += (int64_t)gridDim.x * 256) {
     const int c = (int)(e % C);
     const int64_t row = e / C;
-    const int b = (int)(row / S);
+    const int b = (int)(row / S) % Bsrc;
     const int32_t* ir = idx + row * ns;
     float best = -INFINITY;
     int bj = -1;
@@ -222,15 +222,21 @@
   return SUG_OK;
 }
 
+extern "C" int sug_group_max_shared(const float* feat, int64_t ldf, int Bsrc, const int32_t* idx, int B, int N, int S,
+                                    int ns, int C, float* out, int32_t* arg, void* stream) {
+  SUG_REQUIRE(feat && idx && out && arg, "sug_group_max: null pointer");
+  SUG_REQUIRE(B > 0 && N > 0 && S > 0 && ns > 0 && C > 0 && ldf >= C, "sug_group_max: bad shape");
+  SUG_REQUIRE(Bsrc > 0 && B % Bsrc == 0, "sug_group_max: %d clouds are not whole passes over %d source clouds", B, Bsrc);
+  const int64_t total = (int64_t)B * S * C;
+  hipLaunchKernelGGL(group_max_kernel, dim3(ew_grid(total)), dim3(256), 0, (hipStream_t)stream, feat,
+                     ldf, idx, N, S, ns, C, total, Bsrc, out, arg);
+  SUG_LAUNCH_CHECK("sug_group_max");
+  return SUG_OK;
+}
+
 extern "C" int sug_group_max(const float* feat, int64_t ldf, const int32_t* idx, int B, int N, int S,
                              int ns, int C, float* out, int32_t* arg, void* stream) {
-  SUG_REQUIRE(feat && idx && out && arg, "sug_group_max: null pointer");
-  SUG_REQUIRE(B > 0 && N > 0 && S > 0 && ns > 0 && C > 0 && ldf >= C, "sug_group_max: bad shape");
-  const int64_t total = (int64_t)B * S * C;
-  hipLaunchKernelGGL(group_max_kernel, dim3(ew_grid(total)), dim3(256), 0, (hipStream_t)stream, feat,
-                     ldf, idx, N, S, ns, C, total, out, arg);
-  SUG_LAUNCH_CHECK("sug_group_max");
-  return SUG_OK;
+  return sug_group_max_shared(feat, ldf, B, idx, B, N, S, ns, C, out, arg, stream);
 }
 
 extern "C" int sug_group_max_bwd(const float* g, const int32_t* arg, int B, int N, int S, int C,
diff --git a/sug_amd/model/Model.py b/sug_amd/model/Model.py
--- a/sug_amd/model/Model.py
+++ b/sug_amd/model/Model.py
@@ -21,6 +21,7 @@
         self._live, self.provider = live, provider
         self._source = weakref.ref(source) if source is not None else None
         self._flag = flag = [True]
+        self.shared = None
         last = tensors[-1]
         if last.requires_grad:
             last.register_hook(lambda grad, f=flag: f.__setitem__(0, False))
@@ -75,7 +76,7 @@
 
 def _dead_prefix_entry():
     e = _PrefixEntry.__new__(_PrefixEntry)
-    e.tensors, e.extra, e._source, e._flag, e._live, e.provider = (), None, None, [False], None, None
+    e.tensors, e.extra, e._source, e._flag, e._live, e.provider, e.shared = (), None, None, [False], None, None, None
     return e
 
 
@@ -140,24 +141,34 @@
         self._prefix_cache = {}
 
     def _prefix_params(self):
-        return [p for m in (self.conv1, self.conv2) for p in m.parameters()]
+        return [p for m in (self.conv1, self.conv2) for p in m.parameters()] + self.node_fea_adapt.shared_params()
 
     def _prefix(self, x, loc, nb, out1=None, wc=(None, None)):
         if not _sharing_on(self.share_prefix, self.training):
             x1 = self.conv1.edge_rows(loc, nb(loc, 0), out=out1, wcat=wc[0])
-            return x1, self.conv2.edge_rows(x1, nb(x1, 1), wcat=wc[1])
+            return x1, self.conv2.edge_rows(x1, nb(x1, 1), wcat=wc[1]), None, None
         key = self._prefix_key(x)
         hit = self._prefix_cache.get(key)
         if hit is not None and hit.serves(x):
             x1, x2 = hit.tensors
-            st1, st2 = hit.extra
-            ops.replay_bn_stats([(self.conv1.conv[1], st1), (self.conv2.conv[1], st2)])
-            return x1, x2
+            st1, st2, st_res, proj, y, res = hit.extra
+            if st_res is None:
+                ops.replay_bn_stats([(self.conv1.conv[1], st1), (self.conv2.conv[1], st2)])
+                return x1, x2, None, None
+            bn_res = self.node_fea_adapt.residual.conv[1]
+            ops.replay_bn_stats([(self.conv1.conv[1], st1), (self.conv2.conv[1], st2), (bn_res, st_res)])
+            if hit.shared is None:
+                hit.shared = _mu.SharedHalf(proj, y, res, [(bn_res, st_res)])
+            return x1, x2, hit.shared, None
         x1, st1 = self.conv1.edge_rows(loc, nb(loc, 0), return_stats=True, out=out1, wcat=wc[0])
         x2, st2 = self.conv2.edge_rows(x1, nb(x1, 1), return_stats=True, wcat=wc[1])
+        return x1, x2, _mu.SharedHalf(), (st1, st2)
+
+    def _keep_prefix(self, x, x1, x2, shared, st12):
+        half = (shared.stats[0][1], shared.proj, shared.y, shared.res) if shared.filled else (None,) * 4
         self._prune_prefix_cache()
-        self._prefix_cache[key] = _PrefixEntry((x1, x2), (st1, st2), source=x)
-        return x1, x2
+        e = self._prefix_cache[self._prefix_key(x)] = _PrefixEntry((x1, x2), st12 + half, source=x)
+        e.shared = shared if shared.filled else None
 
     def plan_geometry(self, x, passes, groups=1):
         return self.node_fea_adapt.plan_geometry(ops.cloud_rows(x), passes, groups)
@@ -171,8 +182,10 @@
         nb = lambda f, i: gi[i] if gi[i] is not None else ops.knn(f, self.k)
         cat_in = torch.empty(B, N, 512, dtype=torch.float32, device=x.device)
         wc = edge_wcats((self.conv1, self.conv2, self.conv3, self.conv4))
-        x1, x2 = self._prefix(x, loc, nb, out1=cat_in[:, :, 0:64], wc=wc[:2])
-        x_, node_fea, _ = self.node_fea_adapt.rows(x2, loc)
+        x1, x2, shared, miss = self._prefix(x, loc, nb, out1=cat_in[:, :, 0:64], wc=wc[:2])
+        x_, node_fea, _ = self.node_fea_adapt.rows(x2, loc, shared=shared)
+        if miss is not None:
+            self._keep_prefix(x, x1, x2, shared, miss)
         with torch.set_grad_enabled(torch.is_grad_enabled() and feat_grad):
             x2 = ops.linear_rows(x_, self.conv1d.weight.squeeze(-1), self.conv1d.bias)
             x3 = self.conv3.edge_rows(x2, nb(x2, 2), out=cat_in[:, :, 128:256], wcat=wc[2])
diff --git a/sug_amd/model/model_utils.py b/sug_amd/model/model_utils.py
--- a/sug_amd/model/model_utils.py
+++ b/sug_amd/model/model_utils.py
@@ -1,3 +1,5 @@
+import os
+
 import torch
 import torch.nn as nn
 import torch.nn.functional as F
@@ -65,10 +67,14 @@
         w = self.conv[0].weight
         return w.view(w.shape[0], w.shape[1])
 
-    def rows(self, x):
-        y = ops.linear_rows(x, self.weight2d(), self.conv[0].bias)
+    def rows(self, x, pre=None, keep=None):
+        y = ops.linear_rows(x, self.weight2d(), self.conv[0].bias, pre=None if pre is None else pre[0])
+        if keep is not None:
+            keep.append(y)
         if self.activation in _ACT_SLOPE and OWN_BN(self.conv[1]):
-            return ops.bn_act_rows(y, self.conv[1], _ACT_SLOPE[self.activation])
+            return ops.bn_act_rows(y, self.conv[1], _ACT_SLOPE[self.activation], pre=None if pre is None else pre[1:])
+        if pre is not None:
+            raise RuntimeError('conv_2d.rows: a precomputed forward needs the fused BatchNorm + activation path')
         return self.conv[2](_bn_rows(self.conv[1], y))
 
     def forward(self, x):
@@ -167,6 +173,23 @@
         return y.view(-1, self.K, self.K)
 
 
+SA_GLUE_BATCHED = os.environ.get('SUG_SA_GLUE_BATCHED', '1') != '0'
+
+
+class SharedHalf:
+    __slots__ = ('proj', 'y', 'res', 'stats', 'glue')
+
+    def __init__(self, proj=None, y=None, res=None, stats=()):
+        self.proj, self.y, self.res, self.stats, self.glue = proj, y, res, tuple(stats), None
+
+    @property
+    def filled(self):
+        return self.proj is not None
+
+    def fill(self, proj, y, res, stats):
+        self.proj, self.y, self.res, self.stats = proj.detach(), y.detach(), res.detach(), tuple(stats)
+
+
 class adapt_layer_off(nn.Module):
 
     def __init__(self, num_node=64, offset_dim=3, trans_dim_in=64, trans_dim_out=64, fc_dim=64):
@@ -179,12 +202,16 @@
             nn.Tanh())
         self.residual = conv_2d(trans_dim_in, fc_dim, 1)
 
-    def rows(self, fea, loc):
+    def shared_params(self):
+        return list(self.pred_offset.parameters()) + list(self.residual.parameters())
+
+    def rows(self, fea, loc, shared=None):
         B, N, _ = loc.shape
         S = self.num_node
         plan = ops.CTX.geometry_plan
+        passes = None
         if plan:
-            fidx, f_loc, gidx = plan.pop(0)
+            fidx, f_loc, gidx, passes, p = plan.pop(0)
             if fidx.shape != (B, S) or gidx.shape[:2] != (B, S):
                 raise RuntimeError('geometry plan does not match the SA-node module')
         else:
@@ -193,19 +220,39 @@
             f_loc = ops.gather_rows(loc, fidx)
             gidx = ops.ball_query(loc, f_loc, 0.3, 64)
         w_off = self.pred_offset[0].weight.view(self.offset_dim, -1)
-        proj = ops.linear_rows(fea, w_off)
+        if shared is not None and shared.filled:
+            proj = ops.linear_rows(fea, w_off, pre=shared.proj)
+            res = self.residual.rows(fea, pre=(shared.y, shared.res, shared.stats[0][1]))
+        else:
+            proj = ops.linear_rows(fea, w_off)
+            if shared is not None:
+                keep = []
+                with ops.record_bn_stats() as rec:
+                    res = self.residual.rows(fea, keep=keep)
+                if len(rec) == 1:
+                    shared.fill(proj, keep[0], res, rec)
+            else:
+                res = self.residual.rows(fea)
+        fused = self.offset_dim == 3 and gidx.shape[2] == S and fea.shape[2] % 4 == 0 and res.shape[2] % 4 == 0
+        pre = None
+        if shared is not None and passes is not None and fused and passes['count'] > 1 and SA_GLUE_BATCHED:
+            if shared.glue is None or shared.glue[0] is not passes:
+                shared.glue = (passes, ops.sa_glue_passes(proj, res, fea, passes['loc'], passes['fidx'], passes['gidx'], 64))
+            pre = {k: v[p * B:(p + 1) * B] for k, v in shared.glue[1].items()}
+            if p == passes['count'] - 1:
+                shared.glue = None
+        P = (lambda *ks: tuple(pre[k] for k in ks)) if pre is not None else (lambda *ks: None)
         if self.offset_dim == 3 and gidx.shape[2] == S:
-            node_off, n_loc = ops.node_offset(proj, loc, fidx, gidx)
+            node_off, n_loc = ops.node_offset(proj, loc, fidx, gidx, P('off', 'nloc'))
         else:
             sem = torch.tanh(ops.gather_rows(proj, gidx) - ops.gather_rows(proj, fidx).unsqueeze(2))
             g_loc = ops.gather_rows(loc, gidx) - f_loc.unsqueeze(2)
             node_off = (sem * g_loc).mean(dim=2)
             n_loc = f_loc + node_off
-        gidx2 = ops.knn_query(loc, n_loc, 64)
-        res = self.residual.rows(fea)
-        node_fea = ops.group_max(res, gidx2)
+        gidx2 = pre['gidx2'] if pre is not None else ops.knn_query(loc, n_loc, 64)
+        node_fea = ops.group_max(res, gidx2, P('node', 'arg'))
         if fea.shape[2] % 4 == 0 and node_fea.shape[2] % 4 == 0:
-            out = ops.interp3_cat(fea, node_fea, loc, n_loc)
+            out = ops.interp3_cat(fea, node_fea, loc, n_loc, P('out', 'idx3', 'd3'))
         else:
             out = torch.cat((fea, point_utils.interpolate_rows(loc, n_loc, node_fea, 3)), dim=2)
         return out, node_fea, node_off
@@ -225,7 +272,8 @@
         fidx = ops.fps(locp, S, st)
         f_loc = ops.gather_rows(locp, fidx)
         gidx = ops.ball_query(locp, f_loc, 0.3, 64)
-        return [[(fidx[p * B:(p + 1) * B], f_loc[p * B:(p + 1) * B], gidx[p * B:(p + 1) * B])] for p in range(passes)]
+        whole = {'count': passes, 'loc': locp, 'fidx': fidx, 'gidx': gidx}
+        return [[(fidx[p * B:(p + 1) * B], f_loc[p * B:(p + 1) * B], gidx[p * B:(p + 1) * B], whole, p)] for p in range(passes)]
 
     def forward(self, input_fea, input_loc):
         out, node_fea, node_off = self.rows(input_fea.squeeze(-1).transpose(1, 2).contiguous(),
diff --git a/sug_amd/ops.py b/sug_amd/ops.py
--- a/sug_amd/ops.py
+++ b/sug_amd/ops.py
@@ -348,14 +348,15 @@
 
 class _GroupMax(torch.autograd.Function):
     @staticmethod
-    def forward(ctx, feat, idx):
+    def forward(ctx, feat, idx, pre=None):
         _need_gpu(feat, idx)
-        feat_c, B, N, C, ld = _rows3(feat)
-        idx = _i32(idx).contiguous()
-        S, ns = idx.shape[1], idx.shape[2]
-        out = torch.empty(B, S, C, dtype=torch.float32, device=feat.device)
-        arg = torch.empty(B, S, C, dtype=torch.int32, device=feat.device)
-        check(lib().sug_group_max(_p(feat_c), ld, _p(idx), B, N, S, ns, C, _p(out), _p(arg), _st()), 'sug_group_max')
+        if pre is not None:
+            out, arg = pre
+            B, N, C = feat.shape
+        else:
+            feat_c, B, N, C, ld = _rows3(feat)
+            idx = _i32(idx).contiguous()
+            out, arg = _group_max_raw(feat_c, ld, B, idx, N, C)
         ctx.save_for_backward(arg)
         ctx.shape = (B, N, C)
         return out
@@ -368,11 +369,23 @@
         g = g.contiguous()
         d = torch.zeros(B, N, C, dtype=torch.float32, device=g.device)
         check(lib().sug_group_max_bwd(_p(g), _p(arg), B, N, S, C, _p(d), C, _st()), 'sug_group_max_bwd')
-        return d, None
-
-
-def group_max(feat, idx):
-    return _GroupMax.apply(feat, idx)
+        return d, None, None
+
+
+def _group_max_raw(feat_c, ld, Bsrc, idx, N, C):
+    B, S, ns = idx.shape
+    out = torch.empty(B, S, C, dtype=torch.float32, device=feat_c.device)
+    arg = torch.empty(B, S, C, dtype=torch.int32, device=feat_c.device)
+    if Bsrc == B:
+        check(lib().sug_group_max(_p(feat_c), ld, _p(idx), B, N, S, ns, C, _p(out), _p(arg), _st()), 'sug_group_max')
+    else:
+        check(lib().sug_group_max_shared(_p(feat_c), ld, Bsrc, _p(idx), B, N, S, ns, C, _p(out), _p(arg), _st()),
+              'sug_group_max_shared')
+    return out, arg
+
+
+def group_max(feat, idx, pre=None):
+    return _GroupMax.apply(feat, idx, pre)
 
 
 DW_LIBRARY_SHAPES = set()
@@ -384,10 +397,12 @@
 class _LinearRows(torch.autograd.Function):
 
     @staticmethod
-    def forward(ctx, x, weight, bias):
+    def forward(ctx, x, weight, bias, pre=None):
         M, N = weight.shape
         x2 = x.reshape(-1, N)
-        if OWN_ROWS_GEMM and N in (64, 128) and M % 128 == 0 and x2.shape[0] >= 4096 and x2.stride(1) == 1 \
+        if pre is not None:
+            y = pre.detach()
+        elif OWN_ROWS_GEMM and N in (64, 128) and M % 128 == 0 and x2.shape[0] >= 4096 and x2.stride(1) == 1 \
                 and x2.stride(0) % 4 == 0 and x2.data_ptr() % 16 == 0 and weight.is_contiguous():
             y = torch.empty(x2.shape[0], M, dtype=torch.float32, device=x.device)
             check(_timed('rows_gemm_K%d_Co%d' % (N, M), {'B': x2.shape[0], 'N': 1, 'k': N, 'Co': M},
@@ -407,7 +422,7 @@
         M, N = weight.shape
         dx, dw, db = linear_rows_backward(x.reshape(-1, N), weight, g.reshape(-1, M), ctx.needs_input_grad[0],
                                           ctx.needs_input_grad[1], ctx.has_bias and ctx.needs_input_grad[2])
-        return (None if dx is None else dx.view(x.shape)), dw, db
+        return (None if dx is None else dx.view(x.shape)), dw, db, None
 
 
 DW_BMM = _os.environ.get('SUG_DW_BMM', '1') == '1'
@@ -464,26 +479,24 @@
     return dx, dw, db
 
 
-def linear_rows(x, weight, bias=None):
+def linear_rows(x, weight, bias=None, pre=None):
     _need_gpu(x, weight)
     if x.dtype != torch.float32:
         raise RuntimeError('sug_amd.ops.linear_rows: fp32 rows only (got %s)' % x.dtype)
-    return _LinearRows.apply(x, weight, bias)
+    return _LinearRows.apply(x, weight, bias, pre)
 
 
 class _NodeOffset(torch.autograd.Function):
 
     @staticmethod
-    def forward(ctx, proj, loc, fidx, gidx):
+    def forward(ctx, proj, loc, fidx, gidx, pre=None):
         _need_gpu(proj, loc, fidx, gidx)
         proj, loc = proj.contiguous(), loc.detach().contiguous()
         fidx, gidx = _i32(fidx).contiguous(), _i32(gidx).contiguous()
-        B, N, _ = proj.shape
-        S, ns = gidx.shape[1], gidx.shape[2]
-        off = torch.empty(B, S, 3, dtype=torch.float32, device=proj.device)
-        nloc = torch.empty(B, S, 3, dtype=torch.float32, device=proj.device)
-        check(lib().sug_node_offset_fwd(_p(proj), _p(loc), _p(fidx), _p(gidx), B, N, S, ns, _p(off), _p(nloc), _st()),
-              'sug_node_offset_fwd')
+        if pre is not None:
+            off, nloc = pre
+        else:
+            off, nloc = _node_offset_raw(proj, loc, fidx, gidx)
         ctx.save_for_backward(proj, loc, fidx, gidx)
         ctx.set_materialize_grads(False)
         return off, nloc
@@ -494,31 +507,46 @@
         B, N, _ = proj.shape
         S, ns = gidx.shape[1], gidx.shape[2]
         if goff is None and gnloc is None:
-            return None, None, None, None
+            return None, None, None, None, None
         g = (goff if gnloc is None else gnloc if goff is None else goff + gnloc).contiguous()
         dproj = torch.empty_like(proj)
         check(lib().sug_node_offset_bwd(_p(proj), _p(loc), _p(fidx), _p(gidx), _p(g), B, N, S, ns, _p(dproj), _st()),
               'sug_node_offset_bwd')
-        return dproj, None, None, None
-
-
-def node_offset(proj, loc, fidx, gidx):
-    return _NodeOffset.apply(proj, loc, fidx, gidx)
+        return dproj, None, None, None, None
+
+
+def _node_offset_raw(proj, loc, fidx, gidx):
+    Bsrc, N, _ = proj.shape
+    B, S, ns = gidx.shape
+    off = torch.empty(B, S, 3, dtype=torch.float32, device=proj.device)
+    nloc = torch.empty(B, S, 3, dtype=torch.float32, device=proj.device)
+    if Bsrc == B:
+        check(lib().sug_node_offset_fwd(_p(proj), _p(loc), _p(fidx), _p(gidx), B, N, S, ns, _p(off), _p(nloc), _st()),
+              'sug_node_offset_fwd')
+    else:
+        check(lib().sug_node_offset_fwd_shared(_p(proj), Bsrc, _p(loc), _p(fidx), _p(gidx), B, N, S, ns, _p(off), _p(nloc),
+                                               _st()), 'sug_node_offset_fwd_shared')
+    return off, nloc
+
+
+def node_offset(proj, loc, fidx, gidx, pre=None):
+    return _NodeOffset.apply(proj, loc, fidx, gidx, pre)
 
 
 class _Interp3Cat(torch.autograd.Function):
 
     @staticmethod
-    def forward(ctx, fea, node, xyz, nloc):
+    def forward(ctx, fea, node, xyz, nloc, pre=None):
         _need_gpu(fea, node, xyz, nloc)
         fea, B, N, C1, ldf = _rows3(fea)
         node = node.contiguous()
         xyz, nlocd = xyz.detach().contiguous(), nloc.detach().contiguous()
         S, C2 = node.shape[1], node.shape[2]
-        idx3, d3 = three_nn_raw(xyz, nlocd)
-        out = torch.empty(B, N, C1 + C2, dtype=torch.float32, device=fea.device)
-        check(lib().sug_interp3_cat_fwd(_p(fea) if C1 else None, ldf if C1 else 0, C1, _p(node), _p(idx3), _p(d3), B, N, S,
-                                        C2, _p(out), C1 + C2, _st()), 'sug_interp3_cat_fwd')
+        if pre is not None:
+            out, idx3, d3 = pre
+        else:
+            idx3, d3 = three_nn_raw(xyz, nlocd)
+            out = _interp3_cat_raw(fea, ldf, C1, B, node, idx3, d3, N)
         ctx.save_for_backward(node, idx3, d3, xyz, nlocd)
         ctx.meta = (B, N, S, C1, C2)
         return out
@@ -543,11 +571,43 @@
             dnloc = torch.zeros_like(nloc)
             check(L.sug_interp3_cat_bwd(_p(g), C1 + C2, C1, _p(node), _p(idx3), _p(d3), _p(xyz), _p(nloc), B, N, S, C2,
                                         _p(dnode), _p(dnloc), _st()), 'sug_interp3_cat_bwd')
-        return g[:, :, :C1], dnode, None, dnloc
-
-
-def interp3_cat(fea, node, xyz, nloc):
-    return _Interp3Cat.apply(fea, node, xyz, nloc)
+        return g[:, :, :C1], dnode, None, dnloc, None
+
+
+def _interp3_cat_raw(fea, ldf, C1, Bsrc, node, idx3, d3, N):
+    B, S, C2 = node.shape
+    out = torch.empty(B, N, C1 + C2, dtype=torch.float32, device=node.device)
+    fp, ld = (_p(fea), ldf) if C1 else (None, 0)
+    if Bsrc == B:
+        check(lib().sug_interp3_cat_fwd(fp, ld, C1, _p(node), _p(idx3), _p(d3), B, N, S, C2, _p(out), C1 + C2, _st()),
+              'sug_interp3_cat_fwd')
+    else:
+        check(lib().sug_interp3_cat_fwd_shared(fp, ld, C1, Bsrc, _p(node), _p(idx3), _p(d3), B, N, S, C2, _p(out), C1 + C2,
+                                               _st()), 'sug_interp3_cat_fwd_shared')
+    return out
+
+
+def interp3_cat(fea, node, xyz, nloc, pre=None):
+    return _Interp3Cat.apply(fea, node, xyz, nloc, pre)
+
+
+def sa_glue_passes(proj, res, fea, locp, fidx, gidx, k):
+    _need_gpu(proj, res, fea, locp, fidx, gidx)
+    with torch.no_grad():
+        B, N, _ = proj.shape
+        proj_c, locp = proj.detach().contiguous(), locp.detach().contiguous()
+        fidx, gidx = _i32(fidx).contiguous(), _i32(gidx).contiguous()
+        if locp.shape[0] % B or fidx.shape[0] != locp.shape[0] or gidx.shape[0] != locp.shape[0] or fea.shape[0] != B or \
+                res.shape[0] != B:
+            raise RuntimeError('sa_glue_passes: %d planned clouds are not whole passes over a batch of %d' % (locp.shape[0], B))
+        off, nloc = _node_offset_raw(proj_c, locp, fidx, gidx)
+        gidx2 = knn_query(locp, nloc, k)
+        res_c, _, _, C, ldr = _rows3(res.detach())
+        node, arg = _group_max_raw(res_c, ldr, B, gidx2, N, C)
+        idx3, d3 = three_nn_raw(locp, nloc)
+        fea_c, _, _, C1, ldf = _rows3(fea.detach())
+        out = _interp3_cat_raw(fea_c, ldf, C1, B, node, idx3, d3, N)
+    return {'off': off, 'nloc': nloc, 'gidx2': gidx2, 'node': node, 'arg': arg, 'idx3': idx3, 'd3': d3, 'out': out}
 
 
 def bn_coef(stats, gamma, beta, count, eps, momentum, running_mean, running_var, out=None):
@@ -629,7 +689,7 @@
 class _BNActRows(torch.autograd.Function):
 
     @staticmethod
-    def forward(ctx, y, gamma, beta, st, slope):
+    def forward(ctx, y, gamma, beta, st, slope, pre=None):
         _need_gpu(y, gamma)
         C = y.shape[-1]
         y2 = y.reshape(-1, C)
@@ -638,13 +698,16 @@
         rows = y2.shape[0]
         _check_groups('bn_act_rows', rows, 'rows', st.G)
         dev = y.device
-        g, b, coef = _bn_params(gamma, beta, st, C)
-        out = torch.empty(rows, C, dtype=torch.float32, device=dev)
-        stats = torch.empty(2 * C, dtype=torch.float64, device=dev)
-        ws = _stats_ws(C, dev)
-        check(lib().sug_bn_act_rows_fwd(_p(y2), C, rows, C, st.G, _p(g), _p(b), st.train, st.eps, st.momentum,
-                                        float(slope), _p(st.mean), _p(st.var), _p(coef), _p(out), C,
-                                        _p(stats), _p(ws), _st()), 'sug_bn_act_rows_fwd')
+        if pre is not None:
+            out, coef = pre[0].detach().reshape(rows, C), pre[1].detach()
+        else:
+            g, b, coef = _bn_params(gamma, beta, st, C)
+            out = torch.empty(rows, C, dtype=torch.float32, device=dev)
+            stats = torch.empty(2 * C, dtype=torch.float64, device=dev)
+            ws = _stats_ws(C, dev)
+            check(lib().sug_bn_act_rows_fwd(_p(y2), C, rows, C, st.G, _p(g), _p(b), st.train, st.eps, st.momentum,
+                                            float(slope), _p(st.mean), _p(st.var), _p(coef), _p(out), C,
+                                            _p(stats), _p(ws), _st()), 'sug_bn_act_rows_fwd')
         if any(ctx.needs_input_grad[i] for i in (0, 1, 2)):
             ctx.save_for_backward(y2, coef)
             ctx.meta = (rows, C, float(slope), st.training, tuple(y.shape), st.G)
@@ -659,7 +722,7 @@
         if gout is None:
             gout = torch.zeros_like(y2)
         dy, dgamma, dbeta = _bn_act_rows_backward(gout, y2, coef, rows, C, slope, training, G)
-        return dy.view(shape), dgamma, dbeta, None, None
+        return dy.view(shape), dgamma, dbeta, None, None, None
 
 
 def _bn_act_rows_backward(gout, y2, coef, rows, C, slope, training, G):
@@ -1104,7 +1167,9 @@
     _count_bn_call(bn, G)
 
 
-def bn_act_rows(y, bn, slope):
+def bn_act_rows(y, bn, slope, pre=None):
+    if pre is not None:
+        return _BNActRows.apply(y, bn.weight, bn.bias, _bn_state(bn), slope, pre)[0]
     _count_bn_call(bn)
     out, coef = _BNActRows.apply(y, bn.weight, bn.bias, _bn_state(bn), slope)
     _record_bn(bn, coef)
```

Measured after the change: 13840 (median of 6 runs). 1.02x the previous value.
